# sb17v/GaussianK-SGD

Measured on AMD Instinct MI355X. Metric: images/sec (whole node) ResNet-50 k=0.1% at 1/2/4/8 MI355X; effective grad compression ratio, higher is better.
Workload: dtype fp32; 1 GPU; model=resnet50, global_batch=512, per_gpu_batch=512, image_size=224, parallelism=dp1, compressor=gaussian, buckets=1, threshold=524288000, planner=threshold, exchange=local, momentum_correction=True, hip_graph=False, f32_matmul=bf16x6

## Files before the change

### gaussiank_sgd_amd/models/resnet_imagenet.py

```python
from __future__ import annotations

from typing import List, Optional, Type, Union

import torch
import torch.nn as nn

from ..ops.bn import BNAct, global_avg_pool
from ..ops.conv1x1 import Conv1x1, Conv3x3, conv_stats
from ..ops.stem import StemConv


def conv3x3(inp: int, out: int, stride: int = 1, groups: int = 1, dilation: int = 1) -> nn.Conv2d:
    return Conv3x3(inp, out, stride, groups, dilation)


def conv1x1(inp: int, out: int, stride: int = 1) -> nn.Conv2d:
    return Conv1x1(inp, out, stride)


class BasicBlock(nn.Module):
    expansion = 1

    def __init__(self, inplanes, planes, stride=1, downsample=None, groups=1, base_width=64):
        super().__init__()
        self.conv1 = conv3x3(inplanes, planes, stride)
        self.bn1 = BNAct(planes, act="relu")
        self.conv2 = conv3x3(planes, planes)
        self.bn2 = BNAct(planes, act="relu")
        self.downsample = downsample

    def forward(self, x):
        x, xs = x if isinstance(x, tuple) else (x, x)
        identity = xs if self.downsample is None else _shortcut(self.downsample, xs, self.bn2)
        y, st = conv_stats(self.conv1, x)
        out = self.bn1(y, stats=st)
        y, st = conv_stats(self.conv2, out)
        return self.bn2(y, identity, stats=st)


class Bottleneck(nn.Module):
    expansion = 4

    def __init__(self, inplanes, planes, stride=1, downsample=None, groups=1, base_width=64):
        super().__init__()
        width = int(planes * (base_width / 64.0)) * groups
        self.conv1 = conv1x1(inplanes, width)
        self.bn1 = BNAct(width, act="relu")
        self.conv2 = conv3x3(width, width, stride, groups)
        self.bn2 = BNAct(width, act="relu")
        self.conv3 = conv1x1(width, planes * self.expansion)
        self.bn3 = BNAct(planes * self.expansion, act="relu")
        self.downsample = downsample

    def forward(self, x):
        x, xs = x if isinstance(x, tuple) else (x, x)
        identity = xs if self.downsample is None else _shortcut(self.downsample, xs, self.bn3)
        y, st = conv_stats(self.conv1, x)
        out = self.bn1(y, stats=st)
        y, st = conv_stats(self.conv2, out)
        out = self.bn2(y, stats=st)
        y, st = conv_stats(self.conv3, out)
        return self.bn3(y, identity, stats=st)


class ConvBN(nn.Sequential):

    def forward(self, x):
        y, st = conv_stats(self[0], x)
        return self[1](y, stats=st)

    def forward_deferred(self, x, consumer: BNAct):
        y, st = conv_stats(self[0], x)
        if consumer.fused_ok(y):
            h = self[1].deferred(y, stats=st)
            if h is not None:
                return h
        return self[1](y, stats=st)


def _shortcut(ds: nn.Module, xs: torch.Tensor, consumer: BNAct) -> torch.Tensor:
    if isinstance(ds, ConvBN):
        return ds.forward_deferred(xs, consumer)
    return ds(xs)


class ResNet(nn.Module):
    def __init__(self, block: Type[Union[BasicBlock, Bottleneck]], layers: List[int], num_classes: int = 1000,
                 zero_init_residual: bool = False, groups: int = 1, width_per_group: int = 64,
                 name: Optional[str] = None):
        super().__init__()
        self.inplanes = 64
        self.groups = groups
        self.base_width = width_per_group
        self.conv1 = StemConv(3, 64)
        self.bn1 = BNAct(64, act="relu", pool=(3, 2, 1))
        self.maxpool = nn.Identity()
        self.layer1 = self._make_layer(block, 64, layers[0])
        self.layer2 = self._make_layer(block, 128, layers[1], stride=2)
        self.layer3 = self._make_layer(block, 256, layers[2], stride=2)
        self.layer4 = self._make_layer(block, 512, layers[3], stride=2)
        self.avgpool = nn.AdaptiveAvgPool2d((1, 1))
        self.fc = nn.Linear(512 * block.expansion, num_classes)
        self.name = name or "resnet"
        for m in self.modules():
            if isinstance(m, nn.Conv2d):
                nn.init.kaiming_normal_(m.weight, mode="fan_out", nonlinearity="relu")
            elif isinstance(m, nn.BatchNorm2d):
                nn.init.ones_(m.weight)
                nn.init.zeros_(m.bias)
        blocks = [b for layer in (self.layer1, self.layer2, self.layer3, self.layer4) for b in layer]
        self.bn1.twin = True
        for b in blocks[:-1]:
            (b.bn3 if isinstance(b, Bottleneck) else b.bn2).twin = True
        for i, b in enumerate(blocks):
            b.bn1.bwd_link = True
            if isinstance(b, Bottleneck):
                b.bn2.bwd_link = True
            if i + 1 < len(blocks) and blocks[i + 1].downsample is None:
                (b.bn3 if isinstance(b, Bottleneck) else b.bn2).bwd_link = True
        if zero_init_residual:
            for m in self.modules():
                if isinstance(m, Bottleneck):
                    nn.init.zeros_(m.bn3.weight)
                elif isinstance(m, BasicBlock):
                    nn.init.zeros_(m.bn2.weight)

    def _make_layer(self, block, planes, blocks, stride=1):
        downsample = None
        if stride != 1 or self.inplanes != planes * block.expansion:
            downsample = ConvBN(conv1x1(self.inplanes, planes * block.expansion, stride),
                                BNAct(planes * block.expansion))
        layers = [block(self.inplanes, planes, stride, downsample, self.groups, self.base_width)]
        self.inplanes = planes * block.expansion
        for _ in range(1, blocks):
            layers.append(block(self.inplanes, planes, groups=self.groups, base_width=self.base_width))
        return nn.Sequential(*layers)

    def forward(self, x):
        y, st = conv_stats(self.conv1, x)
        x = self.maxpool(self.bn1(y, stats=st))
        x = self.layer4(self.layer3(self.layer2(self.layer1(x))))
        return self.fc(global_avg_pool(x))


def resnet18(num_classes=1000, **kw):
    return ResNet(BasicBlock, [2, 2, 2, 2], num_classes, name="resnet18", **kw)


def resnet34(num_classes=1000, **kw):
    return ResNet(BasicBlock, [3, 4, 6, 3], num_classes, name="resnet34", **kw)


def resnet50(num_classes=1000, **kw):
    return ResNet(Bottleneck, [3, 4, 6, 3], num_classes, name="resnet50", **kw)


def resnet101(num_classes=1000, **kw):
    return ResNet(Bottleneck, [3, 4, 23, 3], num_classes, name="resnet101", **kw)


def resnet152(num_classes=1000, **kw):
    return ResNet(Bottleneck, [3, 8, 36, 3], num_classes, name="resnet152", **kw)


def resnext50_32x4d(num_classes=1000, **kw):
    return ResNet(Bottleneck, [3, 4, 6, 3], num_classes, groups=32, width_per_group=4, name="resnext50", **kw)
```

### gaussiank_sgd_amd/ops/autotune.py

```python
from __future__ import annotations

import os
from typing import Callable, Dict, Iterable, List, Optional, Tuple

import torch

_TUNE = os.environ.get("GKSGD_GEMM_TUNE", "1") != "0"
_choices: Dict[tuple, tuple] = {}
_OWN = ("hip", "w3", "mat", "wino", "wx6")
_GK_MARGIN = float(os.environ.get("GKSGD_GK_MARGIN", "0.05"))
_timings: Dict[tuple, list] = {}
_NT_CFGS = [1, 2, 3, 4, 11, 13, 21, 22, 23, 24, 111, 113, 121, 122, 123, 124, 25, 26, 27, 125, 126, 127,
            211, 212, 213, 214, 221, 222, 223, 224]
NT_GRIDS = (0, 512, 1 << 20)
_TN_CFGS = [(c, s) for c in (1, 2, 3, 4, 5, 6, 7, 8, 21, 22, 23, 24, 27, 9, 29, 101, 121, 102, 122) for s in (0, 128)]
_NT_CFGS_F32 = [1, 2, 3, 4, 7, 11, 12, 13, 14, 21, 22, 23, 24, 101, 102, 103, 104, 201, 202, 203, 204,
                1001, 1002, 1003, 1004, 1005, 1006, 1007, 1021, 1022, 1101, 1102, 1103]
_TN_CFGS_F32 = [(c, s) for c in (1, 2, 3, 4, 5, 6, 7, 8, 9, 11, 12, 13, 14, 15, 16) for s in (0, 64)]
_TN_SMALL_M = 1 << 17
_TN_SMALL_F32 = [(c, s) for c in (4, 5, 11, 14, 15) for s in (16, 32, 128)]


X6 = 100000
_NT_CFGS_X6 = [c + X6 for c in (1, 2, 3, 4, 5, 6, 7, 12, 13, 101, 102, 103, 104, 105, 106, 107, 202, 203, 1001, 1002, 1003)]
_NT_CFGS_X62 = [2 * X6 + t for t in range(1, 8)] + [3 * X6 + t for t in range(1, 8)]
_F32MM = os.environ.get("GKSGD_F32_MATMUL", "bf16x6")


def set_f32_matmul(mode: str) -> str:
    global _F32MM
    if mode not in ("native", "bf16x6"):
        raise ValueError("f32 matmul mode must be 'native' or 'bf16x6', got %r" % (mode,))
    prev, _F32MM = _F32MM, mode
    return prev


def f32_matmul() -> str:
    return _F32MM


def _x6() -> bool:
    return _F32MM == "bf16x6"


_TN_CFGS_X62 = [(2 * X6 + t, sp) for t in (1, 2, 3, 4, 5, 6, 7, 8) for sp in (0, 64)]


def tn_cfgs(dt: torch.dtype) -> List[Tuple[int, int]]:
    if dt == torch.float32:
        extra = _TN_CFGS_X62 if os.environ.get("GKSGD_TN_X62", "0") == "1" else []
        return _TN_CFGS_F32 + ([(c + X6, sp) for c, sp in _TN_CFGS_F32] + extra if _x6() else [])
    return _TN_CFGS


def tn_small_cfgs(dt: torch.dtype, rows: int) -> List[Tuple[int, int]]:
    if dt != torch.float32 or rows > _TN_SMALL_M:
        return []
    return _TN_SMALL_F32 + ([(c + X6, sp) for c, sp in _TN_SMALL_F32] if _x6() else [])


def nt_cfgs(dt: torch.dtype) -> List[int]:
    if dt == torch.float32:
        return _NT_CFGS_F32 + (_NT_CFGS_X6 + _NT_CFGS_X62 if _x6() else [])
    return _NT_CFGS


_SPLITK_BASE = (4, 1, 1001, 1002, 1003)
_SPLITK_MAX_OUT = 1 << 22
SPLITK_GRIDS = (0, 1 << 20)


def splitk_cfgs(dt: torch.dtype, M: int, N: int, K: int) -> List[int]:
    if dt != torch.float32 or M * N > _SPLITK_MAX_OUT:
        return []
    base = list(_SPLITK_BASE) + ([c + X6 for c in _SPLITK_BASE] if _x6() else [])
    return [c + 10000 * S for S in (2, 4, 8) if K % (64 * S) == 0 and K // S >= 128 for c in base]




def dkey(dt: torch.dtype) -> tuple:
    if dt == torch.float32:
        return ("f32", "x6") if _x6() else ("f32",)
    return ()


def hip_cands(run: Callable[[int, int], object], pairs: Iterable[Tuple[int, int]]) -> list:
    return [(("hip", c, g), (lambda c=c, g=g: run(c, g))) for c, g in pairs]


def _time(fn: Callable[[], None], reps: int = 5) -> float:
    fn()
    a = torch.cuda.Event(enable_timing=True)
    b = torch.cuda.Event(enable_timing=True)
    a.record()
    for _ in range(reps):
        fn()
    b.record()
    b.synchronize()
    return a.elapsed_time(b) / reps


def choice(key: tuple) -> Optional[tuple]:
    return _choices.get(key)


def pick(key: tuple, cands: List[Tuple[tuple, Callable[[], None]]]) -> tuple:
    got = _choices.get(key)
    if got is not None:
        return got
    if len(cands) == 1:
        _choices[key] = cands[0][0]
        return cands[0][0]
    if not _TUNE:
        for tag, fn in cands:
            try:
                fn()
            except RuntimeError:
                continue
            _choices[key] = tag
            return tag
        raise RuntimeError("no candidate ran for %s" % (key,))
    log = _timings.setdefault(key, [])
    screened = []
    for tag, fn in cands:
        try:
            t = _time(fn, reps=3)
        except RuntimeError as e:
            log.append((tag, "error: %s" % str(e).splitlines()[0][:200]))
            continue
        screened.append((t, tag, fn))
    screened.sort(key=lambda e: e[0])
    best, best_t = cands[-1][0], float("inf")
    timed = []
    for _, tag, fn in screened[:4]:
        t = _time(fn, reps=12)
        log.append((tag, round(t, 4)))
        timed.append((t, tag))
        if t < best_t:
            best, best_t = tag, t
    if best[0] not in _OWN and _GK_MARGIN > 0:
        own = [(t, tag) for t, tag in timed if tag[0] in _OWN]
        if own and min(own)[0] <= best_t * (1.0 + _GK_MARGIN):
            best = min(own)[1]
            log.append((best, "kept: within GKSGD_GK_MARGIN of %s" % (best_t,)))
    _choices[key] = best
    return best


def tuning_log() -> Dict[tuple, list]:
    return dict(_timings)


def load_choices(path: str) -> int:
    import json
    try:
        with open(path) as f:
            rows = json.load(f)
    except (OSError, ValueError):
        return 0
    for k, v in rows:
        _choices.setdefault(tuple(k), tuple(v))
    return len(rows)


def save_choices(path: str) -> None:
    import json
    with open(path, "w") as f:
        json.dump([[list(k), list(v)] for k, v in sorted(_choices.items(), key=str)], f, indent=0)


_CACHE = os.environ.get("GKSGD_GEMM_CACHE", os.path.join(os.path.dirname(os.path.dirname(os.path.dirname(
    os.path.abspath(__file__)))), "tuning", "gemm_choices.json"))
if _TUNE and _CACHE and os.path.exists(_CACHE) and os.environ.get("GKSGD_GEMM_RETUNE", "0") == "0":
    load_choices(_CACHE)
    _only = {d for d in os.environ.get("GKSGD_GEMM_RETUNE_ONLY", "").split(",") if d}
    if _only:
        for _k in [k for k in _choices if k and k[0] in _only]:
            del _choices[_k]


def tuned_choices() -> Dict[tuple, tuple]:
    return dict(_choices)
```

### gaussiank_sgd_amd/ops/bn.py

```python
from __future__ import annotations

import os
from typing import Optional

import torch
import torch.nn as nn
import torch.nn.functional as F

from . import load, require_native

_CL = torch.channels_last
_FIN_FUSE = os.environ.get("GKSGD_BN_FIN_FUSE", "0") == "1"


def _ops():
    return torch.ops.gksgd


def _grad_pair(grads, like):
    gs = [g for g in grads if g is not None]
    out = []
    for g in gs:
        g = g.contiguous(memory_format=_CL)
        if g.dtype != like.dtype:
            g = g.to(like.dtype)
        out.append(g)
    return (out + [None, None])[:2]


class BnLink:

    __slots__ = ("h", "mask", "twin", "dy2", "dz", "part")

    def __init__(self):
        self.h = self.mask = self.dy2 = self.dz = self.part = None
        self.twin = False

    def ready(self) -> bool:
        return self.h is not None and (not self.twin or self.dy2 is not None)

    def clear(self) -> None:
        self.h = self.mask = self.dy2 = self.dz = self.part = None


class ProducerLink:

    __slots__ = ("lazy", "dx")

    def __init__(self):
        self.lazy = None
        self.dx = None

    def matches(self, dy: torch.Tensor) -> bool:
        return self.lazy is not None and dy.data_ptr() == self.lazy[0].data_ptr() and dy.shape == self.lazy[0].shape

    def materialize(self) -> torch.Tensor:
        if self.dx is None:
            dz, x, coef, _, _ = self.lazy
            self.dx = torch.empty_like(x, memory_format=_CL)
            _ops().bn_lazy_apply(dz, x, self.dx, coef)
        return self.dx

    def clear(self) -> None:
        self.lazy = self.dx = None


def _lazy_buffers(x: torch.Tensor):
    C = x.shape[1]
    coef = torch.empty(C, 4, dtype=torch.float32, device=x.device)
    padz = torch.empty(C, dtype=x.dtype, device=x.device)
    padx = torch.empty(C, dtype=x.dtype, device=x.device)
    return coef, padz, padx


def _lazy_ok(x: torch.Tensor, plink) -> bool:
    import os
    return (plink is not None and x.dtype == torch.float32 and x.shape[1] % 64 == 0 and
            os.environ.get("GKSGD_BN_LAZY", "0") != "0")


class _BNActFn(torch.autograd.Function):
    @staticmethod
    def forward(ctx, x, residual, weight, bias, running_mean, running_var, momentum, eps, relu, direct=None,
                nbt=None, twin=False, pre=None, link=None, res_link=None, plink=None, fin=None, rbn=None):
        ctx.direct = direct
        ctx.set_materialize_grads(False)
        C = x.shape[1]
        M = x.numel() // C
        eb = x.element_size()
        y = torch.empty_like(x, memory_format=_CL)
        stats = torch.empty(4, C, dtype=torch.float32, device=x.device)
        ws = torch.empty(int(_ops().bn_workspace_floats(M, C, eb)), dtype=torch.float32, device=x.device)
        rscale, rshift, dlink = rbn if rbn is not None else (None, None, None)
        ctx.dlink = dlink
        if rbn is not None and (residual.dtype != x.dtype or not residual.is_contiguous(memory_format=_CL)):
            raise RuntimeError("deferred residual BN: the pending tensor must match x (dtype, channels-last)")
        if residual is not None and residual.dtype != x.dtype:
            residual = residual.to(x.dtype)
        if residual is not None and not residual.is_contiguous(memory_format=_CL):
            residual = residual.contiguous(memory_format=_CL)
        mask = None
        if relu:
            mask = torch.empty(int(_ops().bn_mask_bytes(M, C, eb)), dtype=torch.uint8, device=x.device)
        pre_t, pre_rows = pre if pre is not None else (None, 0)
        _ops().bn_act_forward(x, residual, y, mask, weight, bias, running_mean, running_var, stats[0], stats[1],
                              stats[2], stats[3], ws, float(eps), float(momentum), bool(relu), nbt, pre_t, pre_rows,
                              fin, rscale, rshift)
        ctx.fin = fin
        ctx.relu = bool(relu)
        ctx.has_res = residual is not None
        ctx.save_for_backward(x, mask, weight, stats[0], stats[1])
        ctx.link = link
        ctx.res_link = res_link
        ctx.plink = plink
        if link is not None:
            link.h, link.mask, link.twin = x, mask, bool(twin)
        return (y, y.view_as(y)) if twin else y

    @staticmethod
    def backward(ctx, *grads):
        x, mask, weight, mean, invstd = ctx.saved_tensors
        link, res_link, plink, dlink = ctx.link, ctx.res_link, ctx.plink, ctx.dlink
        ctx.link = ctx.res_link = ctx.plink = ctx.dlink = None
        gw, gb = ctx.direct if ctx.direct is not None else (None, None)
        lazy = _lazy_ok(x, plink) and ctx.needs_input_grad[0]
        if link is not None and link.part is not None:
            dz = grads[0]
            if dz is None or dz.data_ptr() != link.dz.data_ptr():
                raise RuntimeError("BNAct bwd_link: the linked output had another consumer")
            part, rows = link.part
            link.clear()
            g = torch.empty(2, x.shape[1], dtype=torch.float32, device=x.device)
            if lazy:
                coef, padz, padx = _lazy_buffers(x)
                _ops().bn_bwd_lazy_pre(x, part, rows, weight, mean, invstd, g[0], g[1], coef, padz, padx, gw, gb)
                plink.lazy = (dz, x, coef, padz, padx)
                dx = dz
            elif dlink is not None and ctx.needs_input_grad[1]:
                dx = torch.empty_like(x, memory_format=_CL)
                x2 = dlink.x
                dx2 = torch.empty_like(x2, memory_format=_CL)
                g2 = torch.empty(2, x2.shape[1], dtype=torch.float32, device=x.device)
                ws2 = torch.empty(int(_ops().bn_workspace_floats(x2.numel() // x2.shape[1], x2.shape[1],
                                                                 x2.element_size())),
                                  dtype=torch.float32, device=x.device)
                gw2, gb2 = dlink.direct if dlink.direct is not None else (None, None)
                _ops().bn_act_backward_pre_dual(dz, x, dx, weight, mean, invstd, g[0], g[1], part, rows, gw, gb, x2,
                                                dx2, dlink.weight, dlink.mean, dlink.invstd, g2[0], g2[1], ws2, gw2,
                                                gb2)
                dlink.dz, dlink.dx, dlink.g = dz, dx2, g2
            else:
                dx = torch.empty_like(x, memory_format=_CL)
                _ops().bn_act_backward_pre(dz, x, dx, weight, mean, invstd, g[0], g[1], part, rows, gw, gb, ctx.fin)
            dres = dz if ctx.has_res and ctx.needs_input_grad[1] else None
            if res_link is not None and dres is not None:
                res_link.dy2 = dres
            if ctx.direct is not None:
                return (dx, dres) + (None,) * 16
            dgamma = g[0] if weight is not None and ctx.needs_input_grad[2] else None
            dbeta = g[1] if ctx.needs_input_grad[3] else None
            return (dx, dres, dgamma, dbeta) + (None,) * 14
        if link is not None:
            link.clear()
        dy, dy2 = _grad_pair(grads, x)
        if dy is None:
            return (None,) * 18
        C = x.shape[1]
        M = x.numel() // C
        g = torch.empty(2, C, dtype=torch.float32, device=x.device)
        ws = torch.empty(int(_ops().bn_workspace_floats(M, C, x.element_size())), dtype=torch.float32,
                         device=x.device)
        if lazy:
            dz = torch.empty_like(x, memory_format=_CL)
            coef, padz, padx = _lazy_buffers(x)
            _ops().bn_act_backward_lazy(dy, dy2, mask, x, dz, weight, mean, invstd, g[0], g[1], ws, ctx.relu, coef,
                                        padz, padx, gw, gb)
            plink.lazy = (dz, x, coef, padz, padx)
            dx = dz
            dres = dz if ctx.has_res and ctx.needs_input_grad[1] else None
        else:
            dx = torch.empty_like(x, memory_format=_CL)
            dres = torch.empty_like(x, memory_format=_CL) if ctx.has_res and ctx.needs_input_grad[1] else None
            _ops().bn_act_backward(dy, mask, x, dx, dres, weight, mean, invstd, g[0], g[1], ws, ctx.relu, gw, gb,
                                   dy2, ctx.fin)
        if res_link is not None and dres is not None:
            res_link.dy2 = dres
        if ctx.direct is not None:
            return (dx, dres) + (None,) * 16
        dgamma = g[0] if weight is not None and ctx.needs_input_grad[2] else None
        dbeta = g[1] if ctx.needs_input_grad[3] else None
        return (dx, dres, dgamma, dbeta) + (None,) * 14


class DeferLink:

    __slots__ = ("x", "weight", "mean", "invstd", "direct", "dz", "dx", "g")

    def __init__(self, x, weight, mean, invstd, direct):
        self.x, self.weight, self.mean, self.invstd, self.direct = x, weight, mean, invstd, direct
        self.dz = self.dx = self.g = None


class _BNDeferFn(torch.autograd.Function):

    @staticmethod
    def forward(ctx, x, weight, bias, running_mean, running_var, momentum, eps, stats, direct=None, nbt=None,
                pre=None, dlink=None):
        ctx.direct = direct
        ctx.set_materialize_grads(False)
        C = x.shape[1]
        M = x.numel() // C
        ws = torch.empty(int(_ops().bn_workspace_floats(M, C, x.element_size())), dtype=torch.float32,
                         device=x.device)
        pre_t, pre_rows = pre if pre is not None else (None, 0)
        _ops().bn_act_finalize(x, weight, bias, running_mean, running_var, stats[0], stats[1], stats[2], stats[3], ws,
                               float(eps), float(momentum), nbt, pre_t, pre_rows)
        ctx.save_for_backward(x, weight, stats[0], stats[1])
        ctx.dlink = dlink
        return x.view_as(x)

    @staticmethod
    def backward(ctx, dy):
        x, weight, mean, invstd = ctx.saved_tensors
        dl, ctx.dlink = ctx.dlink, None
        if dy is None:
            return (None,) * 12
        if dl is not None and dl.dx is not None and dl.dz is not None and dy.data_ptr() == dl.dz.data_ptr():
            dx, g = dl.dx, dl.g
            dl.dz = dl.dx = dl.g = None
            if ctx.direct is not None:
                return (dx,) + (None,) * 11
            dgamma = g[0] if weight is not None and ctx.needs_input_grad[1] else None
            dbeta = g[1] if ctx.needs_input_grad[2] else None
            return (dx, dgamma, dbeta) + (None,) * 9
        if dl is not None and dl.dx is not None:
            raise RuntimeError("deferred BN: the consumer's gradient reached the shortcut BN as another tensor")
        dy = dy.contiguous(memory_format=_CL)
        if dy.dtype != x.dtype:
            dy = dy.to(x.dtype)
        C = x.shape[1]
        M = x.numel() // C
        g = torch.empty(2, C, dtype=torch.float32, device=x.device)
        ws = torch.empty(int(_ops().bn_workspace_floats(M, C, x.element_size())), dtype=torch.float32,
                         device=x.device)
        gw, gb = ctx.direct if ctx.direct is not None else (None, None)
        dx = torch.empty_like(x, memory_format=_CL)
        _ops().bn_act_backward(dy, None, x, dx, None, weight, mean, invstd, g[0], g[1], ws, False, gw, gb, None, None)
        if ctx.direct is not None:
            return (dx,) + (None,) * 11
        dgamma = g[0] if weight is not None and ctx.needs_input_grad[1] else None
        dbeta = g[1] if ctx.needs_input_grad[2] else None
        return (dx, dgamma, dbeta) + (None,) * 9


_DEFER = os.environ.get("GKSGD_BN_DEFER", "1") != "0"
_DEFER_BWD = os.environ.get("GKSGD_BN_DEFER_BWD", "1") != "0"


class _BNReLUPoolFn(torch.autograd.Function):

    @staticmethod
    def forward(ctx, x, weight, bias, running_mean, running_var, momentum, eps, pool, direct=None, nbt=None,
                twin=False, pre=None):
        ctx.set_materialize_grads(False)
        k, st, pad = pool
        N, C, H, W = x.shape
        OH = (H + 2 * pad - k) // st + 1
        OW = (W + 2 * pad - k) // st + 1
        y = torch.empty((N, C, OH, OW), dtype=x.dtype, device=x.device, memory_format=_CL)
        amax = torch.empty(N * C * OH * OW, dtype=torch.uint8, device=x.device)
        stats = torch.empty(4, C, dtype=torch.float32, device=x.device)
        M = N * H * W
        ws = torch.empty(int(_ops().bn_workspace_floats(M, C, x.element_size())), dtype=torch.float32,
                         device=x.device)
        pre_t, pre_rows = pre if pre is not None else (None, 0)
        _ops().bn_relu_pool_forward(x, y, amax, weight, bias, running_mean, running_var, stats[0], stats[1],
                                    stats[2], stats[3], ws, float(eps), float(momentum), k, st, pad, nbt, pre_t,
                                    pre_rows)
        ctx.pool = (k, st, pad)
        ctx.direct = direct
        ctx.save_for_backward(x, amax, weight, stats[0], stats[1])
        return (y, y.view_as(y)) if twin else y

    @staticmethod
    def backward(ctx, *grads):
        x, amax, weight, mean, invstd = ctx.saved_tensors
        dy, dy2 = _grad_pair(grads, x)
        if dy is None:
            return (None,) * 12
        k, st, pad = ctx.pool
        C = x.shape[1]
        M = x.numel() // C
        dx = torch.empty_like(x, memory_format=_CL)
        g = torch.empty(2, C, dtype=torch.float32, device=x.device)
        ws = torch.empty(int(_ops().bn_workspace_floats(M, C, x.element_size())), dtype=torch.float32,
                         device=x.device)
        gw, gb = ctx.direct if ctx.direct is not None else (None, None)
        _ops().bn_relu_pool_backward(dy, amax, x, dx, weight, mean, invstd, g[0], g[1], ws, k, st, pad, gw, gb, dy2)
        if ctx.direct is not None:
            return (dx,) + (None,) * 11
        dgamma = g[0] if weight is not None and ctx.needs_input_grad[1] else None
        dbeta = g[1] if ctx.needs_input_grad[2] else None
        return (dx, dgamma, dbeta) + (None,) * 9


_supported_cache = {}


def fused_bn_available(x: torch.Tensor) -> bool:
    if not (x.is_cuda and x.dim() == 4 and x.dtype in (torch.bfloat16, torch.float32)):
        return False
    if not x.is_contiguous(memory_format=_CL):
        return False
    key = (x.shape[1], x.element_size())
    ok = _supported_cache.get(key)
    if ok is None:
        if not load():
# ... 122 lines not shown
```

### gaussiank_sgd_amd/ops/conv1x1.py

```python
from __future__ import annotations

import os
from itertools import product
from typing import Dict

import torch
import torch.nn as nn
import torch.nn.functional as F

from . import autotune
from . import load
from . import streams
from . import weight_prep
from .autotune import (X6, f32_matmul, load_choices, save_choices, set_f32_matmul,
                       tuned_choices, tuning_log)

_CL = torch.channels_last
_ENABLED = os.environ.get("GKSGD_FASTCONV", "1") != "0"
_BIAS_COLSUM = os.environ.get("GKSGD_CONV_BIAS_COLSUM", "1") != "0"
_WINO = os.environ.get("GKSGD_WINO", "1") != "0"
_FORCE = os.environ.get("GKSGD_CONV_FORCE", "")
_WINO_GRIDS = (0, 1 << 20)
_zeros: Dict[torch.device, torch.Tensor] = {}

# ... 101 lines not shown
    cands += autotune.hip_cands(run, product(split, autotune.SPLITK_GRIDS))
    wino = bias is None and _wino_ok(dt, k, s, C, K) and _wino_shape_fits(N, H, W, C, K)
    if wino:
        cands += _wino_cands(x, w, y, False, st, wp=wp)

    def miopen():
        out = F.conv2d(x, w, b16, stride=s, padding=p)
        if st is not None and ws is not None:
            g.bn_stats_partials(out.contiguous(memory_format=_CL), ws)
        return out
    ws = None
    if st is not None and autotune.choice(("fwd", N, C, H, W, K, k, s, True) + autotune.dkey(dt)) is None and \
            g.bn_supported(K, x.element_size()):
        ws = torch.empty(int(g.bn_workspace_floats(M, K, x.element_size())), dtype=torch.float32, device=x.device)
    cands.append((("miopen", 0, 0), miopen))
    ch = autotune.pick(("fwd", N, C, H, W, K, k, s, st is not None) + autotune.dkey(dt) +
                       (_wino_tag(C, K) if wino else ()), _forced(cands))
    if ch[0] == "miopen":
        return F.conv2d(x, w, b16, stride=s, padding=p).contiguous(memory_format=_CL)
    if ch[0] in ("wino", "wx6"):
        rows = dict(cands)[ch]()
    else:
        rows = run(ch[1], ch[2])
    if st is not None:
        stats_box.append((st, int(rows)))
    return y


def _lz_kw(lz, rows: bool = False) -> dict:
    _, x, coef, padz, padx = lz
    return dict(lz_x=_rows(x) if rows else x, lz_coef=coef, lz_padz=padz, lz_padx=padx)


def _dgrad(dy: torch.Tensor, w: torch.Tensor, x_shape, s: int, lz=None, plink=None, wp: bool = False) -> torch.Tensor:
    N, C, H, W, K, k, p, OH, OW = _geom(x_shape, w, s)
    g = _g()
    dt = dy.dtype
    xs = torch.empty(x_shape, dtype=dt, device=dy.device, memory_format=_CL)
    kw = _lz_kw(lz, rows=(s == 1 and k == 1)) if lz is not None else {}

    def miopen():
        return torch.ops.aten.convolution_backward(dy, xs, w, None, [s, s], [p, p], [1, 1], False, [0, 0], 1,
                                                   [True, False, False])[0]
    cands = []
    split = []
    dx = None
    if s == 2:
        dx = xs
        z = _zero(dy.device)
        run = lambda c, mb: g.conv_dgrad_s2(dy, w, dx, z, c, mb, **kw)
        cands = autotune.hip_cands(run, product(autotune.nt_cfgs(dt), autotune.NT_GRIDS))
    if s == 1:
        dx = xs
        if k == 1:
            DY, DX = _rows(dy), _rows(dx)
            Wt = _lazy(lambda: weight_prep.transposed_1x1(w, wp))
            run = lambda c, mb: g.gemm_nt(DY, Wt(), DX, c, mb, **kw)
            if lz is None:
                split = autotune.splitk_cfgs(dt, N * H * W, C, K)
        else:
            wf = _lazy(lambda: weight_prep.flipped_3x3(w, wp))
            z = _zero(dy.device)
            run = lambda c, mb: g.conv_nt(dy, wf(), dx, z, 1, p, c, mb, **kw)
        cands = autotune.hip_cands(run, product(autotune.nt_cfgs(dt), autotune.NT_GRIDS))
        cands += autotune.hip_cands(run, product(split, autotune.SPLITK_GRIDS))
    if lz is not None:
        cands.append((("mat", 0, 0), lambda: _dgrad(plink.materialize(), w, x_shape, s, wp=wp)))
        ch = autotune.pick(("dgrad", N, C, H, W, K, k, s) + autotune.dkey(dt) + ("lz",), cands)
        if ch[0] == "mat":
            return _dgrad(plink.materialize(), w, x_shape, s, wp=wp)
        run(ch[1], ch[2])
        return dx
    wino = _wino_ok(dt, k, s, K, C) and _wino_shape_fits(N, H, W, C, K)
    if wino:
        cands += _wino_cands(dy, w, dx, True, wp=wp)
    cands.append((("miopen", 0, 0), miopen))
    ch = autotune.pick(_dgrad_key(N, C, H, W, K, k, s, dt), _forced(cands))
    if ch[0] == "miopen":
        return miopen().contiguous(memory_format=_CL)
    if ch[0] in ("wino", "wx6"):
        dict(cands)[ch]()
        return dx
    run(ch[1], ch[2])
    return dx


_WGRAD_AFTER = os.environ.get("GKSGD_WGRAD_AFTER_DGRAD", "0") == "1"
_SIDE_QROUNDS = int(os.environ.get("GKSGD_WGRAD_SIDE_QROUNDS", "0"))
_FORK_BIAS = os.environ.get("GKSGD_WGRAD_STREAM_BIAS", "0") == "1"
_FORKABLE = tuple(k for k in os.environ.get("GKSGD_WGRAD_STREAM_KINDS", "hip,w3,wino").split(",")
                  if k and (k != "wino" or os.environ.get("GKSGD_WGRAD_STREAM_WINO", "1") == "1"))


def _lazy(make):
    box = []

    def get():
        if not box:
            box.append(make())
        return box[0]
    return get


def _dgrad_key(N, C, H, W, K, k, s, dt) -> tuple:
    wino = _wino_ok(dt, k, s, K, C) and _wino_shape_fits(N, H, W, C, K)
    return ("dgrad", N, C, H, W, K, k, s) + autotune.dkey(dt) + (_wino_tag(K, C) if wino else ())


def _dgrad_bn(dy: torch.Tensor, w: torch.Tensor, x_shape, s: int, link, lz=None, plink=None,
              wp: bool = False) -> torch.Tensor:
    N, C, H, W, K, k, p, OH, OW = _geom(x_shape, w, s)
    kw = _lz_kw(lz, rows=(k == 1)) if lz is not None else {}
    g = _g()
    M = N * H * W
    dt = dy.dtype
    dz = torch.empty(x_shape, dtype=dt, device=dy.device, memory_format=_CL)
    st = torch.empty(2, min(1280, (M + 63) // 64), C, dtype=torch.float32, device=dy.device)
    h, mask, dy2 = link.h, link.mask, link.dy2
    if k == 1:
        DY, DZ = _rows(dy), _rows(dz)
        Wt = _lazy(lambda: weight_prep.transposed_1x1(w, wp))
        H2 = _rows(h)
        D2 = _rows(dy2) if dy2 is not None else None
        run = lambda c, mb: g.gemm_nt(DY, Wt(), DZ, c, mb, st, None, H2, D2, mask, **kw)
        split = autotune.splitk_cfgs(dt, M, C, K) if lz is None else []
    else:
        split = []
        wf = _lazy(lambda: weight_prep.flipped_3x3(w, wp))
        z = _zero(dy.device)
        run = lambda c, mb: g.conv_nt(dy, wf(), dz, z, 1, p, c, mb, st, None, h, dy2, mask, **kw)
    bn_cfgs = [c for c in autotune.nt_cfgs(dt) if c % 10 <= 4 or c >= 1000]
    cands = autotune.hip_cands(run, product(bn_cfgs, autotune.NT_GRIDS))
    cands += autotune.hip_cands(run, product(split, autotune.SPLITK_GRIDS))
    key = ("dgrad_bn", N, C, H, W, K, k, s, dy2 is not None) + autotune.dkey(dt)
    if lz is not None:
        cands.append((("mat", 0, 0), lambda: _dgrad_bn(plink.materialize(), w, x_shape, s, link, wp=wp)))
        ch = autotune.pick(key + ("lz",), cands)
        if ch[0] == "mat":
            return _dgrad_bn(plink.materialize(), w, x_shape, s, link, wp=wp)
    else:
        if _wino_ok(dt, k, s, K, C) and _wino_shape_fits(N, H, W, C, K):
            cands += _wino_cands(dy, w, dz, True, st, (h, dy2, mask), wp=wp)
            key = key + _wino_tag(K, C)
        ch = autotune.pick(key, _forced(cands))
    if ch[0] in ("wino", "wx6"):
        rows = dict(cands)[ch]()
    else:
        rows = run(ch[1], ch[2])
    link.part = (st, int(rows))
    link.dz = dz
    return dz


def _bn_fusable(link, s: int, dgrad_key: tuple) -> bool:
    if link is None or s != 1 or os.environ.get("GKSGD_BN_LINK", "1") == "0" or not link.ready():
        return False
    if link.h.dtype != dgrad_key_dtype(dgrad_key):
        return False
    ch = autotune.choice(dgrad_key)
    return ch is None or ch[0] in ("hip", "wino", "wx6")


def dgrad_key_dtype(key: tuple) -> torch.dtype:
    return torch.float32 if "f32" in key[8:] else torch.bfloat16


def _wgrad_key(x: torch.Tensor, w: torch.Tensor, s: int, lz=None) -> tuple:
    N, C, H, W, K, k, p, OH, OW = _geom(x.shape, w, s)
    wino = lz is None and _wino_ok(x.dtype, k, s, C, K) and C % 64 == 0 and _wino_shape_fits(N, H, W, C, K)
    return ("wgrad", N, C, H, W, K, k, s) + autotune.dkey(x.dtype) + (("lz",) if lz is not None else ()) + \
        (("wino",) if wino else ())


def _wgrad_into(dy: torch.Tensor, x: torch.Tensor, w: torch.Tensor, s: int, out_f32: torch.Tensor, lz=None,
                plink=None, side: bool = False) -> None:
    N, C, H, W, K, k, p, OH, OW = _geom(x.shape, w, s)
    g = _g()
    dt = x.dtype
    key = _wgrad_key(x, w, s, lz)
    scratch = torch.zeros_like(out_f32) if autotune.choice(key) is None else None
    kw = _lz_kw(lz, rows=(k == 1 and s == 1)) if lz is not None else {}

    def miopen():
        return torch.ops.aten.convolution_backward(dy, x, w, None, [s, s], [p, p], [1, 1], False, [0, 0], 1,
                                                   [False, True, False])[1]
    if k == 1 and s == 1:
        DY, X = _rows(dy), _rows(x)
        run = lambda o, c, sp: g.gemm_tn_acc(DY, X, o.view(K, C), c, sp, **kw)
    else:
        z = _zero(x.device)
        run = lambda o, c, sp: g.conv_tn_acc(dy, x, o, z, s, p, c, sp, **kw)
    tn = autotune.tn_cfgs(dt) + autotune.tn_small_cfgs(dt, N * OH * OW)
    cands = autotune.hip_cands(lambda c, sp: run(scratch, c, sp), tn)
    if lz is not None:
        cands.append((("mat", 0, 0), lambda: _wgrad_into(plink.materialize(), x, w, s, scratch)))
        ch = autotune.pick(key, cands)
        if ch[0] == "mat":
            _wgrad_into(plink.materialize(), x, w, s, out_f32)
        else:
            run(out_f32, ch[1], ch[2])
        return
    if key[-1] == "wino":
        def wino_w(o, sp):
            part = torch.empty(int(g.wino_wgrad_ws(N, H, W, C, K, sp)), dtype=torch.float32, device=x.device)
            g.wino_wgrad(x, dy, o, part, sp)
        for sp in (0, 512):
            cands.append((("wino", 0, sp), (lambda sp=sp: wino_w(scratch, sp))))
    w3 = None
    if k == 3 and s == 1 and dt == torch.bfloat16 and g.wgrad3_supported(H, W, C, K):
        def w3(o):
            part = torch.empty(int(g.wgrad3_ws(N, H, W, C, K)), dtype=torch.float32, device=x.device)
            g.conv3_wgrad(dy, x, o, part, _zero(x.device))
        cands.append((("w3", 0, 0), lambda: w3(scratch)))

    def miopen_acc(o):
        from . import accum_grad_
        accum_grad_(o, miopen().contiguous(memory_format=_CL))
    cands.append((("miopen", 0, 0), lambda: miopen_acc(scratch)))
    ch = autotune.pick(key, _forced(cands))
    if ch[0] == "miopen":
        miopen_acc(out_f32)
        return
    if ch[0] == "wino":
        wino_w(out_f32, ch[2])
        return
    if ch[0] == "w3" and w3 is not None:
        w3(out_f32)
        return
    sp = ch[2]
    if side and sp == 0 and _SIDE_QROUNDS > 0:
        sp = -_SIDE_QROUNDS
    run(out_f32, ch[1], sp)


class _FastConvFn(torch.autograd.Function):

    @staticmethod
    def forward(ctx, x, param, w_bf16, sink, stride, stats_box=None, bias=None, bias_sink=None, link=None,
                dt=torch.bfloat16, plink=None):
        if x.dtype != dt:
            x = x.to(dt)
        x = x.contiguous(memory_format=_CL)
        if dt == torch.bfloat16:
            w = w_bf16 if w_bf16 is not None else param.detach().to(torch.bfloat16)
        else:
            w = param.detach()
        w = w.contiguous(memory_format=_CL)
        wp = w.data_ptr() == param.data_ptr() or (w_bf16 is not None and w.data_ptr() == w_bf16.data_ptr())
        b = bias.detach().float().contiguous() if bias is not None else None
        y = _fwd(x, w, stride, stats_box, b, wp=wp)
        ctx.wp = wp
        ctx.prep = weight_prep.current() if wp else None
        ctx.sink = sink
        ctx.bias_sink = bias_sink
        ctx.has_bias = bias is not None
        ctx.stride = stride
        ctx.param_dtype = param.dtype
        ctx.link = link
        ctx.dt = dt
        ctx.plink = plink
        ctx.save_for_backward(x, w)
        return y

    @staticmethod
    def backward(ctx, dy):
        x, w = ctx.saved_tensors
        s = ctx.stride
        dy = dy.to(ctx.dt).contiguous(memory_format=_CL)
        link, ctx.link = ctx.link, None
        plink, ctx.plink = ctx.plink, None
        lz = plink.lazy if plink is not None and plink.matches(dy) else None
        if plink is not None and plink.lazy is not None and lz is None:
            raise RuntimeError("FastConv2d: lazy BN gradient mixed with another consumer of the conv output; "
                               "set GKSGD_BN_LAZY=0 for this model")
        sink = ctx.sink if ctx.needs_input_grad[1] else None
        direct = sink is not None and getattr(sink, "grad_view", None) is not None and \
            sink.grad_view.is_contiguous(memory_format=_CL)
        fork = direct and lz is None and not getattr(sink, "shared", False) and \
            streams.worth(x.device, 2.0 * dy.numel() * x.shape[1] * w.shape[2] * w.shape[3]) and \
            (autotune.choice(_wgrad_key(x, w, s)) or ("",))[0] in _FORKABLE

        bs0 = ctx.bias_sink if ctx.has_bias and ctx.needs_input_grad[6] else None
        gvb = getattr(bs0, "grad_view", None) if bs0 is not None else None
        bias_fork = fork and _FORK_BIAS and _BIAS_COLSUM and gvb is not None and gvb.is_contiguous() and \
            not getattr(bs0, "shared", False) and dy.is_contiguous(memory_format=_CL)

        def fork_wgrad():
            sink.check()
            if bias_fork:
                bs0.check()
            side = streams.fork(x.device)
            with torch.cuda.stream(side):
                _wgrad_into(dy, x, w, s, sink.grad_view, side=True)
                if bias_fork:
                    from .linear import bias_grad_acc_
                    bias_grad_acc_(gvb, _rows(dy))
            streams.hold(x.device, dy, x, w)
        if fork and not _WGRAD_AFTER:
            fork_wgrad()
        dx = None
        if ctx.needs_input_grad[0]:
            N, C, H, W = x.shape
            key = _dgrad_key(N, C, H, W, w.shape[0], w.shape[2], s, ctx.dt)
            prep, ctx.prep = ctx.prep, None
            with weight_prep.use(prep):
                if _bn_fusable(link, s, key):
                    dx = _dgrad_bn(dy, w, x.shape, s, link, lz, plink, wp=ctx.wp)
                else:
                    dx = _dgrad(dy, w, x.shape, s, lz, plink, wp=ctx.wp)
        if fork and _WGRAD_AFTER:
            fork_wgrad()
        gparam = None
        if ctx.needs_input_grad[1] and not fork:
            if direct:
                sink.check()
                _wgrad_into(dy, x, w, s, sink.grad_view, lz, plink)
            else:
                out = torch.zeros(w.shape, dtype=torch.float32, device=x.device).contiguous(memory_format=_CL)
                _wgrad_into(dy, x, w, s, out, lz, plink)
                if sink is not None:
                    sink(out)
                else:
                    gparam = out.to(ctx.param_dtype)
        gbias = None
        if ctx.has_bias and ctx.needs_input_grad[6] and not bias_fork:
            src = plink.materialize() if lz is not None else dy
            bs = ctx.bias_sink
            gv = getattr(bs, "grad_view", None) if bs is not None else None
            if src.is_contiguous(memory_format=_CL) and _BIAS_COLSUM:
                from .linear import bias_grad_acc_
                if gv is not None and gv.is_contiguous():
                    bs.check()
                    bias_grad_acc_(gv, _rows(src))
                    bs = None
                    db = None
                else:
                    db = torch.zeros(src.shape[1], dtype=torch.float32, device=src.device)
                    bias_grad_acc_(db, _rows(src))
            else:
                db = src.sum(dim=(0, 2, 3), dtype=torch.float32)
            if bs is not None:
                bs(db)
            elif db is not None:
                gbias = db
        if plink is not None:
            plink.clear()
        return dx, gparam, None, None, None, None, gbias, None, None, None, None


class FastConv2d(nn.Conv2d):

    def forward(self, x: torch.Tensor) -> torch.Tensor:
        return self._run(x, None)

    def forward_stats(self, x: torch.Tensor):
        box = []
        y = self._run(x, box)
        return y, (box[0] if box else None)

    def _run(self, x: torch.Tensor, box):
        dev = x.device.type
        autocast = torch.is_autocast_enabled(dev)
        bf16 = x.dtype == torch.bfloat16 or (autocast and torch.get_autocast_dtype(dev) == torch.bfloat16)
        f32 = not autocast and x.dtype == torch.float32 and self.weight.dtype == torch.float32 and \
            os.environ.get("GKSGD_FASTCONV_F32", "1") != "0"
        if (bf16 or f32) and supported(x, self) and load():
            if bf16:
                table = getattr(self, "_gk_shadow", None)
                info = table.get("weight") if table else None
                binfo = table.get("bias") if table else None
                use_shadow = info is not None and autocast
                w_bf16, sink = (info[0], info[1]) if use_shadow else (None, None)
                bsink = binfo[1] if (use_shadow and binfo is not None) else None
            else:
                table = getattr(self, "_gk_direct_grads", None) or {}
                w_bf16, sink, bsink = None, table.get("weight"), table.get("bias")
            if not torch.is_grad_enabled() or not self.weight.requires_grad:
                sink = None
            if not torch.is_grad_enabled() or self.bias is None or not self.bias.requires_grad:
                bsink = None
            link = getattr(x, "_gk_bn_link", None)
            plink = None
            if f32 and not bf16 and torch.is_grad_enabled():
                from .bn import ProducerLink
                plink = ProducerLink()
            y = _FastConvFn.apply(x, self.weight, w_bf16, sink, self.stride[0], box, self.bias, bsink, link,
                                  torch.bfloat16 if bf16 else torch.float32, plink)
            if plink is not None:
                y._gk_plink = plink
            return y
        slow = getattr(self, "_gk_slow", None)
        return slow(x) if slow is not None else super().forward(x)


def conv_stats(conv: nn.Module, x: torch.Tensor):
    fs = getattr(conv, "forward_stats", None)
    if fs is not None:
        return fs(x)
    return conv(x), None


class Conv1x1(FastConv2d):

    def __init__(self, inp: int, out: int, stride: int = 1):
        super().__init__(inp, out, 1, stride=stride, bias=False)


class Conv3x3(FastConv2d):

    def __init__(self, inp: int, out: int, stride: int = 1, groups: int = 1, dilation: int = 1):
        super().__init__(inp, out, 3, stride=stride, padding=dilation, groups=groups, bias=False,
                         dilation=dilation)
```

### gaussiank_sgd_amd/ops/csrc/bindings.cpp

```cpp
#include <ATen/ATen.h>
#include <c10/core/DeviceGuard.h>
#include <c10/hip/HIPStream.h>
#include <torch/custom_class.h>
#include <torch/library.h>

#include <cstring>
#include <vector>

#include "comm/rccl_engine.h"
#include "kernels/gemm_cfg.h"
#include "kernels/gk_kernels.h"

namespace {

hipStream_t cur_stream(const at::Tensor& t) {
  return c10::hip::getCurrentHIPStream(t.device().index()).stream();
}

void check_dev(const at::Tensor& t, const char* name) {
  TORCH_CHECK(t.is_cuda(), name, " must be a GPU tensor");
  TORCH_CHECK(t.is_contiguous(), name, " must be contiguous");
}

void check_f32(const at::Tensor& t, const char* name) {
// ... 1031 lines not shown
  if (!st.has_value()) {
    *rows = 0;
    return nullptr;
  }
  const at::Tensor& t = *st;
  TORCH_CHECK(t.is_cuda() && t.scalar_type() == at::kFloat && t.is_contiguous() && t.dim() == 3 && t.size(0) == 2 &&
                  t.size(2) == N && t.size(1) > 0,
              "stats must be a contiguous fp32 [2, rows, N] GPU tensor");
  *rows = (int)t.size(1);
  return t.data_ptr<float>();
}

void check_stem_x(const at::Tensor& x) {
  TORCH_CHECK(x.is_cuda() && x.dim() == 4 && x.size(1) == 3 &&
                  (x.scalar_type() == at::kFloat || x.scalar_type() == at::kBFloat16) &&
                  x.is_contiguous(at::MemoryFormat::ChannelsLast),
              "stem: x must be a channels-last fp32 / bf16 [N, 3, H, W] GPU tensor");
  TORCH_CHECK(gk::stem_supported((int)x.size(2), (int)x.size(3)), "stem: unsupported image size");
  TORCH_CHECK(x.size(0) * x.size(2) * x.size(3) < (int64_t(1) << 31), "stem: batch too large");
}

void stem_pack(at::Tensor w, at::Tensor wp) {
  TORCH_CHECK(w.is_cuda() && w.scalar_type() == at::kFloat && w.dim() == 4 && w.size(0) == 64 && w.size(1) == 3 &&
                  w.size(2) == 7 && w.size(3) == 7,
              "stem_pack: w must be fp32 [64, 3, 7, 7]");
  TORCH_CHECK(wp.is_cuda() && wp.scalar_type() == at::kBFloat16 && wp.is_contiguous() && wp.numel() == 64 * 224,
              "stem_pack: wp must be contiguous bf16 [64, 224]");
  c10::DeviceGuard guard(w.device());
  gk::stem_pack_weight(w.data_ptr<float>(), w.stride(0), w.stride(1), w.stride(2), w.stride(3),
                       static_cast<uint16_t*>(wp.data_ptr()), cur_stream(w));
}

int64_t stem_fwd(at::Tensor x, at::Tensor wp, at::Tensor y, c10::optional<at::Tensor> stats) {
  check_stem_x(x);
  const int64_t N = x.size(0), H = x.size(2), W = x.size(3);
  const int64_t OH = (H - 1) / 2 + 1, OW = (W - 1) / 2 + 1;
  TORCH_CHECK(wp.is_cuda() && wp.scalar_type() == at::kBFloat16 && wp.is_contiguous() && wp.numel() == 64 * 224,
              "stem_fwd: wp must be the packed bf16 [64, 224] weights");
  TORCH_CHECK(y.is_cuda() && y.scalar_type() == at::kBFloat16 && y.dim() == 4 && y.size(0) == N && y.size(1) == 64 &&
                  y.size(2) == OH && y.size(3) == OW && y.is_contiguous(at::MemoryFormat::ChannelsLast),
              "stem_fwd: y must be channels-last bf16 [N, 64, OH, OW]");
  int rows = 0;
  float* sp = stats_ptr(stats, 64, &rows);
  c10::DeviceGuard guard(x.device());
  return gk::stem_forward(x.data_ptr(), x.scalar_type() == at::kFloat, (int)N, (int)H, (int)W,
                          static_cast<const uint16_t*>(wp.data_ptr()), static_cast<uint16_t*>(y.data_ptr()), sp, rows,
                          cur_stream(x));
}

int64_t stem_wgrad_ws(int64_t N, int64_t H, int64_t W) {
  return (int64_t)gk::stem_wgrad_blocks((int)N, (int)H, (int)W) * 64 * 224;
}

void stem_wgrad(at::Tensor x, at::Tensor dy, at::Tensor out, at::Tensor part) {
  check_stem_x(x);
  const int64_t N = x.size(0), H = x.size(2), W = x.size(3);
  const int64_t OH = (H - 1) / 2 + 1, OW = (W - 1) / 2 + 1;
  TORCH_CHECK(dy.is_cuda() && dy.scalar_type() == at::kBFloat16 && dy.dim() == 4 && dy.size(0) == N &&
                  dy.size(1) == 64 && dy.size(2) == OH && dy.size(3) == OW &&
                  dy.is_contiguous(at::MemoryFormat::ChannelsLast),
              "stem_wgrad: dy must be channels-last bf16 [N, 64, OH, OW]");
  TORCH_CHECK(out.is_cuda() && out.scalar_type() == at::kFloat && out.dim() == 4 && out.size(0) == 64 &&
                  out.size(1) == 3 && out.size(2) == 7 && out.size(3) == 7,
              "stem_wgrad: out must be fp32 [64, 3, 7, 7]");
  TORCH_CHECK(part.is_cuda() && part.scalar_type() == at::kFloat && part.is_contiguous() &&
                  part.numel() >= stem_wgrad_ws(N, H, W),
              "stem_wgrad: part must hold stem_wgrad_ws(N, H, W) floats");
  c10::DeviceGuard guard(x.device());
  gk::stem_wgrad(x.data_ptr(), x.scalar_type() == at::kFloat, (int)N, (int)H, (int)W,
                 static_cast<const uint16_t*>(dy.data_ptr()), part.data_ptr<float>(), out.data_ptr<float>(),
                 out.stride(0), out.stride(1), out.stride(2), out.stride(3), cur_stream(x));
}

int64_t stem_f32_fwd(at::Tensor x, at::Tensor w, at::Tensor y, c10::optional<at::Tensor> stats) {
  TORCH_CHECK(x.is_cuda() && x.scalar_type() == at::kFloat && x.dim() == 4 && x.size(1) == 3 &&
                  x.is_contiguous(at::MemoryFormat::ChannelsLast) && gk::stem_f32_supported((int)x.size(2), (int)x.size(3)) &&
                  reinterpret_cast<uintptr_t>(x.data_ptr()) % 16 == 0,
              "stem_f32_fwd: x must be a channels-last fp32 [N, 3, 224, 224] GPU tensor (16-byte aligned)");
  TORCH_CHECK(w.is_cuda() && w.scalar_type() == at::kFloat && w.dim() == 4 && w.size(0) == 64 && w.size(1) == 3 &&
                  w.size(2) == 7 && w.size(3) == 7, "stem_f32_fwd: w must be fp32 [64, 3, 7, 7]");
  const int64_t N = x.size(0);
  TORCH_CHECK(y.is_cuda() && y.scalar_type() == at::kFloat && y.dim() == 4 && y.size(0) == N && y.size(1) == 64 &&
                  y.size(2) == 112 && y.size(3) == 112 && y.is_contiguous(at::MemoryFormat::ChannelsLast),
              "stem_f32_fwd: y must be a channels-last fp32 [N, 64, 112, 112] GPU tensor");
  int rows = 0;
  float* sp = stats_ptr(stats, 64, &rows);
  c10::DeviceGuard guard(x.device());
  return gk::stem_f32_forward(x.data_ptr<float>(), (int)N, (int)x.size(2), (int)x.size(3), w.data_ptr<float>(),
                              w.stride(0), w.stride(1), w.stride(2), w.stride(3), y.data_ptr<float>(), sp, rows,
                              cur_stream(x));
}

int64_t stem_f32x6_wplanes() { return gk::stem_f32x6_wplanes(); }

int64_t stem_f32x6_fwd(at::Tensor x, at::Tensor w, at::Tensor y, c10::optional<at::Tensor> stats, at::Tensor wp3) {
  TORCH_CHECK(x.is_cuda() && x.scalar_type() == at::kFloat && x.dim() == 4 && x.size(1) == 3 &&
                  x.is_contiguous(at::MemoryFormat::ChannelsLast) && gk::stem_f32_supported((int)x.size(2), (int)x.size(3)) &&
                  reinterpret_cast<uintptr_t>(x.data_ptr()) % 16 == 0,
              "stem_f32x6_fwd: x must be a channels-last fp32 [N, 3, 224, 224] GPU tensor (16-byte aligned)");
  TORCH_CHECK(w.is_cuda() && w.scalar_type() == at::kFloat && w.dim() == 4 && w.size(0) == 64 && w.size(1) == 3 &&
                  w.size(2) == 7 && w.size(3) == 7, "stem_f32x6_fwd: w must be fp32 [64, 3, 7, 7]");
  const int64_t N = x.size(0);
  TORCH_CHECK(y.is_cuda() && y.scalar_type() == at::kFloat && y.dim() == 4 && y.size(0) == N && y.size(1) == 64 &&
                  y.size(2) == 112 && y.size(3) == 112 && y.is_contiguous(at::MemoryFormat::ChannelsLast),
              "stem_f32x6_fwd: y must be a channels-last fp32 [N, 64, 112, 112] GPU tensor");
  TORCH_CHECK(wp3.is_cuda() && wp3.scalar_type() == at::kBFloat16 && wp3.is_contiguous() &&
                  wp3.numel() >= gk::stem_f32x6_wplanes() && reinterpret_cast<uintptr_t>(wp3.data_ptr()) % 16 == 0,
              "stem_f32x6_fwd: wp3 must be a contiguous bf16 GPU tensor of stem_f32x6_wplanes() elements");
  int rows = 0;
  float* sp = stats_ptr(stats, 64, &rows);
  c10::DeviceGuard guard(x.device());
  return gk::stem_f32x6_forward(x.data_ptr<float>(), (int)N, (int)x.size(2), (int)x.size(3), w.data_ptr<float>(),
                                w.stride(0), w.stride(1), w.stride(2), w.stride(3),
                                static_cast<uint16_t*>(wp3.data_ptr()), y.data_ptr<float>(), sp, rows, cur_stream(x));
}

int64_t stem_f32_wgrad_ws(int64_t N) { return (int64_t)gk::stem_f32_wgrad_blocks((int)N) * 64 * 148; }

void stem_f32_wgrad(at::Tensor x, at::Tensor dy, at::Tensor out, at::Tensor part, bool x6) {
  TORCH_CHECK(x.is_cuda() && x.scalar_type() == at::kFloat && x.dim() == 4 && x.size(1) == 3 &&
                  x.is_contiguous(at::MemoryFormat::ChannelsLast) && gk::stem_f32_supported((int)x.size(2), (int)x.size(3)) &&
                  reinterpret_cast<uintptr_t>(x.data_ptr()) % 16 == 0,
              "stem_f32_wgrad: x must be a channels-last fp32 [N, 3, 224, 224] GPU tensor (16-byte aligned)");
  const int64_t N = x.size(0);
  TORCH_CHECK(dy.is_cuda() && dy.scalar_type() == at::kFloat && dy.dim() == 4 && dy.size(0) == N &&
                  dy.size(1) == 64 && dy.size(2) == 112 && dy.size(3) == 112 &&
                  dy.is_contiguous(at::MemoryFormat::ChannelsLast),
              "stem_f32_wgrad: dy must be a channels-last fp32 [N, 64, 112, 112] GPU tensor");
  TORCH_CHECK(out.is_cuda() && out.scalar_type() == at::kFloat && out.dim() == 4 && out.size(0) == 64 &&
                  out.size(1) == 3 && out.size(2) == 7 && out.size(3) == 7, "stem_f32_wgrad: out must be fp32 [64, 3, 7, 7]");
  TORCH_CHECK(part.is_cuda() && part.scalar_type() == at::kFloat && part.is_contiguous() &&
                  part.numel() >= stem_f32_wgrad_ws(N), "stem_f32_wgrad: part must hold stem_f32_wgrad_ws(N) floats");
  c10::DeviceGuard guard(x.device());
  gk::stem_f32_wgrad(x.data_ptr<float>(), dy.data_ptr<float>(), (int)N, (int)x.size(2), (int)x.size(3),
                     part.data_ptr<float>(), out.data_ptr<float>(), out.stride(0), out.stride(1), out.stride(2),
                     out.stride(3), x6, cur_stream(x));
}

const uint32_t* seed_word(const c10::optional<at::Tensor>& t) {
  if (!t.has_value() || !t->defined()) return nullptr;
  TORCH_CHECK(t->is_cuda() && t->scalar_type() == at::kInt && t->numel() >= 1, "seed_dev must be a GPU int32[>=1]");
  return reinterpret_cast<const uint32_t*>(t->data_ptr<int32_t>());
}

const float* bias_ptr(const c10::optional<at::Tensor>& b, int64_t N) {
  if (!b.has_value() || !b->defined()) return nullptr;
  TORCH_CHECK(b->is_cuda() && b->scalar_type() == at::kFloat && b->is_contiguous() && b->numel() == N,
              "bias must be a contiguous fp32 [N] GPU tensor");
  return b->data_ptr<float>();
}

bool bn_bwd_args(const c10::optional<at::Tensor>& h, const c10::optional<at::Tensor>& dy2,
                 const c10::optional<at::Tensor>& mask, int64_t M, int64_t N,
                 int64_t ldc, bool has_stats, at::ScalarType dt, gk::BnBwdArgs* out) {
  if (!h.has_value() || !h->defined()) return false;
  TORCH_CHECK(has_stats, "BN-backward epilogue needs the stats partials buffer");
  auto rows_ok = [&](const at::Tensor& t, const char* what) {
    TORCH_CHECK(t.is_cuda() && t.scalar_type() == dt && t.numel() == M * N &&
                    (t.dim() == 2 ? t.stride(0) == ldc && t.stride(1) == 1
                                  : t.is_contiguous(at::MemoryFormat::ChannelsLast) && ldc == N),
                what, " must have C's dtype, shape and row stride");
  };
  rows_ok(*h, "bn h");
  out->h = h->data_ptr();
  out->dy2 = nullptr;
  if (dy2.has_value() && dy2->defined()) {
    rows_ok(*dy2, "bn dy2");
    out->dy2 = dy2->data_ptr();
  }
  out->mask = nullptr;
  if (mask.has_value() && mask->defined()) {
    const int64_t V = dt == at::kFloat ? 4 : 8;
    TORCH_CHECK(mask->is_cuda() && mask->scalar_type() == at::kByte && mask->numel() >= M * (N / V),
                "bn mask must hold M * N / V bytes");
    out->mask = mask->data_ptr<uint8_t>();
  }
  return true;
}

bool lazy_args(const c10::optional<at::Tensor>& x, const c10::optional<at::Tensor>& coef,
               const c10::optional<at::Tensor>& padz, const c10::optional<at::Tensor>& padx, const at::Tensor& dz,
               int64_t C, gk::LazyArgs* out) {
  if (!x.has_value() || !x->defined()) return false;
  TORCH_CHECK(dz.scalar_type() == at::kFloat, "lazy BN operand: fp32 kernels only");
  TORCH_CHECK(x->is_cuda() && x->scalar_type() == dz.scalar_type() && x->sizes() == dz.sizes() &&
                  x->strides() == dz.strides(),
              "lz_x must match the dz operand's dtype, shape and strides");
  TORCH_CHECK(coef.has_value() && coef->defined() && coef->is_cuda() && coef->scalar_type() == at::kFloat &&
                  coef->is_contiguous() && coef->numel() >= 4 * C,
              "lz_coef must be a contiguous fp32 [C, 4] GPU tensor");
  for (const c10::optional<at::Tensor>* t : {&padz, &padx})
    TORCH_CHECK(t->has_value() && (*t)->defined() && (*t)->is_cuda() && (*t)->scalar_type() == dz.scalar_type() &&
                    (*t)->is_contiguous() && (*t)->numel() >= C,
                "lz_padz / lz_padx must be contiguous [C] GPU tensors of dz's dtype");
  TORCH_CHECK(C > 0 && C % 64 == 0, "lazy BN operand: channels must be a multiple of 64");
  out->x = x->data_ptr();
  out->coef = coef->data_ptr<float>();
  out->padz = padz->data_ptr();
  out->padx = padx->data_ptr();
  out->C = (int)C;
  return true;
}

struct NtWordAux {
  at::Tensor ws, b3;
  NtWordAux(const char* op, const gk::cfg::NtWord& w, bool gather, bool f32, bool has_lz, const at::Tensor& B,
            int64_t ldb, int64_t M, int64_t N, int64_t K, int64_t C, hipStream_t stream) {
    if (w.planes > 1) {
      TORCH_CHECK(f32 && !has_lz && w.planes <= 16 && gk::cfg::splitk_divides(w.planes, gather, (int)K, (int)C), op,
                  " split-K: fp32, no lazy operand, S <= 16 ", gather ? "dividing the K slices" : "and K % (64 S) == 0");
      ws = at::empty({w.planes, M, N}, B.options().dtype(at::kFloat));
    }
    if (w.family == 3) {
      TORCH_CHECK(B.scalar_type() == at::kFloat && (gather || K % 32 == 0), op, ": cfg family 3 takes fp32 operands");
      b3 = at::empty({N, 3 * K}, B.options().dtype(at::kBFloat16));
      gk::split3_rows(B.data_ptr<float>(), ldb, b3.data_ptr(), N, (int)K, stream);
    }
  }
  float* ws_ptr() const { return ws.defined() ? ws.data_ptr<float>() : nullptr; }
  const void* b3_ptr() const { return b3.defined() ? b3.data_ptr() : nullptr; }
  static int64_t checked(const char* op, int r) {
    TORCH_CHECK(r != gk::cfg::kRowGemmsOnly, op,
                ": the register-staged bf16x6 kernels (cfg digit 200000/300000) take plain row GEMMs only");
    TORCH_CHECK(r >= 0, op, ": the lazy operand's coefficient table does not fit this tile configuration");
    return r;
  }
};

int64_t gemm_nt(at::Tensor A, at::Tensor B, at::Tensor C, int64_t cfg, int64_t max_blocks,
                c10::optional<at::Tensor> stats, c10::optional<at::Tensor> bias, c10::optional<at::Tensor> bn_h,
                c10::optional<at::Tensor> bn_dy2, c10::optional<at::Tensor> bn_mask, c10::optional<at::Tensor> lz_x, c10::optional<at::Tensor> lz_coef,
                c10::optional<at::Tensor> lz_padz, c10::optional<at::Tensor> lz_padx) {
  check_rows(A, "A", A);
  check_rows(B, "B", A);
  check_rows(C, "C", A);
  const int64_t M = A.size(0), K = A.size(1), N = B.size(0);
  TORCH_CHECK(B.size(1) == K && C.size(0) == M && C.size(1) == N, "gemm_nt: shape mismatch");
  TORCH_CHECK(gk::gemm_supported(N, K), "gemm_nt: N and K must be multiples of 64");
  TORCH_CHECK(M > 0, "gemm_nt: empty M");
  int rows = 0;
  float* sp = stats_ptr(stats, N, &rows);
  gk::BnBwdArgs bn{};
  const bool has_bn = bn_bwd_args(bn_h, bn_dy2, bn_mask, M, N, C.stride(0), sp != nullptr, C.scalar_type(), &bn);
  TORCH_CHECK(!has_bn || !bias.has_value() || !bias->defined(), "gemm_nt: bias and BN epilogue are exclusive");
  gk::LazyArgs lz{};
  const bool has_lz = lazy_args(lz_x, lz_coef, lz_padz, lz_padx, A, K, &lz);
  c10::DeviceGuard guard(A.device());
  const bool f32 = A.scalar_type() == at::kFloat;
  const NtWordAux aux("gemm_nt", gk::cfg::NtWord::decode((int)cfg), false, f32, has_lz, B, B.stride(0), M, N, K, K,
                      cur_stream(A));
  const int r = gk::gemm_nt(A.data_ptr(), A.stride(0), B.data_ptr(), B.stride(0), C.data_ptr(), C.stride(0), M, (int)N,
                            (int)K, f32, (int)cfg, (int)max_blocks, sp, rows, bias_ptr(bias, N),
                            has_bn ? &bn : nullptr, has_lz ? &lz : nullptr, cur_stream(A), aux.ws_ptr(), aux.b3_ptr());
  return NtWordAux::checked("gemm_nt", r);
}

void gemm_tn_acc(at::Tensor G, at::Tensor X, at::Tensor W, int64_t cfg, int64_t splits, c10::optional<at::Tensor> lz_x, c10::optional<at::Tensor> lz_coef,
                c10::optional<at::Tensor> lz_padz, c10::optional<at::Tensor> lz_padx) {
  check_rows(G, "G", G);
  check_rows(X, "X", G);
  TORCH_CHECK(W.is_cuda() && W.scalar_type() == at::kFloat && W.dim() == 2 && W.stride(1) == 1,
              "W must be a 2-D fp32 GPU tensor with contiguous rows");
  const int64_t M = G.size(0), N = G.size(1), K = X.size(1);
  TORCH_CHECK(X.size(0) == M && W.size(0) == N && W.size(1) == K, "gemm_tn_acc: shape mismatch");
  TORCH_CHECK(gk::gemm_supported(N, K), "gemm_tn_acc: N and K must be multiples of 64");
  if (M == 0) return;
  gk::LazyArgs lz{};
  const bool has_lz = lazy_args(lz_x, lz_coef, lz_padz, lz_padx, G, N, &lz);
  c10::DeviceGuard guard(G.device());
  const int rc = gk::gemm_tn_acc(G.data_ptr(), G.stride(0), X.data_ptr(), X.stride(0), W.data_ptr<float>(), W.stride(0), M, (int)N,
                  (int)K, G.scalar_type() == at::kFloat, (int)cfg, (int)splits, has_lz ? &lz : nullptr, cur_stream(G));
  TORCH_CHECK(rc != gk::cfg::kRowGemmsOnly, "gemm_tn_acc: the register-staged bf16x6 kernels (cfg digit 200000) take plain row GEMMs only");
}

void check_zero(const at::Tensor& zero) {
  TORCH_CHECK(zero.is_cuda() && zero.is_contiguous() && zero.numel() * zero.element_size() >= 128,
              "zero must hold >= 128 zero bytes");
}

void check_conv(const at::Tensor& x, const at::Tensor& w, const at::Tensor& zero) {
  TORCH_CHECK(x.is_cuda() && is_gemm_dtype(x) && x.dim() == 4 && x.is_contiguous(at::MemoryFormat::ChannelsLast),
              "conv: x must be a channels-last bf16 or fp32 GPU tensor");
  TORCH_CHECK(w.is_cuda() && w.scalar_type() == x.scalar_type() && w.dim() == 4 &&
                  w.is_contiguous(at::MemoryFormat::ChannelsLast) && w.size(1) == x.size(1),
              "conv: w must be a channels-last [Cout, C, KH, KW] GPU tensor of x's dtype");
  TORCH_CHECK(x.size(1) % 64 == 0 && w.size(0) % 64 == 0, "conv: C and Cout must be multiples of 64");
  check_zero(zero);
}

int64_t conv_nt(at::Tensor x, at::Tensor w, at::Tensor y, at::Tensor zero, int64_t stride, int64_t pad, int64_t cfg,
                int64_t max_blocks, c10::optional<at::Tensor> stats, c10::optional<at::Tensor> bias,
                c10::optional<at::Tensor> bn_h, c10::optional<at::Tensor> bn_dy2, c10::optional<at::Tensor> bn_mask,
                c10::optional<at::Tensor> lz_x, c10::optional<at::Tensor> lz_coef,
                c10::optional<at::Tensor> lz_padz, c10::optional<at::Tensor> lz_padx) {
  check_conv(x, w, zero);
  const int64_t N = x.size(0), C = x.size(1), H = x.size(2), W = x.size(3);
  const int64_t Co = w.size(0), KH = w.size(2), KW = w.size(3);
  const int64_t OH = (H + 2 * pad - KH) / stride + 1, OW = (W + 2 * pad - KW) / stride + 1;
  TORCH_CHECK(KH <= 4 && KW <= 4, "conv_nt: kernels up to 4x4 (gemm.hip kMaxTaps)");
  TORCH_CHECK(y.is_cuda() && y.scalar_type() == x.scalar_type() && y.dim() == 4 &&
                  y.is_contiguous(at::MemoryFormat::ChannelsLast) && y.size(0) == N && y.size(1) == Co &&
                  y.size(2) == OH && y.size(3) == OW,
              "conv_nt: y must be channels-last [N, Cout, OH, OW] of x's dtype");
  const int64_t M = N * OH * OW;
  TORCH_CHECK(M > 0 && M < (int64_t(1) << 32), "conv_nt: M out of range");
  int rows = 0;
  float* sp = stats_ptr(stats, Co, &rows);
  gk::BnBwdArgs bn{};
  const bool has_bn = bn_bwd_args(bn_h, bn_dy2, bn_mask, M, Co, Co, sp != nullptr, y.scalar_type(), &bn);
  TORCH_CHECK(!has_bn || !bias.has_value() || !bias->defined(), "conv_nt: bias and BN epilogue are exclusive");
  gk::LazyArgs lz{};
  const bool has_lz = lazy_args(lz_x, lz_coef, lz_padz, lz_padx, x, C, &lz);
  c10::DeviceGuard guard(x.device());
  const bool f32 = x.scalar_type() == at::kFloat;
  const int64_t K = KH * KW * C;
  const NtWordAux aux("conv_nt", gk::cfg::NtWord::decode((int)cfg), true, f32, has_lz, w, K, M, Co, K, C, cur_stream(x));
  const int r = gk::conv_nt(x.data_ptr(), zero.data_ptr(), (int)H, (int)W, (int)C, (int)OH, (int)OW, (int)stride,
                            (int)pad, (int)KH, (int)KW, w.data_ptr(), y.data_ptr(), M, (int)Co, f32, (int)cfg,
                            (int)max_blocks, sp, rows, bias_ptr(bias, Co), has_bn ? &bn : nullptr,
                            has_lz ? &lz : nullptr, cur_stream(x), aux.ws_ptr(), aux.b3_ptr());
  return NtWordAux::checked("conv_nt", r);
}

int64_t weight_prep_blocks(int64_t kind, int64_t R, int64_t S) { return gk::weight_prep_blocks((int)kind, (int)R, (int)S); }

void weight_prep(at::Tensor table, int64_t ndesc, int64_t total_blocks) {
  TORCH_CHECK(table.is_cuda() && table.scalar_type() == at::kByte && table.is_contiguous() &&
                  table.numel() == ndesc * (int64_t)sizeof(gk::PrepDesc),
              "weight_prep: table must be a contiguous GPU uint8 tensor of ndesc descriptors");
  TORCH_CHECK(ndesc > 0 && ndesc <= gk::weight_prep_max_descs(), "weight_prep: 1..", gk::weight_prep_max_descs(),
              " descriptors");
  TORCH_CHECK(reinterpret_cast<uintptr_t>(table.data_ptr()) % 8 == 0, "weight_prep: table must be 8-byte aligned");
  c10::DeviceGuard guard(table.device());
  gk::weight_prep(reinterpret_cast<const gk::PrepDesc*>(table.data_ptr()), (int)ndesc, total_blocks,
                  cur_stream(table));
}

void wino_weights(at::Tensor w, at::Tensor u, bool flip) {
  TORCH_CHECK(w.is_cuda() && w.scalar_type() == at::kFloat && w.dim() == 4 && w.size(2) == 3 && w.size(3) == 3 &&
                  w.is_contiguous(at::MemoryFormat::ChannelsLast),
              "wino_weights: w must be a channels-last fp32 [K, C, 3, 3] GPU tensor");
  const int64_t K = w.size(0), C = w.size(1);
  const int64_t Co = flip ? C : K, Ci = flip ? K : C;
  TORCH_CHECK(Ci % 8 == 0 && Co % 64 == 0, "wino_weights: input channels % 8 and output channels % 64");
  TORCH_CHECK(u.is_cuda() && u.scalar_type() == at::kFloat && u.is_contiguous() && u.numel() == 16 * K * C,
              "wino_weights: u must be a contiguous fp32 tensor of 16 * K * C elements");
  c10::DeviceGuard guard(w.device());
  gk::wino_weights(w.data_ptr<float>(), u.data_ptr<float>(), (int)Co, (int)Ci, flip ? 1 : 0, cur_stream(w));
}

int64_t wino_conv(at::Tensor x, at::Tensor u, at::Tensor y, int64_t max_blocks, c10::optional<at::Tensor> stats,
                  c10::optional<at::Tensor> bn_h, c10::optional<at::Tensor> bn_dy2, c10::optional<at::Tensor> bn_mask,
                  int64_t splits) {
  TORCH_CHECK(x.is_cuda() && x.scalar_type() == at::kFloat && x.dim() == 4 &&
                  x.is_contiguous(at::MemoryFormat::ChannelsLast),
              "wino_conv: x must be a channels-last fp32 GPU tensor");
  const int64_t N = x.size(0), Ci = x.size(1), H = x.size(2), W = x.size(3);
  TORCH_CHECK(y.is_cuda() && y.scalar_type() == at::kFloat && y.dim() == 4 &&
                  y.is_contiguous(at::MemoryFormat::ChannelsLast) && y.size(0) == N && y.size(2) == H &&
                  y.size(3) == W,
              "wino_conv: y must be a channels-last fp32 [N, Co, H, W] GPU tensor");
  const int64_t Co = y.size(1);
  TORCH_CHECK(Ci % 8 == 0 && Co % 64 == 0, "wino_conv: Ci % 8 == 0 and Co % 64 == 0");
  TORCH_CHECK(u.is_cuda() && u.scalar_type() == at::kFloat && u.is_contiguous() && u.numel() == 16 * Ci * Co,
              "wino_conv: u must hold 16 * Ci * Co fp32 (wino_weights)");
  TORCH_CHECK(N * ((H + 1) / 2) * ((W + 1) / 2) < (int64_t(1) << 31) && x.numel() > 0 &&
                  x.numel() * 4 < (int64_t(1) << 31) && y.numel() * 4 < (int64_t(1) << 31),
              "wino_conv: size out of range (input / output bytes < 2^31: buffer-descriptor addressing)");
  int rows = 0;
  float* sp = stats_ptr(stats, Co, &rows);
  gk::BnBwdArgs bn{};
  const bool has_bn = bn_bwd_args(bn_h, bn_dy2, bn_mask, N * H * W, Co, Co, sp != nullptr, at::kFloat, &bn);
  c10::DeviceGuard guard(x.device());
  TORCH_CHECK(splits >= 1 && splits <= 16 && Ci % (8 * splits) == 0, "wino_conv: splits in [1, 16] dividing Ci / 8");
  at::Tensor ws;
  if (splits > 1) ws = at::empty({splits, N * H * W, Co}, x.options());
  const int r = gk::wino_conv(x.data_ptr<float>(), u.data_ptr<float>(), y.data_ptr<float>(), (int)N, (int)H, (int)W,
                              (int)Ci, (int)Co, (int)max_blocks, sp, rows, has_bn ? &bn : nullptr, cur_stream(x),
                              (int)splits, splits > 1 ? ws.data_ptr<float>() : nullptr);
  TORCH_CHECK(r >= 0, "wino_conv: split configuration refused");
  return r;
}

void wino_x6_weights(at::Tensor w, at::Tensor u3, bool flip) {
  TORCH_CHECK(w.is_cuda() && w.scalar_type() == at::kFloat && w.dim() == 4 && w.size(2) == 3 && w.size(3) == 3 &&
                  w.is_contiguous(at::MemoryFormat::ChannelsLast),
              "wino_x6_weights: w must be a channels-last fp32 [K, C, 3, 3] GPU tensor");
  const int64_t K = w.size(0), C = w.size(1);
  const int64_t Co = flip ? C : K, Ci = flip ? K : C;
  TORCH_CHECK(Ci % 32 == 0 && Co % 32 == 0, "wino_x6_weights: input and output channels % 32");
  TORCH_CHECK(u3.is_cuda() && u3.scalar_type() == at::kBFloat16 && u3.is_contiguous() && u3.numel() == 48 * K * C,
              "wino_x6_weights: u3 must be a contiguous bf16 tensor of 48 * K * C elements");
  c10::DeviceGuard guard(w.device());
  gk::wino_x6_weights(w.data_ptr<float>(), reinterpret_cast<uint16_t*>(u3.data_ptr()), (int)Co, (int)Ci,
                      flip ? 1 : 0, cur_stream(w));
}
// ... 536 lines not shown
                  B3.stride(0) % 8 == 0,
              "lstm_rec_gemm_x6: fp32 A / bf16 B3 GPU operands with unit column stride and 16-byte aligned rows");
  TORCH_CHECK(reinterpret_cast<uintptr_t>(A.data_ptr()) % 16 == 0 && reinterpret_cast<uintptr_t>(B3.data_ptr()) % 16 == 0,
              "lstm_rec_gemm_x6: 16-byte aligned operands");
  check_lstm(P, at::kFloat, S * M * N, "P");
  c10::DeviceGuard guard(A.device());
  gk::lstm_rec_gemm_x6(A.data_ptr<float>(), A.stride(0), static_cast<const uint16_t*>(B3.data_ptr()), B3.stride(1),
                       B3.stride(0), P.data_ptr<float>(), (int)M, (int)N, (int)K, (int)S, cur_stream(A));
}

void lstm_cell_fwd(at::Tensor xg, c10::optional<at::Tensor> hg, c10::optional<at::Tensor> P, int64_t S, at::Tensor c_prev, at::Tensor c,
                   at::Tensor h, c10::optional<at::Tensor> h_pad, at::Tensor gates) {
  TORCH_CHECK(xg.dim() == 2 && xg.size(1) % 4 == 0, "xg must be [B, 4H]");
  const int64_t B = xg.size(0), H = xg.size(1) / 4;
  const bool f32 = xg.scalar_type() == at::kFloat;
  const auto dt = f32 ? at::kFloat : at::kBFloat16;
  check_lstm(xg, dt, B * 4 * H, "xg");
  check_lstm(c_prev, at::kFloat, B * H, "c_prev");
  check_lstm(c, at::kFloat, B * H, "c");
  check_lstm(h, dt, B * H, "h");
  check_lstm(gates, at::kFloat, B * 4 * H, "gates");
  const float* pp = nullptr;
  int64_t Hp = lstm_partials(P, S, B, H, 4, &pp);
  if (!pp) S = 0, Hp = (H + 63) / 64 * 64;
  void* hp = lstm_pad(h_pad, B, Hp, "h_pad", dt);
  const void* ph = lstm_pad(hg, B, 4 * H, "hg", dt);
  c10::DeviceGuard guard(xg.device());
  if (f32)
    gk::lstm_cell_fwd_f32(xg.data_ptr<float>(), static_cast<const float*>(ph), pp, (int)S, c_prev.data_ptr<float>(),
                          c.data_ptr<float>(), h.data_ptr<float>(), static_cast<float*>(hp), gates.data_ptr<float>(),
                          (int)B, (int)H, (int)Hp, cur_stream(xg));
  else
    gk::lstm_cell_fwd(static_cast<const uint16_t*>(xg.data_ptr()), static_cast<const uint16_t*>(ph), pp, (int)S,
                      c_prev.data_ptr<float>(), c.data_ptr<float>(), static_cast<uint16_t*>(h.data_ptr()),
                      static_cast<uint16_t*>(hp), gates.data_ptr<float>(), (int)B, (int)H, (int)Hp, cur_stream(xg));
}

void lstm_cell_bwd(c10::optional<at::Tensor> dout, c10::optional<at::Tensor> dh_rec, c10::optional<at::Tensor> P,
                   int64_t S,
                   c10::optional<at::Tensor> dc_next, at::Tensor gates, at::Tensor c, at::Tensor c_prev, at::Tensor dG,
                   c10::optional<at::Tensor> dG_pad, at::Tensor dc_prev) {
  TORCH_CHECK(gates.dim() == 2 && gates.size(1) % 4 == 0, "gates must be [B, 4H]");
  const int64_t B = gates.size(0), H = gates.size(1) / 4;
  const bool f32 = dG.scalar_type() == at::kFloat;
  const auto dt = f32 ? at::kFloat : at::kBFloat16;
  check_lstm(gates, at::kFloat, B * 4 * H, "gates");
  check_lstm(c, at::kFloat, B * H, "c");
  check_lstm(c_prev, at::kFloat, B * H, "c_prev");
  check_lstm(dG, dt, B * 4 * H, "dG");
  check_lstm(dc_prev, at::kFloat, B * H, "dc_prev");
  const void* po = nullptr;
  const float* pc = nullptr;
  if (dout.has_value() && dout->defined()) {
    check_lstm(*dout, dt, B * H, "dout");
    po = dout->data_ptr();
  }
  if (dc_next.has_value() && dc_next->defined()) {
    check_lstm(*dc_next, at::kFloat, B * H, "dc_next");
    pc = dc_next->data_ptr<float>();
  }
  const float* pp = nullptr;
  int64_t Hp = lstm_partials(P, S, B, H, 1, &pp);
  if (!pp) S = 0, Hp = (H + 63) / 64 * 64;
  void* gp = lstm_pad(dG_pad, B, 4 * Hp, "dG_pad", dt);
  const void* pr = lstm_pad(dh_rec, B, H, "dh_rec", dt);
  c10::DeviceGuard guard(gates.device());
  if (f32)
    gk::lstm_cell_bwd_f32(static_cast<const float*>(po), static_cast<const float*>(pr), pp, (int)S, pc,
                          gates.data_ptr<float>(), c.data_ptr<float>(), c_prev.data_ptr<float>(), dG.data_ptr<float>(),
                          static_cast<float*>(gp), dc_prev.data_ptr<float>(), (int)B, (int)H, (int)Hp, cur_stream(gates));
  else
    gk::lstm_cell_bwd(static_cast<const uint16_t*>(po), static_cast<const uint16_t*>(pr), pp, (int)S, pc,
                      gates.data_ptr<float>(), c.data_ptr<float>(), c_prev.data_ptr<float>(),
                      static_cast<uint16_t*>(dG.data_ptr()), static_cast<uint16_t*>(gp), dc_prev.data_ptr<float>(),
                      (int)B, (int)H, (int)Hp, cur_stream(gates));
}

}


TORCH_LIBRARY(gksgd, m) {
  m.def("ctrl_bytes() -> int", &ctrl_bytes);
  m.def("workspace_bytes() -> int", &workspace_bytes);
  m.def(
      "compress(Tensor(a!) g, Tensor(b!) r, Tensor(c!) ctrl, Tensor(d!) ws, Tensor(e!) record, int mode, bool ec, "
      "bool zero_g, int loops, float z, float fixed_thr, float sample_p, int k, int k_cap, int seed, "
      "int n_stats, Tensor(f!)? stats_out=None, Tensor? valid=None, Tensor(g!)? u=None, Tensor? w=None, "
      "Tensor? chunks=None, int chunk_begin=0, int chunk_count=0, int chunk_base=0, float[] mc_mu=[], "
      "float[] mc_wd=[], Tensor? seed_dev=None, int handoff=-1) -> ()");
  m.def("apply_records_sgd(Tensor(a!) w, Tensor(b!)? w_bf16, Tensor records, int P, int k_cap, float scale, float lr, "
        "Tensor? lr_mult=None) -> ()");
  m.def("arena_digest(Tensor x, Tensor(a!) out, Tensor(b!) ws) -> ()");
  m.def("tensor_stats(Tensor x, Tensor(a!) ctrl, Tensor(b!) ws) -> ()");
  m.def("quality_workspace_bytes() -> int", &quality_workspace_bytes);
  m.def("selection_quality(Tensor r, Tensor record, int k, int k_cap, Tensor(a!) out, Tensor(b!) ws) -> ()");
  m.def("scatter_add_records(Tensor(a!) dst, Tensor records, int P, int k_cap, float scale, bool deterministic) -> ()");
  m.def("fill_zero(Tensor(a!) dst) -> ()");
  m.def("sign_bucket_workspace_bytes() -> int", &sign_bucket_workspace_bytes);
  m.def("sign_bucket_compress(Tensor(a!) x, Tensor(b!) mask, Tensor(c!) means, Tensor(d!) ws) -> ()");
  m.def("sign_bucket_decompress(Tensor(a!) x, Tensor mask, Tensor means) -> ()");
  m.def(
      "fused_sgd(Tensor(a!) w, Tensor(b!)? m, Tensor(c!) g, Tensor chunks, float[] lr, float[] momentum, "
      "float[] dampening, float[] weight_decay, int[] nesterov, int[] first_step, bool zero_grad, "
      "Tensor? grad_scale=None, Tensor(d!)? w_bf16=None, Tensor? lr_mult=None) -> ()");
  m.def(
      "fused_adam(Tensor(a!) w, Tensor(b!) m, Tensor(c!) v, Tensor(d!) g, Tensor chunks, Tensor(e!) step, float[] lr, "
      "float[] beta1, float[] beta2, float[] eps, float[] weight_decay, int[] decoupled, bool zero_grad, "
      "Tensor? grad_scale=None, Tensor(f!)? w_bf16=None, Tensor? lr_mult=None) -> ()");
  m.def(
      "fused_lamb(Tensor(a!) w, Tensor(b!) m, Tensor(c!) v, Tensor(d!) g, Tensor chunks, Tensor(e!) step, "
      "Tensor seg_range, Tensor(f!) part, Tensor(g!) trust, float[] lr, float[] beta1, float[] beta2, float[] eps, "
      "float[] weight_decay, int[] adapt, float[] trust_clip, bool zero_grad, Tensor? grad_scale=None, "
      "Tensor(h!)? w_bf16=None, Tensor? lr_mult=None, int passes=7) -> ()");
  m.def("segmented_sumsq(Tensor w, Tensor g, Tensor chunks, Tensor(a!) out) -> ()");
  m.def(
      "fused_lars(Tensor(a!) w, Tensor(b!) m, Tensor g, Tensor chunks, Tensor seg_sumsq, float[] lr, "
      "float[] momentum, float[] weight_decay, float[] eeta, float[] epsilon) -> ()");
  m.def("clip_grad_norm(Tensor(a!) g, float max_norm, Tensor(b!) ws, Tensor(c!) coef, Tensor(d!) norm) -> ()");

  m.def("bn_workspace_floats(int M, int C, int elem_bytes) -> int", &bn_workspace_floats);
  m.def("bn_supported(int C, int elem_bytes) -> bool", &bn_supported);
  m.def("bn_set_blocks(int blocks) -> ()", [](int64_t b) { gk::bn_set_blocks((int)b); });
  m.def("bn_mask_bytes(int M, int C, int elem_bytes) -> int", &bn_mask_bytes);
  m.def(
      "bn_act_forward(Tensor x, Tensor? res, Tensor(a!) y, Tensor(i!)? mask, Tensor? w, Tensor? b, Tensor(b!)? run_mean, "
      "Tensor(c!)? run_var, Tensor(d!) save_mean, Tensor(e!) save_invstd, Tensor(f!) scale, Tensor(g!) shift, "
      "Tensor(h!) ws, float eps, float momentum, bool relu, Tensor(j!)? nbt=None, Tensor? pre=None, "
      "int pre_rows=0, Tensor(k!)? fin=None, Tensor? rscale=None, Tensor? rshift=None) -> ()");
  m.def(
      "bn_act_finalize(Tensor x, Tensor? w, Tensor? b, Tensor(a!)? run_mean, Tensor(b!)? run_var, "
      "Tensor(c!) save_mean, Tensor(d!) save_invstd, Tensor(e!) scale, Tensor(f!) shift, Tensor(g!) ws, float eps, "
      "float momentum, Tensor(h!)? nbt=None, Tensor? pre=None, int pre_rows=0) -> ()");
  m.def(
      "bn_relu_pool_forward(Tensor x, Tensor(a!) y, Tensor(b!) amax, Tensor? w, Tensor? b, Tensor(c!)? run_mean, "
      "Tensor(d!)? run_var, Tensor(e!) save_mean, Tensor(f!) save_invstd, Tensor(g!) scale, Tensor(h!) shift, "
      "Tensor(i!) ws, float eps, float momentum, int k, int s, int p, Tensor(j!)? nbt=None, Tensor? pre=None, "
      "int pre_rows=0) -> ()");
  m.def(
      "bn_relu_pool_backward(Tensor dy, Tensor amax, Tensor x, Tensor(a!) dx, Tensor? w, Tensor mean, "
      "Tensor invstd, Tensor(b!) dgamma, Tensor(c!) dbeta, Tensor(d!) ws, int k, int s, int p, "
      "Tensor(e!)? gw_acc=None, Tensor(f!)? gb_acc=None, Tensor? dy2=None) -> ()");
  m.def(
      "bn_act_backward(Tensor dy, Tensor? mask, Tensor x, Tensor(a!) dx, Tensor(b!)? dres, Tensor? w, Tensor mean, "
      "Tensor invstd, Tensor(c!) dgamma, Tensor(d!) dbeta, Tensor(e!) ws, bool relu, Tensor(f!)? gw_acc=None, "
      "Tensor(g!)? gb_acc=None, Tensor? dy2=None, Tensor(h!)? fin=None) -> ()");
  m.def("accum_grad(Tensor(a!) dst, Tensor src) -> ()");
  m.def(
      "momentum_correct(Tensor(a!) u, Tensor(b!) g, Tensor w, Tensor chunks, int begin, int count, "
      "float[] momentum, float[] weight_decay) -> ()");
  m.def("mask_records(Tensor(a!) u, Tensor record, int k_cap) -> ()");
  m.def("cast_bf16(Tensor(a!) dst, Tensor src) -> ()");
  m.def("gemm_supported(int N, int K) -> bool", &gemm_supported);
  m.def("gemm_nt(Tensor A, Tensor B, Tensor(a!) C, int cfg=0, int max_blocks=0, Tensor(b!)? stats=None, "
        "Tensor? bias=None, Tensor? bn_h=None, Tensor? bn_dy2=None, Tensor? bn_mask=None, Tensor? lz_x=None, Tensor? lz_coef=None, Tensor? lz_padz=None, Tensor? lz_padx=None) -> int");
  m.def("gemm_tn_acc(Tensor G, Tensor X, Tensor(a!) W, int cfg=0, int splits=0, Tensor? lz_x=None, Tensor? lz_coef=None, Tensor? lz_padz=None, Tensor? lz_padx=None) -> ()");
  m.def("conv_nt(Tensor x, Tensor w, Tensor(a!) y, Tensor zero, int stride, int pad, int cfg=0, int max_blocks=0, "
        "Tensor(b!)? stats=None, Tensor? bias=None, Tensor? bn_h=None, Tensor? bn_dy2=None, Tensor? bn_mask=None, "
        "Tensor? lz_x=None, Tensor? lz_coef=None, Tensor? lz_padz=None, Tensor? lz_padx=None) -> int");
  m.def("stem_supported(int H, int W) -> bool", [](int64_t H, int64_t W) { return gk::stem_supported((int)H, (int)W); });
  m.def("stem_wgrad_ws(int N, int H, int W) -> int", &stem_wgrad_ws);
  m.def("stem_pack(Tensor w, Tensor(a!) wp) -> ()");
  m.def("stem_fwd(Tensor x, Tensor wp, Tensor(a!) y, Tensor(b!)? stats=None) -> int");
  m.def("stem_wgrad(Tensor x, Tensor dy, Tensor(a!) out, Tensor(b!) part) -> ()");
  m.def("stem_f32_supported(int H, int W) -> bool", [](int64_t H, int64_t W) { return gk::stem_f32_supported((int)H, (int)W); });
  m.def("stem_f32_fwd(Tensor x, Tensor w, Tensor(a!) y, Tensor(b!)? stats=None) -> int");
  m.def("stem_f32x6_wplanes() -> int", &stem_f32x6_wplanes);
  m.def("stem_f32x6_fwd(Tensor x, Tensor w, Tensor(a!) y, Tensor(b!)? stats, Tensor(c!) wp3) -> int");
  m.def("stem_f32_wgrad_ws(int N) -> int", &stem_f32_wgrad_ws);
  m.def("stem_f32_wgrad(Tensor x, Tensor dy, Tensor(a!) out, Tensor(b!) part, bool x6=False) -> ()");
  m.def("wgrad3_supported(int H, int W, int C, int K) -> bool", [](int64_t H, int64_t W, int64_t C, int64_t K) {
    return gk::wgrad3_supported((int)H, (int)W, (int)C, (int)K);
  });
  m.def("wgrad3_ws(int N, int H, int W, int C, int K) -> int", &wgrad3_ws);
  m.def("conv3_wgrad(Tensor dy, Tensor x, Tensor(a!) out, Tensor(b!) part, Tensor zero) -> ()");
  m.def("wino_weights(Tensor w, Tensor(a!) u, bool flip) -> ()");
  m.def("weight_prep(Tensor table, int ndesc, int total_blocks) -> ()");
  m.def("weight_prep_blocks(int kind, int R, int S) -> int", &weight_prep_blocks);
  m.def("wino_wgrad_ws(int N, int H, int W, int C, int K, int splits=0) -> int", &wino_wgrad_ws);
  m.def("wino_wgrad(Tensor x, Tensor dy, Tensor(a!) out, Tensor(b!) part, int splits=0) -> ()");
  m.def("wino_conv(Tensor x, Tensor u, Tensor(a!) y, int max_blocks=0, Tensor(b!)? stats=None, Tensor? bn_h=None, "
        "Tensor? bn_dy2=None, Tensor? bn_mask=None, int splits=1) -> int");
  m.def("wino_x6_weights(Tensor w, Tensor(a!) u3, bool flip) -> ()");
  m.def("wino_x6_conv(Tensor x, Tensor u3, Tensor(a!) y, int max_blocks=0, Tensor(b!)? stats=None, "
        "Tensor? bn_h=None, Tensor? bn_dy2=None, Tensor? bn_mask=None) -> int");
  m.def("conv_dgrad_s2(Tensor dy, Tensor w, Tensor(a!) dx, Tensor zero, int cfg=0, int max_blocks=0, "
        "Tensor? lz_x=None, Tensor? lz_coef=None, Tensor? lz_padz=None, Tensor? lz_padx=None) -> ()");
  m.def("bn_bwd_lazy_pre(Tensor x, Tensor part, int rows, Tensor? w, Tensor mean, Tensor invstd, "
        "Tensor(a!) dgamma, Tensor(b!) dbeta, Tensor(c!) coef, Tensor(d!) padz, Tensor(e!) padx, "
        "Tensor(f!)? gw_acc=None, Tensor(g!)? gb_acc=None) -> ()");
  m.def("bn_act_backward_lazy(Tensor dy, Tensor? dy2, Tensor? mask, Tensor x, Tensor(a!) dz, Tensor? w, "
        "Tensor mean, Tensor invstd, Tensor(b!) dgamma, Tensor(c!) dbeta, Tensor(d!) ws, bool relu, "
        "Tensor(e!) coef, Tensor(f!) padz, Tensor(g!) padx, Tensor(h!)? gw_acc=None, Tensor(i!)? gb_acc=None) -> ()");
  m.def("bn_lazy_apply(Tensor dz, Tensor x, Tensor(a!) dx, Tensor coef) -> ()");
  m.def("bn_stats_partials(Tensor x, Tensor(a!) ws) -> ()");
  m.def(
      "bn_act_backward_pre_dual(Tensor dz, Tensor x, Tensor(a!) dx, Tensor? w, Tensor mean, Tensor invstd, "
      "Tensor(b!) dgamma, Tensor(c!) dbeta, Tensor part, int rows, Tensor(d!)? gw_acc, Tensor(e!)? gb_acc, Tensor x2, "
      "Tensor(f!) dx2, Tensor? w2, Tensor mean2, Tensor invstd2, Tensor(g!) dgamma2, Tensor(h!) dbeta2, "
      "Tensor(i!) ws2, Tensor(j!)? gw2_acc, Tensor(k!)? gb2_acc) -> ()");
  m.def("bn_act_backward_pre(Tensor dz, Tensor x, Tensor(a!) dx, Tensor? w, Tensor mean, Tensor invstd, "
        "Tensor(b!) dgamma, Tensor(c!) dbeta, Tensor part, int rows, Tensor(d!)? gw_acc=None, "
        "Tensor(e!)? gb_acc=None, Tensor(f!)? fin=None) -> ()");
  m.def("bn_fin_state_bytes(int C) -> int", &bn_fin_state_bytes);
  m.def("attn_supported(int T, int D) -> bool",
        [](int64_t T, int64_t D) { return gk::attn_supported((int)T, (int)D); });
  m.def("attn_fwd(Tensor qkv, Tensor(a!) out, Tensor(b!) lse, int heads, float p, int seed, Tensor? seed_dev=None, "
        "Tensor? key_bits=None, Tensor(c!)? out_lo=None) -> ()");
  m.def("attn_pack_key_mask(Tensor mask, Tensor(a!) bits) -> ()");
  m.def("attn_bwd(Tensor qkv, Tensor out, Tensor dout, Tensor lse, Tensor(a!) delta, Tensor(b!) dqkv, int heads, "
        "float p, int seed, Tensor? seed_dev=None, Tensor? key_bits=None, Tensor? out_lo=None) -> ()");
  m.def("attn_dropout_mask(Tensor(a!) mask, int B, int heads, int T, float p, int seed, Tensor? seed_dev=None) -> ()");
  m.def("attn_f32_fwd(Tensor qkv, Tensor(a!) out, Tensor(b!) lse, int heads, float p, int seed, Tensor? seed_dev=None, "
        "Tensor? key_bits=None) -> ()");
  m.def("attn_f32_bwd(Tensor qkv, Tensor out, Tensor dout, Tensor lse, Tensor(a!) delta, Tensor(b!) dqkv, int heads, "
        "float p, int seed, Tensor? seed_dev=None, Tensor? key_bits=None) -> ()");
  m.def("attn_f32_supported(int T, int D) -> bool",
        [](int64_t T, int64_t D) { return gk::attn_f32_supported((int)T, (int)D); });
  m.def("add_ln_supported(int H) -> bool", &add_ln_supported);
  m.def("add_ln_ws_floats(int R, int H) -> int", &add_ln_ws_floats);
  m.def("xent_supported(int V) -> bool", &xent_supported);
  m.def("xent_forward(Tensor logits, Tensor labels, Tensor(a!) lse, Tensor(b!) loss, int ignore) -> ()");
  m.def("xent_backward(Tensor logits, Tensor labels, Tensor lse, Tensor scale, Tensor(a!) grad, int ignore) -> ()");
  m.def("emb_supported(int H, int NT) -> bool", &emb_supported);
  m.def("emb_part_floats(int H) -> int", &emb_part_floats);
  m.def("emb_forward(Tensor ids, Tensor? tt, Tensor Ww, Tensor Wp, Tensor Wt, Tensor(a!) out) -> ()");
  m.def("emb_word_ws_ints(int V, int M) -> int", &emb_word_ws_ints);
  m.def("emb_word_part_floats(int M, int H) -> int", &emb_word_part_floats);
  m.def("emb_backward(Tensor ids, Tensor? tt, Tensor dx, Tensor(a!)? dWw, Tensor(b!)? dWp, Tensor(c!)? dWt, "
        "Tensor(d!) part, Tensor sid, Tensor order, Tensor(e!) wws, Tensor(f!) wpart) -> ()");
  m.def("add_ln_forward(Tensor a, Tensor x, Tensor? gamma, Tensor? beta, Tensor(a!) y, Tensor(b!) h, "
        "Tensor(c!) mean, Tensor(d!) rstd, float eps, float p, int seed, Tensor? seed_dev=None) -> ()");
  m.def("add_ln_backward(Tensor dy, Tensor h, Tensor mean, Tensor rstd, Tensor? gamma, Tensor(a!) dx, "
        "Tensor(b!)? da, Tensor(c!)? dgamma, Tensor(d!)? dbeta, bool accumulate, Tensor(e!) ws, float p, int seed, "
        "Tensor? seed_dev=None) -> ()");
  m.def("conv_tn_acc(Tensor dy, Tensor x, Tensor(a!) wout, Tensor zero, int stride, int pad, int cfg=0, int splits=0, "
        "Tensor? lz_x=None, Tensor? lz_coef=None, Tensor? lz_padz=None, Tensor? lz_padx=None) -> ()");
  m.def("colsum_acc(Tensor dy, Tensor(a!) db) -> ()");
  m.def("gelu_bwd_colsum(Tensor dy, Tensor pre, Tensor(a!) dpre, Tensor(b!)? db=None) -> ()");
  m.def("lstm_rec_gemm(Tensor A, Tensor B, Tensor(a!) P, int S) -> ()");
  m.def("lstm_rec_gemm_x6(Tensor A, Tensor B3, Tensor(a!) P, int S) -> ()");
  m.def("lstm_cell_fwd(Tensor xg, Tensor? hg, Tensor? P, int S, Tensor c_prev, Tensor(a!) c, Tensor(b!) h, Tensor(c!)? h_pad, "
        "Tensor(d!) gates) -> ()");
  m.def("lstm_cell_bwd(Tensor? dout, Tensor? dh_rec, Tensor? P, int S, Tensor? dc_next, Tensor gates, Tensor c, Tensor c_prev, "
        "Tensor(a!) dG, Tensor(b!)? dG_pad, Tensor(c!) dc_prev) -> ()");

  m.class_<RcclEngine>("RcclEngine")
      .def(torch::init<>())
      .def_static("unique_id", &RcclEngine::unique_id)
      .def("init", &RcclEngine::init)
      .def("init_async", &RcclEngine::init_async)
      .def("init_poll", &RcclEngine::init_poll)
      .def("init_wait", &RcclEngine::init_wait)
      .def("abort", &RcclEngine::abort)
      .def("set_op_timeout", &RcclEngine::set_op_timeout)
      .def("allgather", &RcclEngine::allgather)
      .def("allreduce", &RcclEngine::allreduce)
      .def("broadcast", &RcclEngine::broadcast)
      .def("allgather_many", &RcclEngine::allgather_many)
      .def("set_tracking", &RcclEngine::set_tracking)
      .def("start_watchdog", &RcclEngine::start_watchdog)
      .def("stop_watchdog", &RcclEngine::stop_watchdog)
      .def("poll", &RcclEngine::poll)
      .def("failed", &RcclEngine::failed)
      .def("error", &RcclEngine::error)
      .def("check", &RcclEngine::check)
      .def("in_flight", &RcclEngine::in_flight)
      .def("reset_stats", &RcclEngine::reset_stats)
      .def("stats", &RcclEngine::stats)
      .def("inject_failure", &RcclEngine::inject_failure)
      .def("destroy", &RcclEngine::destroy)
      .def("rank", &RcclEngine::rank)
      .def("world", &RcclEngine::world);
}

TORCH_LIBRARY_IMPL(gksgd, CUDA, m) {
  m.impl("compress", &compress);
  m.impl("tensor_stats", &tensor_stats);
  m.impl("selection_quality", &selection_quality);
  m.impl("scatter_add_records", &scatter_add_records);
  m.impl("apply_records_sgd", &apply_records_sgd);
  m.impl("arena_digest", &arena_digest);
  m.impl("fill_zero", &fill_zero);
  m.impl("sign_bucket_compress", &sign_bucket_compress);
  m.impl("sign_bucket_decompress", &sign_bucket_decompress);
  m.impl("fused_sgd", &fused_sgd);
  m.impl("fused_adam", &fused_adam);
  m.impl("fused_lamb", &fused_lamb);
  m.impl("segmented_sumsq", &segmented_sumsq);
  m.impl("fused_lars", &fused_lars);
  m.impl("clip_grad_norm", &clip_grad_norm);
  m.impl("bn_act_forward", &bn_act_forward);
  m.impl("bn_act_finalize", &bn_act_finalize);
  m.impl("bn_act_backward", &bn_act_backward);
  m.impl("bn_act_backward_pre", &bn_act_backward_pre);
  m.impl("bn_act_backward_pre_dual", &bn_act_backward_pre_dual);
  m.impl("bn_bwd_lazy_pre", &bn_bwd_lazy_pre);
  m.impl("bn_act_backward_lazy", &bn_act_backward_lazy);
  m.impl("bn_lazy_apply", &bn_lazy_apply);
  m.impl("bn_stats_partials", &bn_stats_partials);
  m.impl("stem_pack", &stem_pack);
  m.impl("conv_dgrad_s2", &conv_dgrad_s2);
  m.impl("conv3_wgrad", &conv3_wgrad);
  m.impl("stem_fwd", &stem_fwd);
  m.impl("stem_wgrad", &stem_wgrad);
  m.impl("stem_f32_fwd", &stem_f32_fwd);
  m.impl("stem_f32x6_fwd", &stem_f32x6_fwd);
  m.impl("stem_f32_wgrad", &stem_f32_wgrad);
// ... 36 lines not shown
```

### gaussiank_sgd_amd/ops/csrc/kernels/gemm.hip

```cpp
#include "common.h"
#include "gemm_cfg.h"
#include "gemm_units.h"
#include "mfma_util.h"

namespace gk {

static int nt_unit(cfg::Unit unit, bool gather, GK_NT_UNIT_ARGS) {
  switch (unit) {
    case cfg::Unit::b16: return gather ? nt_b16_gat(GK_NT_UNIT_PASS) : nt_b16_row(GK_NT_UNIT_PASS);
    case cfg::Unit::x6: return gather ? nt_x6_gat(GK_NT_UNIT_PASS) : nt_x6_row(GK_NT_UNIT_PASS);
    case cfg::Unit::x62:
      if (gather)
        return nt_x62_gat(static_cast<const float*>(A), static_cast<const float*>(B), static_cast<float*>(C), M, N, K,
                          w, max_blocks, geo, stats, stats_ld, stats_rows, bb, stream);
      return nt_x62_row(static_cast<const float*>(A), lda, static_cast<const float*>(B), ldb, static_cast<float*>(C),
                        ldc, M, N, K, w, max_blocks, geo.bias, stats, stats_ld, stats_rows, bb, geo.b3, stream);
    default: return gather ? nt_f32_gat(GK_NT_UNIT_PASS) : nt_f32_row(GK_NT_UNIT_PASS);
  }
}

__global__ __launch_bounds__(256) void split3_rows_kernel(const float* __restrict__ src, int64_t ld,
                                                          uint16_t* __restrict__ dst, int64_t R, int S) {
  const int64_t g8 = S / 8;
  const int64_t t = (int64_t)blockIdx.x * 256 + threadIdx.x;
  if (t >= R * g8) return;
  const int64_t r = t / g8;
  const int g = (int)(t - r * g8);
  const float* p = src + r * ld + 8 * g;
  bf16x8 h, m, l;
  split3x8(*reinterpret_cast<const f32x4*>(p), *reinterpret_cast<const f32x4*>(p + 4), h, m, l);
  uint16_t* d = dst + (r * (S / 32) + g / 4) * 96 + (g % 4) * 8;
  *reinterpret_cast<bf16x8*>(d) = h;
  *reinterpret_cast<bf16x8*>(d + 32) = m;
  *reinterpret_cast<bf16x8*>(d + 64) = l;
}

void split3_rows(const float* src, int64_t ld, void* dst, int64_t R, int S, hipStream_t stream) {
  const int64_t n = R * (S / 8);
  if (n <= 0) return;
  hipLaunchKernelGGL(split3_rows_kernel, dim3((unsigned)((n + 255) / 256)), dim3(256), 0, stream, src, ld,
                     static_cast<uint16_t*>(dst), R, S);
}

bool gemm_supported(int64_t N, int64_t K) { return N >= 64 && K >= 64 && N % 64 == 0 && K % 64 == 0; }


__global__ __launch_bounds__(256) void nt_splitk_reduce_kernel(const float* __restrict__ ws, int S, int64_t M, int N,
                                                               float* __restrict__ C, int64_t ldc,
                                                               const float* __restrict__ bias,
                                                               float* __restrict__ stats, int64_t stats_ld,
                                                               int64_t rows_per_block, BnBwd bb) {
  const int q = threadIdx.x & 63, rl = threadIdx.x >> 6;
  const int n = (blockIdx.y * 64 + q) * 4;
  const bool colok = n < N;
  const int64_t r0 = (int64_t)blockIdx.x * rows_per_block;
  const int64_t r1 = r0 + rows_per_block < M ? r0 + rows_per_block : M;
  const int64_t plane = M * (int64_t)N;
  const float* hp = static_cast<const float*>(bb.h);
  const float* d2p = static_cast<const float*>(bb.dy2);
  f32x4 b = f32x4{0.f, 0.f, 0.f, 0.f};
  if (bias && colok) b = *reinterpret_cast<const f32x4*>(bias + n);
  float ps[4] = {0.f, 0.f, 0.f, 0.f}, pq[4] = {0.f, 0.f, 0.f, 0.f};
  if (colok) {
    for (int64_t m = r0 + rl; m < r1; m += 4) {
      const float* src = ws + m * N + n;
      f32x4 v = *reinterpret_cast<const f32x4*>(src);
      for (int z = 1; z < S; ++z) v += *reinterpret_cast<const f32x4*>(src + z * plane);
      v += b;
      if (hp) {
        const f32x4 hv = *reinterpret_cast<const f32x4*>(hp + m * ldc + n);
        const f32x4 d2 = d2p ? *reinterpret_cast<const f32x4*>(d2p + m * ldc + n) : f32x4{0.f, 0.f, 0.f, 0.f};
        const uint32_t bits = bb.mask ? (uint32_t)bb.mask[m * (N >> 2) + (n >> 2)] : 0xfu;
#pragma unroll
        for (int r = 0; r < 4; ++r) {
          const float dz = (bits >> r) & 1u ? v[r] + d2[r] : 0.f;
          v[r] = dz;
          ps[r] += dz;
          pq[r] = fmaf(dz, hv[r], pq[r]);
        }
      } else if (stats) {
#pragma unroll
        for (int r = 0; r < 4; ++r) {
          ps[r] += v[r];
          pq[r] = fmaf(v[r], v[r], pq[r]);
        }
      }
      *reinterpret_cast<f32x4*>(C + m * ldc + n) = v;
    }
  }
  if (!stats) return;
  __shared__ float red[2][4][256];
#pragma unroll
  for (int r = 0; r < 4; ++r) {
    red[0][rl][q * 4 + r] = ps[r];
    red[1][rl][q * 4 + r] = pq[r];
  }
  __syncthreads();
  const int c = threadIdx.x;
  const int nc = blockIdx.y * 256 + c;
  if (nc < N) {
    const float sa = (red[0][0][c] + red[0][1][c]) + (red[0][2][c] + red[0][3][c]);
    const float sb = (red[1][0][c] + red[1][1][c]) + (red[1][2][c] + red[1][3][c]);
    stats[(int64_t)blockIdx.x * N + nc] = sa;
    stats[stats_ld + (int64_t)blockIdx.x * N + nc] = sb;
  }
}

int splitk_reduce(const float* ws, int S, int64_t M, int N, float* C, int64_t ldc, const float* bias, float* stats,
                  int stats_rows, const BnBwdArgs* bn, hipStream_t stream) {
  const BnBwd bb = bn ? BnBwd{bn->h, bn->dy2, bn->mask} : BnBwd{};
  const int ny = (N + 255) / 256;
  int64_t gx = 1024 / ny;
  const int64_t rmax = (M + 3) / 4;
  if (gx > rmax) gx = rmax;
  if (stats && gx > stats_rows) gx = stats_rows;
  if (gx < 1) gx = 1;
  const int64_t rpb = (M + gx - 1) / gx;
  gx = (M + rpb - 1) / rpb;
  hipLaunchKernelGGL(nt_splitk_reduce_kernel, dim3((unsigned)gx, (unsigned)ny), dim3(256), 0, stream, ws, S, M, N, C,
                     ldc, bias, stats, (int64_t)stats_rows * N, rpb, bb);
  return (int)gx;
}

static int nt_run(bool f32, bool gather, const void* A, int64_t lda, const void* B, int64_t ldb, void* C, int64_t ldc,
                  int64_t M, int N, int K, int cfg_word, int max_blocks, const ConvGeo& g, float* stats, int stats_rows,
                  const BnBwdArgs* bn, const LazyArgs* lazy, float* splitk_ws, hipStream_t stream) {
  const cfg::NtWord w = cfg::NtWord::decode(cfg_word);
  if (!f32) lazy = nullptr;
  const int64_t x_elems = gather ? M / ((int64_t)g.OH * g.OW) * g.H * g.W * g.C : 0;
  const cfg::NtPlan p = cfg::nt_plan(w, f32, gather, lazy != nullptr, g.b3 != nullptr, g.RH != 0, splitk_ws != nullptr, K,
                                     g.C, x_elems);
  if (p.status < 0) return p.status;
  if (p.planes > 1) {
    ConvGeo gz = g;
    gz.bias = nullptr;
    gz.b3 = nullptr;
    gz.KZ = p.planes;
    const int r = nt_unit(p.unit, gather, A, lda, B, ldb, splitk_ws, N, M, N, K / p.planes, w, max_blocks, gz, nullptr, 0,
                          0, BnBwd{}, nullptr, stream);
    if (r < 0) return r;
    return splitk_reduce(splitk_ws, p.planes, M, N, static_cast<float*>(C), ldc, g.bias, stats, stats_rows, bn, stream);
  }
  const BnBwd bb = bn ? BnBwd{bn->h, bn->dy2, bn->mask} : BnBwd{};
  return nt_unit(p.unit, gather, A, lda, B, ldb, C, ldc, M, N, K, w, max_blocks, g, stats, (int64_t)stats_rows * N,
                 stats_rows, bb, lazy, stream);
}

int gemm_nt(const void* A, int64_t lda, const void* B, int64_t ldb, void* C, int64_t ldc, int64_t M, int N, int K,
            bool f32, int cfg, int max_blocks, float* stats, int stats_rows, const float* bias, const BnBwdArgs* bn,
            const LazyArgs* lazy, hipStream_t stream, float* splitk_ws, const void* b3) {
  ConvGeo g{};
  g.bias = bias;
  g.b3 = static_cast<const uint16_t*>(b3);
  return nt_run(f32, false, A, lda, B, ldb, C, ldc, M, N, K, cfg, max_blocks, g, stats, stats_rows, bn, lazy, splitk_ws,
                stream);
}

int conv_nt(const void* X, const void* zero, int H, int W, int C, int OH, int OW, int S, int P, int KH, int KW,
            const void* B, void* Y, int64_t M, int N, bool f32, int cfg, int max_blocks, float* stats, int stats_rows,
            const float* bias, const BnBwdArgs* bn, const LazyArgs* lazy, hipStream_t stream, float* splitk_ws, const void* b3) {
  ConvGeo g{zero, H, W, C, OH, OW, S, P, KW, bias};
  g.b3 = static_cast<const uint16_t*>(b3);
  const int K = KH * KW * C;
  return nt_run(f32, true, X, C, B, K, Y, N, M, N, K, cfg, max_blocks, g, stats, stats_rows, bn, lazy, splitk_ws, stream);
}

int conv_nt_remap(const void* X, int64_t ldx, const void* zero, int H, int W, int C, int OH, int OW, int KH, int KW,
                  const void* B, void* Y, int64_t M, int N, int RH, int RW, int RA, int RB, int RZ, bool f32, int cfg,
                  int max_blocks, const LazyArgs* lazy, hipStream_t stream) {
  ConvGeo g{zero, H, W, C, OH, OW, 1, 0, KW, nullptr, RH, RW, RA, RB, RZ};
  const int K = KH * KW * C;
  const bool gather = KH * KW != 1;
  return nt_run(f32, gather, X, gather ? C : ldx, B, K, Y, N, M, N, K, cfg, max_blocks, g, nullptr, 0, nullptr, lazy,
                nullptr, stream);
}

static int tn_run(bool f32, bool gather, const void* G, int64_t ldg, const void* X, int64_t ldx, float* W, int64_t ldw,
                  int64_t M, int N, int K, int cfg_word, int splits, const ConvGeo& geo, const LazyArgs* lazy,
                  hipStream_t stream) {
  if (!f32) {
    tn_unit_b16(gather, G, ldg, X, ldx, W, ldw, M, N, K, cfg::TnWord::decode(cfg_word), splits, geo, stream);
    return 0;
  }
  const cfg::TnF32Word w = cfg::TnF32Word::decode(cfg_word);
  const cfg::TnPlan p = cfg::tn_plan(w, gather, lazy != nullptr);
  if (p.status < 0) return p.status;
  auto g = static_cast<const float*>(G);
  auto x = static_cast<const float*>(X);
  if (p.unit == cfg::Unit::x62) tn_x62_row(g, ldg, x, ldx, W, ldw, M, N, K, w, splits, stream);
  else if (p.unit == cfg::Unit::x6) tn_unit_x6(gather, g, ldg, x, ldx, W, ldw, M, N, K, w, splits, geo, lazy, stream);
  else tn_unit_f32(gather, g, ldg, x, ldx, W, ldw, M, N, K, w, splits, geo, lazy, stream);
  return 0;
}

int gemm_tn_acc(const void* G, int64_t ldg, const void* X, int64_t ldx, float* W, int64_t ldw, int64_t M, int N,
                 int K, bool f32, int cfg, int splits, const LazyArgs* lazy, hipStream_t stream) {
  return tn_run(f32, false, G, ldg, X, ldx, W, ldw, M, N, K, cfg, splits, ConvGeo{}, lazy, stream);
}

int conv_tn_acc(const void* G, const void* X, const void* zero, int H, int W_, int C, int OH, int OW, int S, int P,
                 int KH, int KW, float* Wout, int64_t M, int N, bool f32, int cfg, int splits, const LazyArgs* lazy,
                 hipStream_t stream) {
  ConvGeo g{zero, H, W_, C, OH, OW, S, P, KW, nullptr};
  const int K = KH * KW * C;
  return tn_run(f32, true, G, N, X, C, Wout, K, M, N, K, cfg, splits, g, lazy, stream);
}

}
```

### gaussiank_sgd_amd/ops/csrc/kernels/gemm_cfg.h

```cpp
#pragma once

#include <cstdint>

namespace gk {
namespace cfg {

enum Status : int {
  kDoesNotFit = -1,
  kRowGemmsOnly = -2,
};

inline int family_of(int cfg) {
  const int f = (cfg / 100000) % 10;
  return f >= 1 && f <= 3 ? f : 0;
}

struct NtWord {
  int tile;
  int panel;
  int stages;
  bool wave32;
  int planes;
  int family;
  static NtWord decode(int cfg) {
    const int p = (cfg / 10) % 10, s = (cfg / 100) % 10;
    return NtWord{cfg % 10,           p == 0 ? -1 : (p == 1 ? 1 : 0), s == 1 ? 2 : (s == 2 ? 4 : 3),
                  (cfg / 1000) % 10 == 1, (cfg / 10000) % 10,             family_of(cfg)};
  }
};

struct TnWord {
  int tile;
  int stages;
  static TnWord decode(int cfg) { return TnWord{cfg % 10 + 10 * ((cfg / 100) % 10), (cfg / 10) % 10 == 2 ? 3 : 2}; }
};

struct TnF32Word {
  int tile;
  int stages;
  int family;
  static TnF32Word decode(int cfg) {
    return TnF32Word{(cfg % 100000) % 10, (cfg / 10) % 10 != 1 ? 3 : 2, family_of(cfg)};
  }
};

struct NtSel {
  int wm, wn, msb;
  bool bnb, lz;
  int panel, stages;
};
constexpr int nt_key(int wm, int wn, int msb, bool bnb, bool lz) {
  return (((wm * 8 + wn) * 16 + msb) * 2 + (bnb ? 1 : 0)) * 2 + (lz ? 1 : 0);
}

inline NtSel nt_select(const NtWord& w, int N, bool f32, bool x6, bool bn, bool lazy) {
  static const int bn64[8] = {64, 64, 128, 256, 128, 256, 128, 256};
  int t = w.tile;
  if (t <= 0) t = N % 256 == 0 ? 3 : (N % 128 == 0 ? 2 : 1);
  if (t > 7 || N % bn64[t] != 0) t = 1;
  NtSel s{4, 1, 4, bn, f32 && lazy, w.panel, w.stages};
  if (f32 && w.wave32 && !lazy) {
    static const int bn32[8] = {64, 64, 128, 64, 256, 128, 256, 128};
    static const int wm32[8] = {4, 4, 2, 2, 1, 4, 2, 1}, wn32[8] = {1, 1, 2, 1, 4, 2, 4, 2};
    t = w.tile;
    if (t <= 0 || t > 7 || N % bn32[t] != 0) t = 1;
    s.wm = wm32[t], s.wn = wn32[t], s.msb = 2;
    return s;
  }
  if (bn || s.lz) {
    static const int wm[8] = {4, 4, 4, 2, 2, 2, 2, 2}, wn[8] = {1, 1, 2, 4, 2, 4, 2, 4};
    s.wm = wm[t], s.wn = wn[t];
    return s;
  }
  static const int wm[8] = {4, 4, 4, 2, 2, 2, 2, 1}, wn[8] = {1, 1, 2, 4, 2, 4, 2, 4};
  s.wm = wm[t], s.wn = wn[t];
  if (t >= 5 && (!f32 || x6)) s.msb = 8;
  return s;
}

struct TnSel {
  int wn, wk, ws, stages;
};
constexpr int tn_key(int wn, int wk, int ws) { return (wn * 8 + wk) * 8 + ws; }

inline TnSel tn_select(const TnWord& w, int N, int K) {
  static const int bn[13] = {64, 64, 128, 64, 128, 256, 64, 128, 64, 256, 64, 128, 256};
  static const int bk[13] = {64, 64, 64, 128, 128, 64, 256, 128, 64, 128, 64, 256, 256};
  static const int wn[13] = {1, 1, 2, 1, 2, 4, 1, 2, 1, 4, 1, 2, 4}, wk[13] = {1, 1, 1, 2, 2, 1, 4, 2, 1, 2, 1, 4, 4};
  static const int ws[13] = {4, 4, 2, 2, 1, 1, 1, 2, 2, 1, 4, 1, 1};
  int t = w.tile;
  if (t <= 0) {
    const bool n2 = N % 128 == 0, k2 = K % 128 == 0;
    t = n2 && k2 ? 7 : (n2 ? 2 : (k2 ? 3 : 1));
  }
  if (t > 12 || t == 10 || N % bn[t] != 0 || K % bk[t] != 0) t = 1;
  return TnSel{wn[t], wk[t], ws[t], w.stages};
}

struct TnF32Sel {
  int wn, wk;
  bool lz;
  int stages;
};
constexpr int tn_f32_key(int wn, int wk) { return wn * 8 + wk; }

inline TnF32Sel tn_f32_select(const TnF32Word& w, int N, int K, bool lazy) {
  static const int bn[10] = {64, 64, 128, 64, 128, 256, 64, 256, 128, 256};
  static const int bk[10] = {64, 64, 64, 128, 128, 64, 256, 128, 256, 256};
  int t = w.tile;
  if (t <= 0) t = (N % 128 == 0 && K % 128 == 0) ? 4 : (N % 128 == 0 ? 2 : (K % 128 == 0 ? 3 : 1));
  if (N % bn[t] != 0 || K % bk[t] != 0) t = 1;
  if (t == 9 && lazy) t = 8;
  return TnF32Sel{bn[t] / 64, bk[t] / 64, lazy, w.stages};
}

struct X62NtSel {
  int wm, wn;
  bool p3, bnb;
};
constexpr int x62_key(int a, int b) { return a * 8 + b; }

inline X62NtSel nt_x62_select(const NtWord& w, int N, bool b3, bool bn) {
  static const int bnw[8] = {128, 128, 256, 128, 256, 64, 128, 64};
  static const int wm[8] = {2, 2, 2, 4, 1, 4, 1, 2};
  int t = w.tile;
  if (t < 1 || t > 7 || N % bnw[t] != 0) t = N % 128 == 0 ? 1 : 7;
  if (N % bnw[t] != 0) t = 5;
  return X62NtSel{wm[t], bnw[t] / 64, b3, bn};
}

struct X62TnSel {
  int wn, wk;
};

inline X62TnSel tn_x62_select(const TnF32Word& w, int N, int K) {
  static const int bn[9] = {64, 64, 128, 64, 128, 256, 64, 256, 128};
  static const int bk[9] = {64, 64, 64, 128, 128, 64, 256, 128, 256};
  int t = w.tile;
  if (t < 1 || t > 8 || N % bn[t] != 0 || K % bk[t] != 0) t = 1;
  return X62TnSel{bn[t] / 64, bk[t] / 64};
}

enum class Unit { b16, f32, x6, x62 };

struct NtPlan {
  int status;
  int planes;
  Unit unit;
};

inline bool splitk_divides(int S, bool gather, int K, int C) {
  return gather ? C % 32 == 0 && (K / 32) % S == 0 : K % (64 * S) == 0;
}

inline NtPlan nt_plan(const NtWord& w, bool f32, bool gather, bool lazy, bool b3, bool remap, bool have_ws,
                      int K, int C, int64_t x_elems) {
  NtPlan p{0, 1, !f32 ? Unit::b16 : (w.family >= 2 ? Unit::x62 : (w.family == 1 ? Unit::x6 : Unit::f32))};
  if (!remap && w.planes > 1) {
    const int S = p.planes = w.planes;
    if (!f32 || lazy || !have_ws || !splitk_divides(S, gather, K, C)) p.status = kDoesNotFit;
  }
  if (p.status == 0 && p.unit == Unit::x62) {
// ... 20 lines not shown
```

### gaussiank_sgd_amd/ops/csrc/kernels/gemm_nt_x62.h

```cpp
#pragma once

#include "gemm_common.h"

namespace gk {
namespace {

template <int WM, int WN>
struct X62Cfg {
  static constexpr int NW = WM * WN;
  static constexpr int THREADS = 64 * NW;
  static constexpr int BM = 64 * WM;
  static constexpr int BN = 64 * WN;
  static constexpr int PA = BM * 64;
  static constexpr int PB = BN * 64;
  static constexpr int STAGE = 3 * (PA + PB);
  static constexpr int LDS = 2 * STAGE;
  static constexpr int PRA = BM * 4 / THREADS;
  static constexpr int PRB = BN * 4 / THREADS;
  static_assert(PRA >= 1 && PRB >= 1 && (BM * 4) % THREADS == 0 && (BN * 4) % THREADS == 0, "pieces per thread");
  static_assert(LDS <= 160 * 1024, "LDS");
};

template <int WM, int WN, bool BNB, int NPF = 1, bool GATHER = false, bool P3 = false>
__global__ void __launch_bounds__(64 * WM * WN) __attribute__((amdgpu_waves_per_eu(1)))
gemm_nt_x62_kernel(const float* __restrict__ A, int64_t lda, const float* __restrict__ B, int64_t ldb,
                   float* __restrict__ C, int64_t ldc, int64_t M, int K, const float* __restrict__ bias,
                   float* __restrict__ stats, int64_t stats_ld, BnBwd bb, ConvGeo geo) {
  using Cfg = X62Cfg<WM, WN>;
  extern __shared__ __attribute__((aligned(16))) char smem[];
  int bx, by;
  xcd_remap2(bx, by);
  const int tid = threadIdx.x;
  const int lane = tid & 63;
  const int wave = __builtin_amdgcn_readfirstlane(tid >> 6);
  const int wm = wave / WN, wn = wave % WN;
  const int fr = lane & 15, fq = lane >> 4;
  const int n0 = by * Cfg::BN;
  const int Ntot = (int)gridDim.y * Cfg::BN;
  const int64_t mtiles = (M + Cfg::BM - 1) / Cfg::BM;
  const int nk = K / 32;
  const int64_t my_tiles = bx < mtiles ? (mtiles - 1 - bx) / gridDim.x + 1 : 0;
  const int T_ = (int)(my_tiles * nk);
  if (T_ == 0) {
    if (stats)
      for (int c = tid; c < Cfg::BN; c += Cfg::THREADS) {
        stats[(int64_t)bx * Ntot + n0 + c] = 0.f;
        stats[stats_ld + (int64_t)bx * Ntot + n0 + c] = 0.f;
      }
    return;
  }

  f32x4 ra[NPF][Cfg::PRA][2], rb[NPF][P3 ? 1 : Cfg::PRB][2];
  u32x4 rb3[NPF][P3 ? Cfg::PRB : 1][3];
  const uint16_t* lpb3[P3 ? Cfg::PRB : 1];
  int64_t l_mt = bx;
  int l_ks = 0;
  const float* lpa[GATHER ? 1 : Cfg::PRA];
  const float* lpb[Cfg::PRB];
  int l_kh = 0, l_kw = 0, l_c0 = 0;
  uint32_t okhw[GATHER ? Cfg::PRA : 1];
  int32_t aoff[GATHER ? Cfg::PRA : 1];
  auto set_a_rows = [&]() __attribute__((always_inline)) {
    const int64_t m0 = l_mt * Cfg::BM;
#pragma unroll
    for (int p = 0; p < Cfg::PRA; ++p) {
      const int cid = tid + Cfg::THREADS * p;
      int64_t gr = m0 + (cid >> 2);
      gr = gr < M ? gr : M - 1;
      if constexpr (GATHER) {
        const uint32_t ohw = (uint32_t)(geo.OH * geo.OW);
        const uint32_t mu = (uint32_t)gr;
        const uint32_t n = mu / ohw, rem = mu - n * ohw;
        const uint32_t oh = rem / (uint32_t)geo.OW, ow = rem - oh * (uint32_t)geo.OW;
        const int ih0 = (int)oh * geo.S - geo.P, iw0 = (int)ow * geo.S - geo.P;
        uint32_t bh = 0u, bw = 0u;
#pragma unroll
        for (int t = 0; t < kMaxTaps; ++t) {
          bh |= (uint32_t)((unsigned)(ih0 + t) < (unsigned)geo.H) << t;
          bw |= (uint32_t)((unsigned)(iw0 + t) < (unsigned)geo.W) << t;
        }
        okhw[p] = bh | (bw << 8);
        aoff[p] = (((int)n * geo.H + ih0) * geo.W + iw0) * geo.C + (cid & 3) * 8;
      } else {
        lpa[p] = A + gr * lda + (cid & 3) * 8;
      }
    }
  };
  set_a_rows();
#pragma unroll
  for (int p = 0; p < Cfg::PRB; ++p) {
    const int cid = tid + Cfg::THREADS * p;
    if constexpr (P3) lpb3[p] = geo.b3 + (int64_t)(n0 + (cid >> 2)) * (3 * K) + (cid & 3) * 8;
    else lpb[p] = B + (int64_t)(n0 + (cid >> 2)) * ldb + (cid & 3) * 8;
  }
  const float* zrow = static_cast<const float*>(geo.zero);
  auto issue_loads = [&](auto SET) __attribute__((always_inline)) {
    constexpr int q = decltype(SET)::value;
    const int64_t toff = GATHER ? (int64_t)(l_kh * geo.W + l_kw) * geo.C + l_c0 : 0;
#pragma unroll
    for (int p = 0; p < Cfg::PRA; ++p) {
      const float* src;
      if constexpr (GATHER) {
        const bool ok = ((okhw[p] >> l_kh) & (okhw[p] >> (8 + l_kw)) & 1u) != 0u;
        src = ok ? A + ((int64_t)aoff[p] + toff) : zrow;
      } else {
        src = lpa[p];
        lpa[p] += 32;
      }
      ra[q][p][0] = *reinterpret_cast<const f32x4*>(src);
      ra[q][p][1] = *reinterpret_cast<const f32x4*>(src + 4);
    }
#pragma unroll
    for (int p = 0; p < Cfg::PRB; ++p) {
      if constexpr (P3) {
#pragma unroll
        for (int pl = 0; pl < 3; ++pl) rb3[q][p][pl] = *reinterpret_cast<const u32x4*>(lpb3[p] + pl * 32);
        lpb3[p] += 96;
      } else {
        rb[q][p][0] = *reinterpret_cast<const f32x4*>(lpb[p]);
        rb[q][p][1] = *reinterpret_cast<const f32x4*>(lpb[p] + 4);
        lpb[p] += 32;
      }
    }
    if constexpr (GATHER) {
      l_c0 += 32;
      if (l_c0 == geo.C) {
        l_c0 = 0;
        if (++l_kw == geo.KW) {
          l_kw = 0;
          ++l_kh;
        }
      }
    }
    if (++l_ks == nk) {
      l_ks = 0;
      l_kh = l_kw = l_c0 = 0;
      l_mt += gridDim.x;
      set_a_rows();
#pragma unroll
      for (int p = 0; p < Cfg::PRB; ++p) {
        if constexpr (P3) lpb3[p] -= 3 * K;
        else lpb[p] -= K;
      }
    }
  };
  auto split_write = [&](int buf, auto SET, int pc = -1) __attribute__((always_inline)) {
    constexpr int q = decltype(SET)::value;
    char* st = smem + buf * Cfg::STAGE;
#pragma unroll
    for (int p = 0; p < Cfg::PRA; ++p) {
      if (pc >= 0 && pc != p) continue;
      const int cid = tid + Cfg::THREADS * p;
      const int r = cid >> 2;
      bf16x8 h, m, l;
      split3x8(ra[q][p][0], ra[q][p][1], h, m, l);
      const int off = r * 64 + (((cid & 3) ^ x62_swz(r)) << 4);
      *reinterpret_cast<bf16x8*>(st + off) = h;
      *reinterpret_cast<bf16x8*>(st + Cfg::PA + off) = m;
      *reinterpret_cast<bf16x8*>(st + 2 * Cfg::PA + off) = l;
    }
    char* sb = st + 3 * Cfg::PA;
#pragma unroll
    for (int p = 0; p < Cfg::PRB; ++p) {
      if (pc >= 0 && pc != Cfg::PRA + p) continue;
      const int cid = tid + Cfg::THREADS * p;
      const int r = cid >> 2;
      const int off = r * 64 + (((cid & 3) ^ x62_swz(r)) << 4);
      if constexpr (P3) {
        *reinterpret_cast<u32x4*>(sb + off) = rb3[q][p][0];
        *reinterpret_cast<u32x4*>(sb + Cfg::PB + off) = rb3[q][p][1];
        *reinterpret_cast<u32x4*>(sb + 2 * Cfg::PB + off) = rb3[q][p][2];
      } else {
        bf16x8 h, m, l;
        split3x8(rb[q][p][0], rb[q][p][1], h, m, l);
        *reinterpret_cast<bf16x8*>(sb + off) = h;
        *reinterpret_cast<bf16x8*>(sb + Cfg::PB + off) = m;
        *reinterpret_cast<bf16x8*>(sb + 2 * Cfg::PB + off) = l;
      }
    }
  };

  f32x4 acc[4][4];
#pragma unroll
  for (int a = 0; a < 4; ++a)
#pragma unroll
    for (int b = 0; b < 4; ++b) acc[a][b] = f32x4{0.f, 0.f, 0.f, 0.f};
  float ssum[4][4], ssq[4][4], bia[BNB ? 1 : 4][4];
#pragma unroll
  for (int a = 0; a < 4; ++a)
#pragma unroll
    for (int b = 0; b < 4; ++b) {
      ssum[a][b] = ssq[a][b] = 0.f;
      if constexpr (!BNB) bia[a][b] = bias ? bias[n0 + wn * 64 + a * 16 + fq * 4 + b] : 0.f;
    }

  auto epilogue = [&](int64_t mt) __attribute__((always_inline)) {
    const int64_t mbase = mt * Cfg::BM;
    constexpr int EH = BNB ? 1 : 4;
#pragma unroll
    for (int ms = 0; ms < 4; ++ms) {
      const int64_t m = mbase + wm * 64 + ms * 16 + fr;
      const bool live = m < M;
#pragma unroll
      for (int nh = 0; nh < 4; nh += EH) {
      f32x4 ehv[EH], ed2[EH];
      uint32_t ebits[EH];
      if constexpr (BNB) {
#pragma unroll
        for (int e = 0; e < EH; ++e) {
          ehv[e] = ed2[e] = f32x4{0.f, 0.f, 0.f, 0.f};
          ebits[e] = 0u;
        }
        if (live) {
#pragma unroll
          for (int e = 0; e < EH; ++e) {
            const int n = n0 + wn * 64 + (nh + e) * 16 + fq * 4;
            ehv[e] = *reinterpret_cast<const f32x4*>(static_cast<const float*>(bb.h) + m * ldc + n);
            if (bb.dy2) ed2[e] = *reinterpret_cast<const f32x4*>(static_cast<const float*>(bb.dy2) + m * ldc + n);
            ebits[e] = bb.mask ? (uint32_t)bb.mask[m * (Ntot >> 2) + (n >> 2)] : 0xfu;
          }
        }
      }
#pragma unroll
      for (int e = 0; e < EH; ++e) {
        const int ns = nh + e;
        const int n = n0 + wn * 64 + ns * 16 + fq * 4;
        f32x4 v = acc[ms][ns];
        acc[ms][ns] = f32x4{0.f, 0.f, 0.f, 0.f};
        if constexpr (!BNB) {
#pragma unroll
          for (int r = 0; r < 4; ++r) v[r] += bia[ns][r];
        }
        if constexpr (BNB) {
#pragma unroll
          for (int r = 0; r < 4; ++r) {
            const float dz = (ebits[e] >> r) & 1u ? v[r] + ed2[e][r] : 0.f;
            v[r] = dz;
            ssum[ns][r] += dz;
            ssq[ns][r] = fmaf(dz, ehv[e][r], ssq[ns][r]);
          }
        } else {
          if (stats && live) {
#pragma unroll
            for (int r = 0; r < 4; ++r) {
              ssum[ns][r] += v[r];
              ssq[ns][r] = fmaf(v[r], v[r], ssq[ns][r]);
            }
          }
        }
        if (live) *reinterpret_cast<f32x4*>(C + m * ldc + n) = v;
      }
      }
    }
  };

  using I0 = std::integral_constant<int, 0>;
  using I1 = std::integral_constant<int, (NPF > 1 ? 1 : 0)>;
  issue_loads(I0{});
  split_write(0, I0{});
  if (T_ > 1) issue_loads(I1{});
  if (NPF > 1 && T_ > 2) issue_loads(I0{});
  __syncthreads();
  int ks = 0;
  int64_t mt = bx;
  auto slice = [&](int t, auto PAR) __attribute__((always_inline)) {
    constexpr int par = decltype(PAR)::value;
    using SN = std::integral_constant<int, (NPF > 1 ? (par ^ 1) : 0)>;
    const int cur = par;
    const char* st = smem + cur * Cfg::STAGE;
    const char* pa = st;
    const char* pb = st + 3 * Cfg::PA;
    auto frag = [&](const char* plane, int row) __attribute__((always_inline)) -> bf16x8 {
      return *reinterpret_cast<const bf16x8*>(plane + row * 64 + ((fq ^ x62_swz(row)) << 4));
    };
    bf16x8 bh[4], bm[4], bl[4];
#pragma unroll
    for (int ns = 0; ns < 4; ++ns) {
      const int row = wn * 64 + ns * 16 + fr;
      bh[ns] = frag(pb, row);
      bm[ns] = frag(pb + Cfg::PB, row);
      bl[ns] = frag(pb + 2 * Cfg::PB, row);
    }
    constexpr int NPC = Cfg::PRA + Cfg::PRB;
#pragma unroll
    for (int ms = 0; ms < 4; ++ms) {
      const int row = wm * 64 + ms * 16 + fr;
      const bf16x8 ah = frag(pa, row), am = frag(pa + Cfg::PA, row), al = frag(pa + 2 * Cfg::PA, row);
#pragma unroll
      for (int ns = 0; ns < 4; ++ns) {
        f32x4 c = acc[ms][ns];
        c = __builtin_amdgcn_mfma_f32_16x16x32_bf16(bl[ns], ah, c, 0, 0, 0);
        c = __builtin_amdgcn_mfma_f32_16x16x32_bf16(bh[ns], al, c, 0, 0, 0);
        c = __builtin_amdgcn_mfma_f32_16x16x32_bf16(bm[ns], am, c, 0, 0, 0);
        c = __builtin_amdgcn_mfma_f32_16x16x32_bf16(bm[ns], ah, c, 0, 0, 0);
        c = __builtin_amdgcn_mfma_f32_16x16x32_bf16(bh[ns], am, c, 0, 0, 0);
        acc[ms][ns] = __builtin_amdgcn_mfma_f32_16x16x32_bf16(bh[ns], ah, c, 0, 0, 0);
        const int gstep = 4 * ms + ns;
        if (gstep >= 1 && gstep <= NPC) split_write(cur ^ 1, SN{}, gstep - 1);
        if (gstep == NPC + 1) issue_loads(SN{});
        __builtin_amdgcn_sched_barrier(0);
      }
    }
    if (++ks == nk) {
      ks = 0;
      epilogue(mt);
      mt += gridDim.x;
    }
    __syncthreads();
  };
  for (int t = 0; t < T_; t += 2) {
    slice(t, I0{});
    if (t + 1 < T_) slice(t + 1, std::integral_constant<int, 1>{});
  }

  if (stats) {
#pragma unroll
    for (int a = 0; a < 4; ++a)
#pragma unroll
      for (int b = 0; b < 4; ++b)
#pragma unroll
        for (int off = 1; off < 16; off <<= 1) {
          ssum[a][b] += __shfl_xor(ssum[a][b], off, 64);
          ssq[a][b] += __shfl_xor(ssq[a][b], off, 64);
        }
    float* red = reinterpret_cast<float*>(smem);
    if (fr == 0) {
#pragma unroll
      for (int a = 0; a < 4; ++a)
#pragma unroll
        for (int b = 0; b < 4; ++b) {
          const int col = wn * 64 + a * 16 + fq * 4 + b;
          red[wm * Cfg::BN + col] = ssum[a][b];
          red[(WM + wm) * Cfg::BN + col] = ssq[a][b];
        }
    }
    __syncthreads();
    for (int c = tid; c < Cfg::BN; c += Cfg::THREADS) {
      float sa = 0.f, sb = 0.f;
#pragma unroll
      for (int w2 = 0; w2 < WM; ++w2) {
        sa += red[w2 * Cfg::BN + c];
        sb += red[(WM + w2) * Cfg::BN + c];
      }
      stats[(int64_t)bx * Ntot + n0 + c] = sa;
      stats[stats_ld + (int64_t)bx * Ntot + n0 + c] = sb;
    }
  }
}

template <int WM, int WN, bool BNB, int NPF, bool GATHER, bool P3 = false>
int launch_nt_x62(const float* A, int64_t lda, const float* B, int64_t ldb, float* C, int64_t ldc, int64_t M, int N,
                  int K, int max_blocks, const float* bias, float* stats, int64_t stats_ld, int stats_rows,
                  const BnBwd& bb, const ConvGeo& geo, hipStream_t stream) {
  using Cfg = X62Cfg<WM, WN>;
  const int ntiles = N / Cfg::BN;
  const int64_t mtiles = (M + Cfg::BM - 1) / Cfg::BM;
  const int per_cu = (160 * 1024) / Cfg::LDS > 0 ? (160 * 1024) / Cfg::LDS : 1;
  int64_t gx = ((int64_t)256 * per_cu + ntiles - 1) / ntiles;
  if (max_blocks > 0) gx = max_blocks;
  if (gx < 1) gx = 1;
  if (gx > mtiles) gx = mtiles;
  if (stats && gx > stats_rows) gx = stats_rows;
  static bool attr = [] {
    return hipFuncSetAttribute(reinterpret_cast<const void*>(&gemm_nt_x62_kernel<WM, WN, BNB, NPF, GATHER, P3>),
                               hipFuncAttributeMaxDynamicSharedMemorySize, 160 * 1024) == hipSuccess;
  }();
  (void)attr;
  hipLaunchKernelGGL((gemm_nt_x62_kernel<WM, WN, BNB, NPF, GATHER, P3>), dim3((unsigned)gx, (unsigned)ntiles), dim3(Cfg::THREADS),
                     Cfg::LDS, stream, A, lda, B, ldb, C, ldc, M, K, bias, stats, stats_ld, bb, geo);
  return (int)gx;
}

template <bool GATHER>
int nt_x62_dispatch(const float* A, int64_t lda, const float* B, int64_t ldb, float* C, int64_t ldc, int64_t M,
                    int N, int K, const cfg::NtWord& w, int max_blocks, const float* bias, float* stats,
                    int64_t stats_ld, int stats_rows, const BnBwd& bb, const ConvGeo& geo, hipStream_t stream) {
  const cfg::X62NtSel s = cfg::nt_x62_select(w, N, geo.b3 != nullptr, bb.h != nullptr);
#define GK_X62N(WM_, WN_, P3_)                                                                                      \
  return s.bnb ? launch_nt_x62<WM_, WN_, true, 1, GATHER, P3_>(A, lda, B, ldb, C, ldc, M, N, K, max_blocks, bias, stats, \
                                                               stats_ld, stats_rows, bb, geo, stream)                  \
               : launch_nt_x62<WM_, WN_, false, 1, GATHER, P3_>(A, lda, B, ldb, C, ldc, M, N, K, max_blocks, bias,     \
                                                                stats, stats_ld, stats_rows, bb, geo, stream)
#define GK_X62(WM_, WN_)               \
  case cfg::x62_key(WM_, WN_):         \
    if (s.p3) GK_X62N(WM_, WN_, true); \
    GK_X62N(WM_, WN_, false)
  switch (cfg::x62_key(s.wm, s.wn)) {
    GK_X62(2, 4);
    GK_X62(4, 2);
    GK_X62(1, 4);
    GK_X62(4, 1);
    GK_X62(1, 2);
    GK_X62(2, 1);
    GK_X62(2, 2);
  }
#undef GK_X62
#undef GK_X62N
  return cfg::kDoesNotFit;
}

}
}
```

### gaussiank_sgd_amd/ops/csrc/kernels/gemm_units.h

```cpp
#pragma once

#include <hip/hip_runtime.h>

#include "gemm_cfg.h"
#include "gk_kernels.h"

namespace gk {

constexpr int kMaxTaps = 4;

struct ConvGeo {
  const void* zero;
  int H, W, C, OH, OW, S, P, KW;
  const float* bias;
  int RH, RW, RA, RB, RZ;
  int KZ;
  const uint16_t* b3;
};

struct BnBwd {
  const void* h;
  const void* dy2;
  const uint8_t* mask;
};

struct LazyA {
  const void* x;
  const float* coef;
  const void* padz;
  const void* padx;
  int C;
};

#define GK_NT_UNIT_ARGS                                                                                  \
  const void *A, int64_t lda, const void *B, int64_t ldb, void *C, int64_t ldc, int64_t M, int N, int K, \
      const cfg::NtWord &w, int max_blocks, const ConvGeo &geo, float *stats, int64_t stats_ld,         \
      int stats_rows, const BnBwd &bb, const LazyArgs *lza, hipStream_t stream
#define GK_NT_UNIT_PASS A, lda, B, ldb, C, ldc, M, N, K, w, max_blocks, geo, stats, stats_ld, stats_rows, bb, lza, stream
int nt_b16_row(GK_NT_UNIT_ARGS);
int nt_b16_gat(GK_NT_UNIT_ARGS);
int nt_f32_row(GK_NT_UNIT_ARGS);
int nt_f32_gat(GK_NT_UNIT_ARGS);
int nt_x6_row(GK_NT_UNIT_ARGS);
int nt_x6_gat(GK_NT_UNIT_ARGS);
int nt_x62_row(const float* A, int64_t lda, const float* B, int64_t ldb, float* C, int64_t ldc, int64_t M, int N, int K,
               const cfg::NtWord& w, int max_blocks, const float* bias, float* stats, int64_t stats_ld, int stats_rows,
               const BnBwd& bb, const uint16_t* b3, hipStream_t stream);
int nt_x62_gat(const float* A, const float* B, float* C, int64_t M, int N, int K, const cfg::NtWord& w, int max_blocks,
               const ConvGeo& geo, float* stats, int64_t stats_ld, int stats_rows, const BnBwd& bb,
               hipStream_t stream);
void tn_x62_row(const float* G, int64_t ldg, const float* X, int64_t ldx, float* W, int64_t ldw, int64_t M, int N,
                int K, const cfg::TnF32Word& w, int splits, hipStream_t stream);
void tn_unit_x6(bool gather, const float* G, int64_t ldg, const float* X, int64_t ldx, float* W, int64_t ldw,
                int64_t M, int N, int K, const cfg::TnF32Word& w, int splits, const ConvGeo& geo, const LazyArgs* lza,
                hipStream_t stream);
void tn_unit_b16(bool gather, const void* G, int64_t ldg, const void* X, int64_t ldx, float* W, int64_t ldw, int64_t M,
                 int N, int K, const cfg::TnWord& w, int splits, const ConvGeo& geo, hipStream_t stream);
void tn_unit_f32(bool gather, const float* G, int64_t ldg, const float* X, int64_t ldx, float* W, int64_t ldw,
                 int64_t M, int N, int K, const cfg::TnF32Word& w, int splits, const ConvGeo& geo, const LazyArgs* lza,
                 hipStream_t stream);

}
```

### gaussiank_sgd_amd/ops/csrc/kernels/gk_kernels.h

```cpp
#pragma once

#include <hip/hip_runtime.h>
#include <stddef.h>
#include <stdint.h>

namespace gk {

enum Mode : int {
  kModeGaussian = 0,
  kModeRedSync = 1,
  kModeRedSyncTrim = 2,
  kModeTopK = 3,
  kModeRandomK = 4,
  kModeThreshold = 5,
  kModeDGC = 6,
  kModeGaussianCal = 7,
};

constexpr int kCalFallback = 16;
constexpr int kOverflowExact = 17;

constexpr int kMaxCand = 16;
constexpr int kRecHdr = 4;
constexpr int kMaxCountBlocks = 1024;
// ... 114 lines not shown
  uint16_t* w_bf16 = nullptr;
  const float* lr_mult = nullptr;
};
void fused_sgd(const SgdArgs& a, hipStream_t stream);

struct AdamGroup {
  double lr, beta1, beta2, eps, weight_decay;
  int decoupled;
  int pad0;
};
struct AdamArgs {
  float* w = nullptr;
  float* m = nullptr;
  float* v = nullptr;
  float* g = nullptr;
  const Chunk* chunks = nullptr;
  int nchunks = 0;
  AdamGroup groups[kMaxGroups];
  int ngroups = 0;
  int zero_grad = 1;
  float* step = nullptr;
  const float* grad_scale = nullptr;
  uint16_t* w_bf16 = nullptr;
  const float* lr_mult = nullptr;
};
void fused_adam(const AdamArgs& a, hipStream_t stream);

struct LambGroup {
  double lr, beta1, beta2, eps, weight_decay;
  double trust_clip;
  int adapt;
  int pad0;
};
struct LambArgs {
  float* w = nullptr;
  float* m = nullptr;
  float* v = nullptr;
  float* g = nullptr;
  const Chunk* chunks = nullptr;
  int nchunks = 0;
  LambGroup groups[kMaxGroups];
  int ngroups = 0;
  int zero_grad = 1;
  float* step = nullptr;
  const float* grad_scale = nullptr;
  uint16_t* w_bf16 = nullptr;
  const float* lr_mult = nullptr;
  const int32_t* seg_range = nullptr;
  int nseg = 0;
  double* part = nullptr;
  float* trust = nullptr;
  int passes = 7;
};
void fused_lamb(const LambArgs& a, hipStream_t stream);

struct McArgs {
  float* u = nullptr;
  float* g = nullptr;
  const float* w = nullptr;
  const Chunk* chunks = nullptr;
  int nchunks = 0;
  float momentum[kMaxGroups];
  float weight_decay[kMaxGroups];
};
void momentum_correct(const McArgs& a, hipStream_t stream);
void mask_records(float* u, const int32_t* record, int64_t k_cap, hipStream_t stream);

void accum_grad(float* dst, const void* src, int64_t n, int src_bytes, hipStream_t stream);
void cast_bf16(uint16_t* dst, const float* src, int64_t n, hipStream_t stream);

void segmented_sumsq(const float* w, const float* g, const Chunk* chunks, int nchunks, double* out,
                     hipStream_t stream);

struct LarsArgs {
  float* w = nullptr;
  float* m = nullptr;
  const float* g = nullptr;
  const Chunk* chunks = nullptr;
  int nchunks = 0;
  const double* seg_sumsq = nullptr;
  float lr[kMaxGroups], momentum[kMaxGroups], weight_decay[kMaxGroups], eeta[kMaxGroups],
      epsilon[kMaxGroups];
  int ngroups = 0;
};
void fused_lars(const LarsArgs& a, hipStream_t stream);

void clip_grad_norm(float* g, int64_t n, float max_norm, double* ws, float* coef_out,
                    float* norm_out, hipStream_t stream);

size_t bn_workspace_floats(int64_t M, int C, int elem_bytes);
size_t bn_fin_state_bytes(int C);
bool bn_supported(int C, int elem_bytes);
void bn_set_blocks(int blocks);
size_t bn_mask_bytes(int64_t M, int C, int elem_bytes);
void bn_stats_partials(const void* x, int64_t M, int C, int elem_bytes, float* ws, hipStream_t s);
void bn_act_forward(const void* x, const void* res, void* y, uint8_t* mask, int64_t M, int C, int elem_bytes,
                    const float* w, const float* b, float eps, float momentum, float* run_mean, float* run_var,
                    float* save_mean, float* save_invstd, float* scale, float* shift, float* ws, int relu,
                    int64_t* nbt, hipStream_t stream, void* fin_state = nullptr, const float* rscale = nullptr,
                    const float* rshift = nullptr);
void bn_act_finalize(const void* x, int64_t M, int C, int elem_bytes, const float* psum, const float* psq, int gy,
                     const float* w, const float* b, float eps, float momentum, float* run_mean, float* run_var,
                     float* save_mean, float* save_invstd, float* scale, float* shift, float* ws, int64_t* nbt,
                     hipStream_t stream);
void bn_act_forward_pre(const void* x, const void* res, void* y, uint8_t* mask, int64_t M, int C, int elem_bytes,
                        const float* psum, const float* psq, int gy, const float* w, const float* b, float eps, float momentum,
                        float* run_mean, float* run_var, float* save_mean, float* save_invstd, float* scale,
                        float* shift, int relu, int64_t* nbt, hipStream_t stream, void* fin_state = nullptr,
                        const float* rscale = nullptr, const float* rshift = nullptr);
void bn_bwd_finalize_lazy(const float* pdb, const float* pdg, int gy, int64_t M, int C, int elem_bytes, int center,
                          const float* w, const float* mean, const float* invstd, float* dgamma, float* dbeta,
                          float* gw_acc, float* gb_acc, float* coef, void* padz, void* padx, hipStream_t stream);
void bn_act_backward_lazy(const void* dy, const void* dy2, const uint8_t* mask, const void* x, void* dz, int64_t M,
                          int C, int elem_bytes, const float* w, const float* mean, const float* invstd,
                          float* dgamma, float* dbeta, float* ws, int relu, float* gw_acc, float* gb_acc, float* coef,
                          void* padz, void* padx, hipStream_t stream);
void bn_lazy_apply(const void* dz, const void* x, void* dx, int64_t M, int C, int elem_bytes, const float* coef,
                   hipStream_t stream);
void bn_act_backward_pre_dual(const void* dz, const void* x, void* dx, int64_t M, int C, int elem_bytes,
                              const float* w, const float* mean, const float* invstd, float* dgamma, float* dbeta,
                              const float* pdb, const float* pdg, int gy, float* gw_acc, float* gb_acc, const void* x2,
                              void* dx2, const float* w2, const float* mean2, const float* invstd2, float* dgamma2,
                              float* dbeta2, float* ws2, float* gw2_acc, float* gb2_acc, hipStream_t stream);
void bn_act_backward_pre(const void* dz, const void* x, void* dx, int64_t M, int C, int elem_bytes, const float* w,
                         const float* mean, const float* invstd, float* dgamma, float* dbeta, const float* pdb,
                         const float* pdg, int gy, float* gw_acc, float* gb_acc, hipStream_t stream,
                         void* fin_state = nullptr);
void bn_act_backward(const void* dy, const void* dy2, const uint8_t* mask, const void* x, void* dx, void* dres,
                     int64_t M, int C, int elem_bytes, const float* w, const float* mean, const float* invstd,
                     float* dgamma, float* dbeta, float* ws, int relu, float* gw_acc, float* gb_acc,
                     hipStream_t stream, void* fin_state = nullptr);

struct PoolGeo {
  int H, W, OH, OW, k, s, p;
};
void bn_relu_pool_forward_pre(const void* x, void* y, uint8_t* amax, int64_t N, int C, PoolGeo pg, int elem_bytes,
                              const float* psum,
                              const float* psq, int gy, const float* w, const float* b, float eps, float momentum,
                              float* run_mean, float* run_var, float* save_mean, float* save_invstd, float* scale,
                              float* shift, int64_t* nbt, hipStream_t stream);
void bn_relu_pool_forward(const void* x, void* y, uint8_t* amax, int64_t N, int C, PoolGeo pg, int elem_bytes,
                          const float* w, const float* b, float eps, float momentum, float* run_mean, float* run_var,
                          float* save_mean, float* save_invstd, float* scale, float* shift, float* ws, int64_t* nbt,
                          hipStream_t stream);
void bn_relu_pool_backward(const void* dy, const void* dy2, const uint8_t* amax, const void* x, void* dx, int64_t N,
                           int C, PoolGeo pg, int elem_bytes, const float* w, const float* mean, const float* invstd,
                           float* dgamma, float* dbeta, float* ws, float* gw_acc, float* gb_acc, hipStream_t stream);

bool gemm_supported(int64_t N, int64_t K);
struct BnBwdArgs {
  const void* h;
  const void* dy2;
  const uint8_t* mask;
};
struct LazyArgs {
  const void* x;
  const float* coef;
  const void* padz;
  const void* padx;
  int C;
};
int gemm_nt(const void* A, int64_t lda, const void* B, int64_t ldb, void* C, int64_t ldc, int64_t M, int N, int K,
            bool f32, int cfg, int max_blocks, float* stats, int stats_rows, const float* bias, const BnBwdArgs* bn,
            const LazyArgs* lazy, hipStream_t stream, float* splitk_ws = nullptr, const void* b3 = nullptr);
int splitk_reduce(const float* ws, int S, int64_t M, int N, float* C, int64_t ldc, const float* bias, float* stats,
                  int stats_rows, const BnBwdArgs* bn, hipStream_t stream);
int gemm_tn_acc(const void* G, int64_t ldg, const void* X, int64_t ldx, float* W, int64_t ldw, int64_t M, int N,
                 int K, bool f32, int cfg, int splits, const LazyArgs* lazy, hipStream_t stream);
int conv_nt(const void* X, const void* zero, int H, int W, int C, int OH, int OW, int S, int P, int KH, int KW,
            const void* B, void* Y, int64_t M, int N, bool f32, int cfg, int max_blocks, float* stats, int stats_rows,
            const float* bias, const BnBwdArgs* bn, const LazyArgs* lazy, hipStream_t stream,
            float* splitk_ws = nullptr, const void* b3 = nullptr);
void split3_rows(const float* src, int64_t ld, void* dst, int64_t R, int S, hipStream_t stream);
int conv_nt_remap(const void* X, int64_t ldx, const void* zero, int H, int W, int C, int OH, int OW, int KH, int KW,
                  const void* B, void* Y, int64_t M, int N, int RH, int RW, int RA, int RB, int RZ, bool f32, int cfg,
                  int max_blocks, const LazyArgs* lazy, hipStream_t stream);
int conv_tn_acc(const void* G, const void* X, const void* zero, int H, int W, int C, int OH, int OW, int S, int P,
                 int KH, int KW, float* Wout, int64_t M, int N, bool f32, int cfg, int splits, const LazyArgs* lazy,
                 hipStream_t stream);
bool stem_f32_supported(int H, int W);
int stem_f32_wgrad_blocks(int N);
int stem_f32x6_wplanes();
int stem_f32x6_forward(const float* x, int N, int H, int W, const float* w, int64_t s0, int64_t s1, int64_t s2,
                       int64_t s3, uint16_t* wp3, float* y, float* stats, int stats_rows, hipStream_t stream);
int stem_f32_forward(const float* x, int N, int H, int W, const float* w, int64_t s0, int64_t s1, int64_t s2,
                     int64_t s3, float* y, float* stats, int stats_rows, hipStream_t stream);
void stem_f32_wgrad(const float* x, const float* dy, int N, int H, int W, float* part, float* out, int64_t s0,
                    int64_t s1, int64_t s2, int64_t s3, bool x6, hipStream_t stream);
void wino_weights(const float* w, float* u, int Co, int Ci, int flip, hipStream_t stream);
enum PrepKind : int32_t { kPrepWino = 0, kPrepWinoFlip = 1, kPrepT32 = 2, kPrepT16 = 3, kPrepWinoX6 = 4,
                          kPrepWinoX6Flip = 5 };
struct PrepDesc {
  const void* src;
  void* dst;
  int64_t ld_in, ld_out;
  int64_t block_begin;
  int32_t kind, R, S, tiles_s;
};
static_assert(sizeof(PrepDesc) == 56, "PrepDesc layout is packed by ops/weight_prep.py");
int64_t weight_prep_blocks(int kind, int R, int S);
int weight_prep_max_descs();
void weight_prep(const PrepDesc* descs, int ndesc, int64_t total_blocks, hipStream_t stream);
int wino_conv(const float* x, const float* u, float* y, int N, int H, int W, int Ci, int Co, int max_blocks,
              float* stats, int stats_rows, const BnBwdArgs* bn, hipStream_t stream, int splits = 1,
              float* split_ws = nullptr);
void wino_x6_weights(const float* w, uint16_t* u3, int Co, int Ci, int flip, hipStream_t stream);
int wino_x6_conv(const float* x, const uint16_t* u3, float* y, int N, int H, int W, int Ci, int Co, int max_blocks,
                 float* stats, int stats_rows, const BnBwdArgs* bn, hipStream_t stream);
int wino_wgrad_splits(int N, int H, int W, int C, int K, int splits);
void wino_wgrad(const float* x, const float* dy, float* part, float* out, int N, int H, int W, int C, int K,
                int splits, hipStream_t stream);

bool stem_supported(int H, int W);
void stem_pack_weight(const float* w, int64_t s0, int64_t s1, int64_t s2, int64_t s3, uint16_t* wp,
                      hipStream_t stream);
int stem_forward(const void* x, bool x_f32, int N, int H, int W, const uint16_t* wp, uint16_t* y, float* stats,
                 int stats_rows, hipStream_t stream);
int stem_wgrad_blocks(int N, int H, int W);
void stem_wgrad(const void* x, bool x_f32, int N, int H, int W, const uint16_t* dy, float* part, float* out,
                int64_t s0, int64_t s1, int64_t s2, int64_t s3, hipStream_t stream);

bool wgrad3_supported(int H, int W, int C, int K);
int64_t wgrad3_ws_floats(int N, int H, int W, int C, int K);
void wgrad3_acc(const void* dy, const void* x, const void* zero, int N, int H, int W, int C, int K, float* part,
                float* out, int64_t s0, int64_t s1, int64_t s2, int64_t s3, hipStream_t stream);

bool attn_supported(int T, int D);
bool attn_f32_supported(int T, int D);
void attn_f32_fwd(const float* qkv, float* out, float* lse, int B, int T, int H, float p, uint32_t seed,
                  const uint32_t* seed_dev, const uint32_t* key_bits, hipStream_t stream);
void attn_f32_bwd(const float* qkv, const float* out, const float* dout, const float* lse, float* delta, float* dqkv,
                  int B, int T, int H, float p, uint32_t seed, const uint32_t* seed_dev, const uint32_t* key_bits,
                  hipStream_t stream);
void attn_fwd(const void* qkv, void* out, float* lse, int B, int T, int H, float p, uint32_t seed,
              const uint32_t* seed_dev, const uint32_t* key_bits, void* out_lo, hipStream_t stream);
void attn_bwd(const void* qkv, const void* out, const void* dout, const float* lse, float* delta, void* dqkv, int B,
              int T, int H, float p, uint32_t seed, const uint32_t* seed_dev, const uint32_t* key_bits,
              const void* out_lo, hipStream_t stream);
void attn_pack_key_mask(const void* mask, int elem_size, bool is_float, uint32_t* bits, int B, int T,
                        hipStream_t stream);
void attn_dropout_mask(uint8_t* mask, int B, int H, int T, float p, uint32_t seed, const uint32_t* seed_dev,
                       hipStream_t stream);

int emb_type_parts();
bool emb_supported(int H, int NT);
void emb_forward(const int64_t* ids, const int64_t* tt, const float* Ww, const float* Wp, const float* Wt, float* out,
                 int64_t M, int T, int H, hipStream_t s);
int64_t emb_word_maxc(int64_t M);
int64_t emb_word_ws_ints(int64_t V, int64_t M);
void emb_backward(const int64_t* ids, const int64_t* tt, const float* dx, float* dWw, float* dWp, float* dWt,
                  float* part, const int64_t* sid, const int64_t* order, int* wws, float* wpart, int64_t V,
                  int64_t M, int B, int T, int P, int NT, int H, hipStream_t s);

bool xent_supported(int V);
void xent_forward(const void* logits, const int64_t* labels, float* lse, float* loss, int64_t R, int V, int64_t ignore,
                  hipStream_t s);
void xent_backward(const void* logits, const int64_t* labels, const float* lse, const float* scale, void* grad,
                   int64_t R, int V, int64_t ignore, hipStream_t s);

bool add_ln_supported(int H);
int64_t add_ln_partial_rows(int64_t R);
void add_ln_forward(const void* a, const void* x, const float* gamma, const float* beta, void* y, void* hsave,
                    float* mean, float* rstd, int64_t R, int H, float eps, float p, uint32_t seed,
                    const uint32_t* seed_dev, hipStream_t stream, bool f32 = false);
void add_ln_backward(const void* dy, const void* hsave, const float* mean, const float* rstd, const float* gamma,
                     void* dx, void* da, float* dgamma, float* dbeta, int accumulate, float* ws, int64_t R, int H,
                     float p, uint32_t seed, const uint32_t* seed_dev, hipStream_t stream, bool f32 = false);

void colsum_acc_bf16(const uint16_t* dy, float* db, int64_t M, int N, hipStream_t stream);
void gelu_bwd_colsum_bf16(const uint16_t* dy, const uint16_t* pre, uint16_t* dpre, float* db, int64_t M, int N,
                          hipStream_t stream);
void colsum_acc_f32(const float* dy, float* db, int64_t M, int N, hipStream_t stream);
void gelu_bwd_colsum_f32(const float* dy, const float* pre, float* dpre, float* db, int64_t M, int N,
                         hipStream_t stream);

void lstm_rec_gemm(const uint16_t* A, int64_t lda, const uint16_t* B, int64_t ldb, float* P, int M, int N, int K,
                   int S, hipStream_t stream);
void lstm_cell_fwd(const uint16_t* xg, const uint16_t* hg, const float* P, int S, const float* c_prev, float* c, uint16_t* h,
                   uint16_t* h_pad, float* gates, int B, int H, int Hp, hipStream_t stream);
void lstm_cell_bwd(const uint16_t* dout, const uint16_t* dh_rec, const float* P, int S, const float* dc_next, const float* gates,
                   const float* c, const float* c_prev, uint16_t* dG, uint16_t* dG_pad, float* dc_prev, int B, int H,
                   int Hp, hipStream_t stream);
void lstm_rec_gemm_x6(const float* A, int64_t lda, const uint16_t* B3, int64_t ldb, int64_t bplane, float* P, int M,
                      int N, int K, int S, hipStream_t stream);
void lstm_rec_gemm_f32(const float* A, int64_t lda, const float* B, int64_t ldb, float* P, int M, int N, int K, int S,
                       hipStream_t stream);
void lstm_cell_fwd_f32(const float* xg, const float* hg, const float* P, int S, const float* c_prev, float* c, float* h,
                       float* h_pad, float* gates, int B, int H, int Hp, hipStream_t stream);
void lstm_cell_bwd_f32(const float* dout, const float* dh_rec, const float* P, int S, const float* dc_next,
                       const float* gates, const float* c, const float* c_prev, float* dG, float* dG_pad, float* dc_prev,
                       int B, int H, int Hp, hipStream_t stream);

}
```

Before: 5117 images/s.

## Fuse stride-2 downsample dgrad into BN-backward epilogue via compact dy2

In backward, the stride-2 1x1 downsample shortcut's input gradient is kept as a compact [N*OH*OW, C] GEMM result instead of a full-resolution scatter. The preceding block's conv dgrad then runs an x62 GEMM whose BN-backward epilogue reads the compact dy2 only at even (h, w) pixels, using magic-number division. This aims to drop the full-size zero-filled dgrad tensor and the separate residual add, and lets the previous block's output BN backward fuse across downsample boundaries. The forward order moves the shortcut call after the main-path convs. Unsupported configs return a new status code, and a Python scatter fallback rebuilds the full tensor when fusion cannot happen.

```diff
diff --git a/gaussiank_sgd_amd/models/resnet_imagenet.py b/gaussiank_sgd_amd/models/resnet_imagenet.py
--- a/gaussiank_sgd_amd/models/resnet_imagenet.py
+++ b/gaussiank_sgd_amd/models/resnet_imagenet.py
@@ -31,10 +31,10 @@
 
     def forward(self, x):
         x, xs = x if isinstance(x, tuple) else (x, x)
-        identity = xs if self.downsample is None else _shortcut(self.downsample, xs, self.bn2)
         y, st = conv_stats(self.conv1, x)
         out = self.bn1(y, stats=st)
         y, st = conv_stats(self.conv2, out)
+        identity = xs if self.downsample is None else _shortcut(self.downsample, xs, self.bn2)
         return self.bn2(y, identity, stats=st)
 
 
@@ -54,12 +54,12 @@
 
     def forward(self, x):
         x, xs = x if isinstance(x, tuple) else (x, x)
-        identity = xs if self.downsample is None else _shortcut(self.downsample, xs, self.bn3)
         y, st = conv_stats(self.conv1, x)
         out = self.bn1(y, stats=st)
         y, st = conv_stats(self.conv2, out)
         out = self.bn2(y, stats=st)
         y, st = conv_stats(self.conv3, out)
+        identity = xs if self.downsample is None else _shortcut(self.downsample, xs, self.bn3)
         return self.bn3(y, identity, stats=st)
 
 
@@ -82,6 +82,12 @@
     if isinstance(ds, ConvBN):
         return ds.forward_deferred(xs, consumer)
     return ds(xs)
+
+
+def _compact_shortcut(b: nn.Module) -> bool:
+    ds = b.downsample
+    return isinstance(b, Bottleneck) and isinstance(ds, ConvBN) and isinstance(ds[0], Conv1x1) and \
+        ds[0].stride == (2, 2)
 
 
 class ResNet(nn.Module):
@@ -116,7 +122,7 @@
             b.bn1.bwd_link = True
             if isinstance(b, Bottleneck):
                 b.bn2.bwd_link = True
-            if i + 1 < len(blocks) and blocks[i + 1].downsample is None:
+            if i + 1 < len(blocks) and (blocks[i + 1].downsample is None or _compact_shortcut(blocks[i + 1])):
                 (b.bn3 if isinstance(b, Bottleneck) else b.bn2).bwd_link = True
         if zero_init_residual:
             for m in self.modules():
diff --git a/gaussiank_sgd_amd/ops/autotune.py b/gaussiank_sgd_amd/ops/autotune.py
--- a/gaussiank_sgd_amd/ops/autotune.py
+++ b/gaussiank_sgd_amd/ops/autotune.py
@@ -75,6 +75,10 @@
         return []
     base = list(_SPLITK_BASE) + ([c + X6 for c in _SPLITK_BASE] if _x6() else [])
     return [c + 10000 * S for S in (2, 4, 8) if K % (64 * S) == 0 and K // S >= 128 for c in base]
+
+
+def nt_x62_cfgs() -> List[int]:
+    return list(_NT_CFGS_X62)
 
 
 
diff --git a/gaussiank_sgd_amd/ops/bn.py b/gaussiank_sgd_amd/ops/bn.py
--- a/gaussiank_sgd_amd/ops/bn.py
+++ b/gaussiank_sgd_amd/ops/bn.py
@@ -30,17 +30,27 @@
 
 class BnLink:
 
-    __slots__ = ("h", "mask", "twin", "dy2", "dz", "part")
+    __slots__ = ("h", "mask", "twin", "dy2", "dz", "part", "dy2c", "geo")
 
     def __init__(self):
-        self.h = self.mask = self.dy2 = self.dz = self.part = None
+        self.h = self.mask = self.dy2 = self.dz = self.part = self.dy2c = self.geo = None
         self.twin = False
 
     def ready(self) -> bool:
         return self.h is not None and (not self.twin or self.dy2 is not None)
 
+    def scatter_dy2c(self) -> Optional[torch.Tensor]:
+        if self.dy2c is None:
+            return None
+        H, W, OH, OW = self.geo
+        C = self.dy2c.shape[1]
+        N = self.dy2c.shape[0] // (OH * OW)
+        full = torch.empty((N, C, H, W), dtype=self.dy2c.dtype, device=self.dy2c.device, memory_format=_CL).zero_()
+        full[:, :, ::2, ::2] = self.dy2c.view(N, OH, OW, C).permute(0, 3, 1, 2)
+        return full
+
     def clear(self) -> None:
-        self.h = self.mask = self.dy2 = self.dz = self.part = None
+        self.h = self.mask = self.dy2 = self.dz = self.part = self.dy2c = self.geo = None
 
 
 class ProducerLink:
@@ -160,9 +170,10 @@
             dgamma = g[0] if weight is not None and ctx.needs_input_grad[2] else None
             dbeta = g[1] if ctx.needs_input_grad[3] else None
             return (dx, dres, dgamma, dbeta) + (None,) * 14
+        d2c = link.scatter_dy2c() if link is not None else None
         if link is not None:
             link.clear()
-        dy, dy2 = _grad_pair(grads, x)
+        dy, dy2 = _grad_pair(tuple(grads) + (d2c,), x)
         if dy is None:
             return (None,) * 18
         C = x.shape[1]
diff --git a/gaussiank_sgd_amd/ops/conv1x1.py b/gaussiank_sgd_amd/ops/conv1x1.py
--- a/gaussiank_sgd_amd/ops/conv1x1.py
+++ b/gaussiank_sgd_amd/ops/conv1x1.py
@@ -277,8 +277,63 @@
     return dz
 
 
+def _link_on(ds: bool = False) -> bool:
+    return os.environ.get("GKSGD_BN_LINK", "1") != "0" and \
+        not (ds and os.environ.get("GKSGD_BN_LINK_DS", "1") == "0")
+
+
+def _ds_compact_ok(ds_link, x: torch.Tensor, w: torch.Tensor, s: int, dt: torch.dtype) -> bool:
+    return (ds_link is not None and s == 2 and w.shape[2] == 1 and dt == torch.float32 and _link_on(ds=True) and
+            f32_matmul() == "bf16x6" and ds_link.h is not None and ds_link.h.dtype == dt and
+            ds_link.h.shape == x.shape and ds_link.dy2 is None and ds_link.dy2c is None and
+            x.numel() // x.shape[1] < (1 << 31))
+
+
+def _dgrad_ds(dy: torch.Tensor, w: torch.Tensor, x_shape, wp: bool = False) -> torch.Tensor:
+    N, C, H, W, K, k, p, OH, OW = _geom(x_shape, w, 2)
+    g = _g()
+    dt = dy.dtype
+    dxc = torch.empty(N * OH * OW, C, dtype=dt, device=dy.device)
+    DY = _rows(dy)
+    Wt = _lazy(lambda: weight_prep.transposed_1x1(w, wp))
+    run = lambda c, mb: g.gemm_nt(DY, Wt(), dxc, c, mb)
+    cands = autotune.hip_cands(run, product(autotune.nt_cfgs(dt), autotune.NT_GRIDS))
+    cands += autotune.hip_cands(run, product(autotune.splitk_cfgs(dt, N * OH * OW, C, K), autotune.SPLITK_GRIDS))
+    ch = autotune.pick(("dgrad_ds", N, C, H, W, K) + autotune.dkey(dt), cands)
+    run(ch[1], ch[2])
+    return dxc
+
+
+def _ds_fusable(link, x: torch.Tensor, w: torch.Tensor, s: int, dt: torch.dtype, dgrad_key: tuple, lz) -> bool:
+    if not (s == 1 and w.shape[2] == 1 and dt == torch.float32 and lz is None and _link_on(ds=True) and
+            f32_matmul() == "bf16x6" and link.h is not None and link.h.dtype == dt and link.h.shape == x.shape):
+        return False
+    ch = autotune.choice(dgrad_key)
+    return ch is None or ch[0] == "hip"
+
+
+def _dgrad_bn_ds(dy: torch.Tensor, w: torch.Tensor, x_shape, link, wp: bool = False) -> torch.Tensor:
+    N, C, H, W, K, k, p, OH, OW = _geom(x_shape, w, 1)
+    g = _g()
+    M = N * H * W
+    dt = dy.dtype
+    dz = torch.empty(x_shape, dtype=dt, device=dy.device, memory_format=_CL)
+    st = torch.empty(2, min(1280, (M + 63) // 64), C, dtype=torch.float32, device=dy.device)
+    DY, DZ, H2 = _rows(dy), _rows(dz), _rows(link.h)
+    D2, geo, mask = link.dy2c, list(link.geo), link.mask
+    Wt = _lazy(lambda: weight_prep.transposed_1x1(w, wp))
+    run = lambda c, mb: g.gemm_nt(DY, Wt(), DZ, c, mb, st, None, H2, D2, mask, bn_dy2_geo=geo)
+    cands = autotune.hip_cands(run, product(autotune.nt_x62_cfgs(), autotune.NT_GRIDS))
+    ch = autotune.pick(("dgrad_bn_ds", N, C, H, W, K) + autotune.dkey(dt), cands)
+    rows = run(ch[1], ch[2])
+    link.part = (st, int(rows))
+    link.dz = dz
+    link.dy2c = None
+    return dz
+
+
 def _bn_fusable(link, s: int, dgrad_key: tuple) -> bool:
-    if link is None or s != 1 or os.environ.get("GKSGD_BN_LINK", "1") == "0" or not link.ready():
+    if link is None or s != 1 or not _link_on() or not link.ready():
         return False
     if link.h.dtype != dgrad_key_dtype(dgrad_key):
         return False
@@ -362,7 +417,7 @@
 
     @staticmethod
     def forward(ctx, x, param, w_bf16, sink, stride, stats_box=None, bias=None, bias_sink=None, link=None,
-                dt=torch.bfloat16, plink=None):
+                dt=torch.bfloat16, plink=None, ds_link=None):
         if x.dtype != dt:
             x = x.to(dt)
         x = x.contiguous(memory_format=_CL)
@@ -382,6 +437,7 @@
         ctx.stride = stride
         ctx.param_dtype = param.dtype
         ctx.link = link
+        ctx.ds_link = ds_link
         ctx.dt = dt
         ctx.plink = plink
         ctx.save_for_backward(x, w)
@@ -393,6 +449,7 @@
         s = ctx.stride
         dy = dy.to(ctx.dt).contiguous(memory_format=_CL)
         link, ctx.link = ctx.link, None
+        ds_link, ctx.ds_link = ctx.ds_link, None
         plink, ctx.plink = ctx.plink, None
         lz = plink.lazy if plink is not None and plink.matches(dy) else None
         if plink is not None and plink.lazy is not None and lz is None:
@@ -429,7 +486,15 @@
             key = _dgrad_key(N, C, H, W, w.shape[0], w.shape[2], s, ctx.dt)
             prep, ctx.prep = ctx.prep, None
             with weight_prep.use(prep):
-                if _bn_fusable(link, s, key):
+                if lz is None and _ds_compact_ok(ds_link, x, w, s, ctx.dt):
+                    ds_link.dy2c = _dgrad_ds(dy, w, x.shape, wp=ctx.wp)
+                    ds_link.geo = (H, W, dy.shape[2], dy.shape[3])
+                elif link is not None and link.dy2c is not None:
+                    if _ds_fusable(link, x, w, s, ctx.dt, key, lz):
+                        dx = _dgrad_bn_ds(dy, w, x.shape, link, wp=ctx.wp)
+                    else:
+                        dx = _dgrad(dy, w, x.shape, s, lz, plink, wp=ctx.wp)
+                elif _bn_fusable(link, s, key):
                     dx = _dgrad_bn(dy, w, x.shape, s, link, lz, plink, wp=ctx.wp)
                 else:
                     dx = _dgrad(dy, w, x.shape, s, lz, plink, wp=ctx.wp)
@@ -470,7 +535,7 @@
                 gbias = db
         if plink is not None:
             plink.clear()
-        return dx, gparam, None, None, None, None, gbias, None, None, None, None
+        return dx, gparam, None, None, None, None, gbias, None, None, None, None, None
 
 
 class FastConv2d(nn.Conv2d):
@@ -505,12 +570,13 @@
             if not torch.is_grad_enabled() or self.bias is None or not self.bias.requires_grad:
                 bsink = None
             link = getattr(x, "_gk_bn_link", None)
+            ds_link = getattr(x, "_gk_res_link", None) if f32 and not bf16 and torch.is_grad_enabled() else None
             plink = None
             if f32 and not bf16 and torch.is_grad_enabled():
                 from .bn import ProducerLink
                 plink = ProducerLink()
             y = _FastConvFn.apply(x, self.weight, w_bf16, sink, self.stride[0], box, self.bias, bsink, link,
-                                  torch.bfloat16 if bf16 else torch.float32, plink)
+                                  torch.bfloat16 if bf16 else torch.float32, plink, ds_link)
             if plink is not None:
                 y._gk_plink = plink
             return y
diff --git a/gaussiank_sgd_amd/ops/csrc/bindings.cpp b/gaussiank_sgd_amd/ops/csrc/bindings.cpp
--- a/gaussiank_sgd_amd/ops/csrc/bindings.cpp
+++ b/gaussiank_sgd_amd/ops/csrc/bindings.cpp
@@ -1207,8 +1207,13 @@
 
 bool bn_bwd_args(const c10::optional<at::Tensor>& h, const c10::optional<at::Tensor>& dy2,
                  const c10::optional<at::Tensor>& mask, int64_t M, int64_t N,
-                 int64_t ldc, bool has_stats, at::ScalarType dt, gk::BnBwdArgs* out) {
-  if (!h.has_value() || !h->defined()) return false;
+                 int64_t ldc, bool has_stats, at::ScalarType dt, gk::BnBwdArgs* out,
+                 c10::OptionalArrayRef<int64_t> dy2_geo = c10::nullopt) {
+  const bool compact = dy2_geo.has_value();
+  if (!h.has_value() || !h->defined()) {
+    TORCH_CHECK(!compact, "bn_dy2_geo needs the BN-backward epilogue operands");
+    return false;
+  }
   TORCH_CHECK(has_stats, "BN-backward epilogue needs the stats partials buffer");
   auto rows_ok = [&](const at::Tensor& t, const char* what) {
     TORCH_CHECK(t.is_cuda() && t.scalar_type() == dt && t.numel() == M * N &&
@@ -1219,7 +1224,19 @@
   rows_ok(*h, "bn h");
   out->h = h->data_ptr();
   out->dy2 = nullptr;
-  if (dy2.has_value() && dy2->defined()) {
+  out->H = out->W = out->OH = out->OW = 0;
+  if (compact) {
+    TORCH_CHECK(dy2_geo->size() == 4 && dy2.has_value() && dy2->defined(), "bn_dy2_geo is [H, W, OH, OW] of a given bn_dy2");
+    const int64_t H = (*dy2_geo)[0], W = (*dy2_geo)[1], OH = (*dy2_geo)[2], OW = (*dy2_geo)[3];
+    TORCH_CHECK(H > 0 && W > 0 && OH == (H + 1) / 2 && OW == (W + 1) / 2 && M % (H * W) == 0 && M < (int64_t(1) << 31),
+                "bn_dy2_geo: OH x OW must be the stride-2 grid of the H x W pixels of C's rows (M < 2^31)");
+    TORCH_CHECK(dt == at::kFloat && dy2->is_cuda() && dy2->scalar_type() == dt && dy2->dim() == 2 &&
+                    dy2->size(0) == M / (H * W) * OH * OW && dy2->size(1) == N && dy2->stride(0) == ldc &&
+                    dy2->stride(1) == 1,
+                "compact bn dy2 must be fp32 [M / (H W) * OH * OW, N] with C's row stride");
+    out->dy2 = dy2->data_ptr();
+    out->H = (int)H, out->W = (int)W, out->OH = (int)OH, out->OW = (int)OW;
+  } else if (dy2.has_value() && dy2->defined()) {
     rows_ok(*dy2, "bn dy2");
     out->dy2 = dy2->data_ptr();
   }
@@ -1277,6 +1294,8 @@
   static int64_t checked(const char* op, int r) {
     TORCH_CHECK(r != gk::cfg::kRowGemmsOnly, op,
                 ": the register-staged bf16x6 kernels (cfg digit 200000/300000) take plain row GEMMs only");
+    TORCH_CHECK(r != gk::cfg::kCompactDy2, op,
+                ": a compact bn_dy2 takes one register-staged bf16x6 row GEMM (cfg digit 200000/300000, no split-K)");
     TORCH_CHECK(r >= 0, op, ": the lazy operand's coefficient table does not fit this tile configuration");
     return r;
   }
@@ -1285,7 +1304,8 @@
 int64_t gemm_nt(at::Tensor A, at::Tensor B, at::Tensor C, int64_t cfg, int64_t max_blocks,
                 c10::optional<at::Tensor> stats, c10::optional<at::Tensor> bias, c10::optional<at::Tensor> bn_h,
                 c10::optional<at::Tensor> bn_dy2, c10::optional<at::Tensor> bn_mask, c10::optional<at::Tensor> lz_x, c10::optional<at::Tensor> lz_coef,
-                c10::optional<at::Tensor> lz_padz, c10::optional<at::Tensor> lz_padx) {
+                c10::optional<at::Tensor> lz_padz, c10::optional<at::Tensor> lz_padx,
+                c10::OptionalArrayRef<int64_t> bn_dy2_geo) {
   check_rows(A, "A", A);
   check_rows(B, "B", A);
   check_rows(C, "C", A);
@@ -1296,7 +1316,8 @@
   int rows = 0;
   float* sp = stats_ptr(stats, N, &rows);
   gk::BnBwdArgs bn{};
-  const bool has_bn = bn_bwd_args(bn_h, bn_dy2, bn_mask, M, N, C.stride(0), sp != nullptr, C.scalar_type(), &bn);
+  const bool has_bn = bn_bwd_args(bn_h, bn_dy2, bn_mask, M, N, C.stride(0), sp != nullptr, C.scalar_type(), &bn,
+                                  bn_dy2_geo);
   TORCH_CHECK(!has_bn || !bias.has_value() || !bias->defined(), "gemm_nt: bias and BN epilogue are exclusive");
   gk::LazyArgs lz{};
   const bool has_lz = lazy_args(lz_x, lz_coef, lz_padz, lz_padx, A, K, &lz);
@@ -2139,7 +2160,8 @@
   m.def("cast_bf16(Tensor(a!) dst, Tensor src) -> ()");
   m.def("gemm_supported(int N, int K) -> bool", &gemm_supported);
   m.def("gemm_nt(Tensor A, Tensor B, Tensor(a!) C, int cfg=0, int max_blocks=0, Tensor(b!)? stats=None, "
-        "Tensor? bias=None, Tensor? bn_h=None, Tensor? bn_dy2=None, Tensor? bn_mask=None, Tensor? lz_x=None, Tensor? lz_coef=None, Tensor? lz_padz=None, Tensor? lz_padx=None) -> int");
+        "Tensor? bias=None, Tensor? bn_h=None, Tensor? bn_dy2=None, Tensor? bn_mask=None, Tensor? lz_x=None, Tensor? lz_coef=None, Tensor? lz_padz=None, Tensor? lz_padx=None, "
+        "int[]? bn_dy2_geo=None) -> int");
   m.def("gemm_tn_acc(Tensor G, Tensor X, Tensor(a!) W, int cfg=0, int splits=0, Tensor? lz_x=None, Tensor? lz_coef=None, Tensor? lz_padz=None, Tensor? lz_padx=None) -> ()");
   m.def("conv_nt(Tensor x, Tensor w, Tensor(a!) y, Tensor zero, int stride, int pad, int cfg=0, int max_blocks=0, "
         "Tensor(b!)? stats=None, Tensor? bias=None, Tensor? bn_h=None, Tensor? bn_dy2=None, Tensor? bn_mask=None, "
diff --git a/gaussiank_sgd_amd/ops/csrc/kernels/gemm.hip b/gaussiank_sgd_amd/ops/csrc/kernels/gemm.hip
--- a/gaussiank_sgd_amd/ops/csrc/kernels/gemm.hip
+++ b/gaussiank_sgd_amd/ops/csrc/kernels/gemm.hip
@@ -131,6 +131,7 @@
   const cfg::NtPlan p = cfg::nt_plan(w, f32, gather, lazy != nullptr, g.b3 != nullptr, g.RH != 0, splitk_ws != nullptr, K,
                                      g.C, x_elems);
   if (p.status < 0) return p.status;
+  if (bn && bn->OW > 0 && (gather || p.unit != cfg::Unit::x62 || p.planes > 1)) return cfg::kCompactDy2;
   if (p.planes > 1) {
     ConvGeo gz = g;
     gz.bias = nullptr;
@@ -141,7 +142,12 @@
     if (r < 0) return r;
     return splitk_reduce(splitk_ws, p.planes, M, N, static_cast<float*>(C), ldc, g.bias, stats, stats_rows, bn, stream);
   }
-  const BnBwd bb = bn ? BnBwd{bn->h, bn->dy2, bn->mask} : BnBwd{};
+  BnBwd bb = bn ? BnBwd{bn->h, bn->dy2, bn->mask, bn->H, bn->W, bn->OH, bn->OW} : BnBwd{};
+  if (bb.OW > 0) {
+    if (M >= ((int64_t)1 << 31) || M % ((int64_t)bb.H * bb.W) != 0) return cfg::kCompactDy2;
+    magic_u32((uint32_t)(bb.H * bb.W), &bb.mg_hw, &bb.sh_hw);
+    magic_u32((uint32_t)bb.W, &bb.mg_w, &bb.sh_w);
+  }
   return nt_unit(p.unit, gather, A, lda, B, ldb, C, ldc, M, N, K, w, max_blocks, g, stats, (int64_t)stats_rows * N,
                  stats_rows, bb, lazy, stream);
 }
diff --git a/gaussiank_sgd_amd/ops/csrc/kernels/gemm_cfg.h b/gaussiank_sgd_amd/ops/csrc/kernels/gemm_cfg.h
--- a/gaussiank_sgd_amd/ops/csrc/kernels/gemm_cfg.h
+++ b/gaussiank_sgd_amd/ops/csrc/kernels/gemm_cfg.h
@@ -8,6 +8,7 @@
 enum Status : int {
   kDoesNotFit = -1,
   kRowGemmsOnly = -2,
+  kCompactDy2 = -3,
 };
 
 inline int family_of(int cfg) {
diff --git a/gaussiank_sgd_amd/ops/csrc/kernels/gemm_nt_x62.h b/gaussiank_sgd_amd/ops/csrc/kernels/gemm_nt_x62.h
--- a/gaussiank_sgd_amd/ops/csrc/kernels/gemm_nt_x62.h
+++ b/gaussiank_sgd_amd/ops/csrc/kernels/gemm_nt_x62.h
@@ -21,7 +21,7 @@
   static_assert(LDS <= 160 * 1024, "LDS");
 };
 
-template <int WM, int WN, bool BNB, int NPF = 1, bool GATHER = false, bool P3 = false>
+template <int WM, int WN, bool BNB, int NPF = 1, bool GATHER = false, bool P3 = false, bool D2C = false>
 __global__ void __launch_bounds__(64 * WM * WN) __attribute__((amdgpu_waves_per_eu(1)))
 gemm_nt_x62_kernel(const float* __restrict__ A, int64_t lda, const float* __restrict__ B, int64_t ldb,
                    float* __restrict__ C, int64_t ldc, int64_t M, int K, const float* __restrict__ bias,
@@ -212,11 +212,23 @@
           ebits[e] = 0u;
         }
         if (live) {
+          int32_t d2row = -1;
+          if constexpr (BNB && D2C) {
+            const uint32_t mu = (uint32_t)m;
+            const uint32_t img = (__umulhi(mu, bb.mg_hw) + mu) >> bb.sh_hw, rem = mu - img * (uint32_t)(bb.H * bb.W);
+            const uint32_t ph = (__umulhi(rem, bb.mg_w) + rem) >> bb.sh_w, pw = rem - ph * (uint32_t)bb.W;
+            if (((ph | pw) & 1u) == 0u) d2row = (int32_t)((img * (uint32_t)bb.OH + (ph >> 1)) * (uint32_t)bb.OW + (pw >> 1));
+          }
 #pragma unroll
           for (int e = 0; e < EH; ++e) {
             const int n = n0 + wn * 64 + (nh + e) * 16 + fq * 4;
             ehv[e] = *reinterpret_cast<const f32x4*>(static_cast<const float*>(bb.h) + m * ldc + n);
-            if (bb.dy2) ed2[e] = *reinterpret_cast<const f32x4*>(static_cast<const float*>(bb.dy2) + m * ldc + n);
+            if constexpr (D2C) {
+              if (d2row >= 0)
+                ed2[e] = *reinterpret_cast<const f32x4*>(static_cast<const float*>(bb.dy2) + (int64_t)d2row * ldc + n);
+            } else {
+              if (bb.dy2) ed2[e] = *reinterpret_cast<const f32x4*>(static_cast<const float*>(bb.dy2) + m * ldc + n);
+            }
             ebits[e] = bb.mask ? (uint32_t)bb.mask[m * (Ntot >> 2) + (n >> 2)] : 0xfu;
           }
         }
@@ -348,7 +360,7 @@
   }
 }
 
-template <int WM, int WN, bool BNB, int NPF, bool GATHER, bool P3 = false>
+template <int WM, int WN, bool BNB, int NPF, bool GATHER, bool P3 = false, bool D2C = false>
 int launch_nt_x62(const float* A, int64_t lda, const float* B, int64_t ldb, float* C, int64_t ldc, int64_t M, int N,
                   int K, int max_blocks, const float* bias, float* stats, int64_t stats_ld, int stats_rows,
                   const BnBwd& bb, const ConvGeo& geo, hipStream_t stream) {
@@ -362,11 +374,11 @@
   if (gx > mtiles) gx = mtiles;
   if (stats && gx > stats_rows) gx = stats_rows;
   static bool attr = [] {
-    return hipFuncSetAttribute(reinterpret_cast<const void*>(&gemm_nt_x62_kernel<WM, WN, BNB, NPF, GATHER, P3>),
+    return hipFuncSetAttribute(reinterpret_cast<const void*>(&gemm_nt_x62_kernel<WM, WN, BNB, NPF, GATHER, P3, D2C>),
                                hipFuncAttributeMaxDynamicSharedMemorySize, 160 * 1024) == hipSuccess;
   }();
   (void)attr;
-  hipLaunchKernelGGL((gemm_nt_x62_kernel<WM, WN, BNB, NPF, GATHER, P3>), dim3((unsigned)gx, (unsigned)ntiles), dim3(Cfg::THREADS),
+  hipLaunchKernelGGL((gemm_nt_x62_kernel<WM, WN, BNB, NPF, GATHER, P3, D2C>), dim3((unsigned)gx, (unsigned)ntiles), dim3(Cfg::THREADS),
                      Cfg::LDS, stream, A, lda, B, ldb, C, ldc, M, K, bias, stats, stats_ld, bb, geo);
   return (int)gx;
 }
@@ -376,11 +388,15 @@
                     int N, int K, const cfg::NtWord& w, int max_blocks, const float* bias, float* stats,
                     int64_t stats_ld, int stats_rows, const BnBwd& bb, const ConvGeo& geo, hipStream_t stream) {
   const cfg::X62NtSel s = cfg::nt_x62_select(w, N, geo.b3 != nullptr, bb.h != nullptr);
-#define GK_X62N(WM_, WN_, P3_)                                                                                      \
-  return s.bnb ? launch_nt_x62<WM_, WN_, true, 1, GATHER, P3_>(A, lda, B, ldb, C, ldc, M, N, K, max_blocks, bias, stats, \
-                                                               stats_ld, stats_rows, bb, geo, stream)                  \
-               : launch_nt_x62<WM_, WN_, false, 1, GATHER, P3_>(A, lda, B, ldb, C, ldc, M, N, K, max_blocks, bias,     \
-                                                                stats, stats_ld, stats_rows, bb, geo, stream)
+#define GK_X62L(WM_, WN_, BNB_, P3_, D2C_)                                                                   \
+  launch_nt_x62<WM_, WN_, BNB_, 1, GATHER, P3_, D2C_>(A, lda, B, ldb, C, ldc, M, N, K, max_blocks, bias, stats, \
+                                                      stats_ld, stats_rows, bb, geo, stream)
+#define GK_X62N(WM_, WN_, P3_)                                             \
+  do {                                                                     \
+    if constexpr (!GATHER)                                                 \
+      if (s.bnb && bb.OW > 0) return GK_X62L(WM_, WN_, true, P3_, true);   \
+    return s.bnb ? GK_X62L(WM_, WN_, true, P3_, false) : GK_X62L(WM_, WN_, false, P3_, false); \
+  } while (0)
 #define GK_X62(WM_, WN_)               \
   case cfg::x62_key(WM_, WN_):         \
     if (s.p3) GK_X62N(WM_, WN_, true); \
@@ -396,6 +412,7 @@
   }
 #undef GK_X62
 #undef GK_X62N
+#undef GK_X62L
   return cfg::kDoesNotFit;
 }
 
diff --git a/gaussiank_sgd_amd/ops/csrc/kernels/gemm_units.h b/gaussiank_sgd_amd/ops/csrc/kernels/gemm_units.h
--- a/gaussiank_sgd_amd/ops/csrc/kernels/gemm_units.h
+++ b/gaussiank_sgd_amd/ops/csrc/kernels/gemm_units.h
@@ -22,7 +22,16 @@
   const void* h;
   const void* dy2;
   const uint8_t* mask;
+  int H, W, OH, OW;
+  uint32_t mg_hw, sh_hw, mg_w, sh_w;
 };
+
+inline void magic_u32(uint32_t d, uint32_t* mg, uint32_t* sh) {
+  uint32_t s = 0;
+  while (((uint64_t)1 << s) < d) ++s;
+  *sh = s;
+  *mg = (uint32_t)(((((uint64_t)1 << s) - d) << 32) / d + 1);
+}
 
 struct LazyA {
   const void* x;
diff --git a/gaussiank_sgd_amd/ops/csrc/kernels/gk_kernels.h b/gaussiank_sgd_amd/ops/csrc/kernels/gk_kernels.h
--- a/gaussiank_sgd_amd/ops/csrc/kernels/gk_kernels.h
+++ b/gaussiank_sgd_amd/ops/csrc/kernels/gk_kernels.h
@@ -290,6 +290,7 @@
   const void* h;
   const void* dy2;
   const uint8_t* mask;
+  int H, W, OH, OW;
 };
 struct LazyArgs {
   const void* x;
```

Result: faster. 5217 images/s (median of 6 runs) (+1.9%).
